# kimkyeonghun/MSA

Hardware: AMD Instinct MI355X
Metric: train-step samples/sec (higher is better)
Workload: dtype bf16

## Files before the change

### include/mmbert_hip.h

```cpp
#ifndef MMBERT_HIP_H
#define MMBERT_HIP_H
#include <stddef.h>
#include <stdint.h>

#ifdef __cplusplus
extern "C" {
#endif

typedef struct ihipStream_t* mmbert_stream_t;

#define MMBERT_EPI_BIAS 1
#define MMBERT_EPI_GELU 2
#define MMBERT_EPI_RESID 4
#define MMBERT_EPI_GELU_BWD 8
#define MMBERT_EPI_OUT_F32 16

int mmbert_gemm_nt(mmbert_stream_t stream, const void* A, int lda, const void* B, int ldb, void* C, int ldc,
                   int M, int N, int K, int epi, const float* bias, const void* R, int ldr, void* aux, int ldaux,
                   const void* U, int ldu, float alpha, const float* alpha_dev,
                   uint32_t drop_stream, uint32_t drop_thr16, float drop_scale, int* tile_queue);

int mmbert_gemm_nt_splitk(mmbert_stream_t stream, const void* A, int lda, const void* B, int ldb, void* C, int ldc,
                          int M, int N, int K, void* workspace, const void* R, int ldr);
size_t mmbert_gemm_nt_splitk_workspace(int M, int N, int K);

void mmbert_gemm_nt_force(int mode);
int mmbert_gemm_nt_describe(int M, int N, int K, int epi, int with_queue, int* out);
void mmbert_gemm_tn_force_splits(int splits);
void mmbert_gemm_tn_force_one_launch(int on);

size_t mmbert_gemm_tn_workspace(int M, int N, int K, int* splits_out);
int mmbert_gemm_tn(mmbert_stream_t stream, const void* A, int lda, const void* B, int ldb, float* W, int ldw,
                   int M, int N, int K, int accumulate, float alpha, const float* alpha_dev, void* slab, float* bias_out);
size_t mmbert_gemm_tn_grouped_workspace(int nprob, const int* N, const int* K, int M, int* splits_out);
int mmbert_gemm_tn_grouped(mmbert_stream_t stream, int nprob, const void* const* A, const int* lda, const void* const* B, const int* ldb,
                           float* const* W, float* const* bias, const int* N, const int* K, int M,
                           int accumulate, float alpha, const float* alpha_dev, void* slab);
int mmbert_gemm_tn_grouped_rows(mmbert_stream_t stream, int nprob, const void* const* A, const int* lda, const void* const* B, const int* ldb,
                                float* const* W, float* const* bias, const int* N, const int* K, const int* M,
                                int accumulate, const int* accumulate_each, float alpha, const float* alpha_dev, void* slab);

int mmbert_colsum(mmbert_stream_t stream, const void* X, int ldx, int M, int N, float* out, float alpha, const float* alpha_dev);

uint32_t mmbert_rng_stream(uint64_t seed, uint32_t site);
uint32_t mmbert_dropout_thr16(float p);
int mmbert_dropout_mask(mmbert_stream_t stream, uint8_t* out, size_t n, uint32_t rng_stream, uint32_t thr16);

int mmbert_mlm_mask(mmbert_stream_t stream, int64_t* ids, int64_t* labels, size_t n, uint32_t rng_stream, uint32_t select_thr16,
                    uint32_t replace_thr16, int64_t special0, int64_t special1, int64_t special2, int64_t mask_id);

int mmbert_ln_fwd(mmbert_stream_t stream, const void* x, int ldx, const int* in_rows, void* y, int ldy, const int* out_rows,
                  int M, int H, const float* gamma, const float* beta, float eps, float* mean, float* rstd,
                  uint32_t dstream, uint32_t dthr, float dscale, int drop_row0);
int mmbert_ln_bwd(mmbert_stream_t stream, const void* dy, int lddy, const int* dy_rows, const void* x, int ldx, const int* x_rows,
                  const float* mean, const float* rstd, const float* gamma, int M, int H,
                  void* dx, int lddx, const int* dx_rows, void* dx2, int lddx2, float* dgamma, float* dbeta, float* dbias2,
                  uint32_t post_stream, uint32_t post_thr, float post_scale,
                  uint32_t pre_stream, uint32_t pre_thr, float pre_scale,
                  float* partial_ws , const int* drop_rows,
                  int defer_reduce ,
                  int dy_row_limit );
size_t mmbert_ln_bwd_workspace(int M, int H);
int mmbert_ln_bwd_reduce(mmbert_stream_t stream, int items, const float* const* partial_ws, float* const* dgamma, float* const* dbeta,
                         float* const* dbias2, int M, int H);
int mmbert_ln_bwd_reduce_rows(mmbert_stream_t stream, int items, const float* const* partial_ws, float* const* dgamma, float* const* dbeta,
                              float* const* dbias2, const int* M, int H);

int mmbert_embed_gather(mmbert_stream_t stream, const int64_t* ids, const int64_t* tts, const float* word, const float* type,
                        const float* pos, int n, int T, int H, int V, void* out, int ldo);
int mmbert_embed_scatter(mmbert_stream_t stream, const int64_t* ids, const int64_t* tts, const void* d, int ldd, int n, int T, int H, int V,
                         float* gword, float* gtype, float* gpos, float* type_slab);

int mmbert_pair_proj_fwd(mmbert_stream_t stream, const void* feat, int feat_f64, int B, int P, int D, const float* W, const float* bias, int H,
                         void* out, int ldo, int T);
int mmbert_pair_proj_bwd(mmbert_stream_t stream, const void* feat, int feat_f64, int B, int P, int D, const void* J, const void* dJ, int ld, int T,
                         float* dW, float* db, int H, void* workspace );
size_t mmbert_pair_proj_bwd_workspace(int B, int P, int D, int H);

int mmbert_attn_tile_rows(int which);
int mmbert_attn_kv_len(mmbert_stream_t stream, const float* key_bias, const int* bias_start, const int* seq_len, int nseq, int* kv_len);
int mmbert_attn_fwd(mmbert_stream_t stream, const void* qkv, void* ctx, float* lse, const float* key_bias, const int* bias_start, int H, int heads,
                    const int* seq_start, const int* seq_len, const unsigned* elem_base, const int* tile_seq, const int* tile_r0, int ntiles,
                    uint32_t dstream, uint32_t dthr, float dscale, const int* kv_len, const int* tile_qshift, const int* tile_qend);
int mmbert_attn_fwd_first(mmbert_stream_t stream, const void* qkv, void* ctx, const float* key_bias, const int* bias_start, int H, int heads,
                          const int* seq_start, const int* seq_len, const int* q_row, int nseq, const int* kv_len);
int mmbert_attn_probs_first(mmbert_stream_t stream, const void* qkv, float* probs, int ld, const float* key_bias, const int* bias_start, int H, int heads,
                            const int* seq_start, const int* seq_len, const int* q_row, int nseq, const int* kv_len );
int mmbert_attn_bwd(mmbert_stream_t stream, const void* qkv, const void* ctx, const void* dctx, void* dqkv, const float* lse, float* delta,
                    const float* key_bias, const int* bias_start, int H, int heads, const int* seq_start, const int* seq_len, const unsigned* elem_base,
                    const int* qtile_seq, const int* qtile_r0, int nqtiles,
                    const int* tile_seq, const int* tile_r0, int ntiles,
                    uint32_t dstream, uint32_t dthr, float dscale, const int* kv_len,
                    const int* qtile_qshift, const int* qtile_qend, int split,
                    const int* q_limit);
int mmbert_attn_q_limit(mmbert_stream_t stream, const int* rows, int n, const int* seq_start, int nseq, int* q_limit);
int mmbert_attn_dropout_mask(mmbert_stream_t stream, uint8_t* out, int S, unsigned elem_base, int head, uint32_t rng_stream, uint32_t thr16);

int mmbert_ce_fwd(mmbert_stream_t stream, const void* logits, int ldv, int V, const int64_t* labels, int M,
                  const int* seg_bounds, int nseg, float* inv_count, float* loss_sum, float* row_lse,
                  int logits_f32 ,
                  float* row_loss );
int mmbert_ce_bwd(mmbert_stream_t stream, const void* logits, int ldv, int V, const int64_t* labels, int M,
                  const int* seg_bounds, int nseg, const float* inv_count, const float* gscale, const float* row_lse, void* dlogits, int ldd,
                  const int* rows , int nrows,
                  int logits_f32 );
int mmbert_vocab_topk(mmbert_stream_t stream, const void* logits, int ldv, int V, int M, int logits_f32, int k,
                      const int64_t* labels ,
                      int32_t* top_ids , float* top_logprob , float* row_lse ,
                      float* label_logprob , int32_t* label_rank );
int mmbert_split_rows(mmbert_stream_t stream, const int64_t* row_seq, const int64_t* row_pos, const int* start_a, const int* start_b,
                      const int* valid, int mode, int M, int rows_a, int64_t* perm, int64_t* inv, const int* rank,
                      int* perm32 , int* inv32);

int mmbert_split_layout(mmbert_stream_t stream, const int* seq_len, const int* valid, int nseq, int tile_rows, int xs, int nf_max, int nq_max,
                        int* out);

int mmbert_prologue(mmbert_stream_t stream, int nseg, const void* const* seg_ptr, const long long* seg_stride_b, const long long* seg_stride_p,
                    const int* seg_dtype, const int* seg_pass, const int* seg_offset, const int* seg_len,
                    int npass, const int* pass_len, int B, const int64_t* labels, int vocab,
                    float* key_bias, int* kv_len, int* valid, int* seq_cnt, int* idx, int* words, int* rank, float* key_bias_perm);

int mmbert_rows_to_block(mmbert_stream_t stream, const int64_t* ids, const void* rows, int rows_bf16, int ldr, int n, int H,
                         const int64_t* uni, int U, int V, float* block);

int mmbert_pack_i64(mmbert_stream_t stream, int nseg, const int64_t* const* src, const long long* dst_offset, const long long* count,
                    const long long* fill, int64_t* out);

int mmbert_active_rows(mmbert_stream_t stream, const int64_t* labels, int M, int V, int* idx, int* count);

int mmbert_heads_gate_fwd(mmbert_stream_t stream, const float* P, const float* Apre, const float* const* vw3, const float* const* vb3, int B, int H, float* g, float* C);
int mmbert_heads_loss_fwd(mmbert_stream_t stream, const float* P, const float* XP, const float* rel, const int64_t* ap, const float* lo, const float* sent,
                          int B, int H, float beta, int tanh_lo, float* out5, float* dXP, float* dPc, float* drel, float* dlo, float* nce_part,
                          const float* mlm, int nmlm, float alpha, float* loss_out , float* aux_out );
int mmbert_heads_scale(mmbert_stream_t stream, float* x, size_t n, const float* s);
int mmbert_heads_seed(mmbert_stream_t stream, const float* src, size_t n, const float* s, float* dst, float* zero, size_t nzero, float* dmlm, int nmlm, float coef);
int mmbert_heads_gate_bwd(mmbert_stream_t stream, const float* dC, const float* P, const float* Apre, const float* g, const float* const* vw3, const float* dPc,
                          int B, int H, float* dP, float* dApre, float* E, float* dg);
int mmbert_heads_tanh(mmbert_stream_t stream, float* x, size_t n);
int mmbert_heads_tanh_bwd(mmbert_stream_t stream, const float* dP, const float* P, float* dpre, size_t n);
int mmbert_heads_colsum(mmbert_stream_t stream, int nseg, const float* const* src, float* const* dst, const int* rows, const int* cols, const int* ld);

typedef struct {
    int B, H, tanh_lo, nmlm;
    float alpha, beta;
    const float* first; const void* y; const int64_t* first_rows; int ldy, ncls;
    const int64_t* ap; const int64_t* ap2; const float* sent; const float* mlm;
    const float *Wp, *bp, *Wal, *bal, *Wsr, *bsr, *Wat, *bat, *vw[3], *vb[3], *Wc1, *bc1, *Wc2, *bc2, *Wq[3], *bq[3];
    float *loss, *aux, *out5, *logits, *t_rel, *rel;
    float* ws;
    const float* dloss; float* dfirst; float* dmlm;
    float *gWp, *gbp, *gWal, *gbal, *gWat, *gbat, *gvw[3], *gvb[3], *gWc1, *gbc1, *gWc2, *gbc2, *gWq[3], *gbq[3];
    unsigned* sync;
    const int64_t* sent_cls; int64_t* pred;
} mmbert_heads_step;
int mmbert_heads_step_struct_size(void);
size_t mmbert_heads_step_workspace(int B, int H);
int mmbert_heads_step_fwd(mmbert_stream_t stream, const mmbert_heads_step* p);
int mmbert_heads_step_bwd(mmbert_stream_t stream, const mmbert_heads_step* p);
int mmbert_heads_step_fwd_levels(mmbert_stream_t stream, const mmbert_heads_step* p, int lo, int hi);
int mmbert_heads_step_bwd_levels(mmbert_stream_t stream, const mmbert_heads_step* p, int lo, int hi);
int mmbert_heads_predict(mmbert_stream_t stream, const mmbert_heads_step* p);
int mmbert_heads_step_outputs(int B, int H, size_t* pooled_offset, size_t* fused_offset);
int mmbert_heads_step_dmlm(mmbert_stream_t stream, const mmbert_heads_step* p);

typedef struct { const float* X; const float* W; int ldx, ldw, inner, row0, rows, w_inner_major; } mmbert_skinny_src;
typedef struct { float* Y; const float* bias; int ldy, M, N, nsrc, act, accumulate; mmbert_skinny_src src[4]; } mmbert_skinny_op;
typedef struct { const float* dY; const float* X; float* dW; float* db; int ldy, ldx, ldw, M, N, K; } mmbert_skinny_wgrad_op;
int mmbert_skinny_mm(mmbert_stream_t stream, int nops, const mmbert_skinny_op* ops);
size_t mmbert_skinny_mm_workspace(int nops, const mmbert_skinny_op* ops);
int mmbert_skinny_mm_ordered(mmbert_stream_t stream, int nops, const mmbert_skinny_op* ops, void* workspace);
int mmbert_skinny_wgrad(mmbert_stream_t stream, int nops, const mmbert_skinny_wgrad_op* ops);

typedef struct { uint32_t stream, thr16; float scale; } mmbert_drop;
typedef struct {
    const float* key_bias; const int* bias_start; const int* seq_start; const int* seq_len; const unsigned* elem_base;
    const int* ftile_seq; const int* ftile_r0; const int* ftile_qshift; const int* ftile_qend;
    const int* qtile_seq; const int* qtile_r0; const int* qtile_qshift; const int* qtile_qend;
    const int* tile_seq; const int* tile_r0;
    const int* kv_len;
    int nftiles, nqtiles, ntiles, split, heads, pad_;
} mmbert_attn_layout;
typedef struct {
    const void* x;
    const void* Wqkv; const void* Wo; const void* W1; const void* W2;
    const float* bqkv; const float* bo; const float* b1; const float* b2; const float* ln1_g; const float* ln1_b; const float* ln2_g; const float* ln2_b;
    void* qkv; void* actx; float* lse; void* z1; void* y1; float* m1; float* r1; void* u ; void* g; void* z2; void* y2; float* m2; float* r2;
    const int* y2_rows;
    int* tile_queue;
    mmbert_drop att, h1, h2;
    int rows, H, I, ldx, ldy2; float ln_eps;
} mmbert_layer_fwd_args;
typedef struct {
    const void* dy; const int* dy_rows;
    const void* z2; const float* m2; const float* r2; const float* ln2_g; float* g_ln2_g; float* g_ln2_b; float* ln2_ws;
    const void* z1; const float* m1; const float* r1; const float* ln1_g; float* g_ln1_g; float* g_ln1_b; float* ln1_ws;
    const void* u; const void* qkv; const void* actx; const float* lse;
    const void* W2T; const void* W1T; const void* WoT; const void* WqkvT;
    void* dz2; void* dz2d ; void* du; void* dy1; void* dz1; void* dz1d ; void* dctx; void* dqkv; float* delta; void* dx;
    int* tile_queue;
    mmbert_drop att, h1, h2;
    int rows, H, I, lddy;
} mmbert_layer_bwd_args;
int mmbert_layer_fwd(mmbert_stream_t stream, const mmbert_attn_layout* layout, const mmbert_layer_fwd_args* a);
int mmbert_layer_bwd(mmbert_stream_t stream, const mmbert_attn_layout* layout, const mmbert_layer_bwd_args* a);
int mmbert_layer_struct_sizes(int* out );

void mmbert_set_deterministic(int on);
int mmbert_get_deterministic(void);
int mmbert_id_runs_sum_rows(mmbert_stream_t stream, const void* src, int src_bf16, int lds, const int64_t* ids, int n,
                            int H, int V, const int64_t* uni, int U, float* dst, int ldd);

int mmbert_adamw(mmbert_stream_t stream, float* p, float* g, float* m, float* v, void* p_bf16, const uint8_t* flags, size_t n,
                 double lr, double beta1, double beta2, double eps, double wd, int step, double gscale, int mode, int zero_grad);

int mmbert_adamw_devscale(mmbert_stream_t stream, float* p, float* g, float* m, float* v, void* p_bf16, const uint8_t* flags, size_t n,
                          double lr, double beta1, double beta2, double eps, double wd, int step, const float* coef, int mode, int zero_grad);

#define MMBERT_ADAMW_MAX_GROUPS 255
#define MMBERT_ADAMW_MAX_SLOTS 64
int mmbert_adamw_grouped(mmbert_stream_t stream, float* p, float* g, float* m, float* v, void* p_bf16, const uint8_t* flags,
                         const uint8_t* group_of_block, size_t n, const double* hyper, int ngroups, int step, double gscale,
                         const float* coef, int mode, int zero_grad);

#define MMBERT_GRAD_NORM_WORKSPACE 8192
int mmbert_grad_norm(mmbert_stream_t stream, const float* g, size_t n, const int64_t* segs, int nseg, double norm_type, double max_norm,
                     double gscale, void* workspace, float* out);
int mmbert_grad_scale(mmbert_stream_t stream, float* g, size_t n, const int64_t* segs, int nseg, const float* coef);

int mmbert_gelu_bwd(mmbert_stream_t stream, const void* dy, const void* u, void* du, size_t n);

int mmbert_cast_f32_bf16(mmbert_stream_t stream, const float* x, void* y, size_t n);
int mmbert_cast_bf16_f32(mmbert_stream_t stream, const void* x, float* y, size_t n);
int mmbert_transpose_cast(mmbert_stream_t stream, const float* src, void* dst, const void* descs, int ndesc, int total_tiles);
int mmbert_compact_rows(mmbert_stream_t stream, const int* rows32, const int64_t* rows64, int n, const int64_t* extra, int nextra, const int64_t* map,
                        int64_t* out64, int* out32);
int mmbert_compact_rows_inv(mmbert_stream_t stream, const int* rows32, const int64_t* rows64, int n, const int64_t* extra, int nextra, const int64_t* map,
                            int64_t* out64, int* out32, int64_t* inv_stamp, unsigned stamp);
int mmbert_scatter_rows_zero(mmbert_stream_t stream, int nseg, const void* const* src, void* const* dst, const long long* src_pitch,
                             const long long* dst_pitch, const int* row_bytes, const int64_t* inv_stamp, unsigned stamp, int nlist, int nrows);
int mmbert_gather_rows(mmbert_stream_t stream, int nseg, const void* const* src, void* const* dst, const long long* src_pitch, const long long* dst_pitch,
                       const int* row_bytes, const int* idx, int nrows);
int mmbert_transpose_bf16(mmbert_stream_t stream, const void* src, void* dst, const void* descs, int ndesc, int total_tiles);

#ifdef __cplusplus
}
#endif
#endif
```

### msa_amd/_lib.py

```python
from __future__ import annotations

import ctypes as C
import os

HERE = os.path.dirname(os.path.abspath(__file__))
LIB_PATH = os.environ.get("MMBERT_LIB_PATH") or os.path.join(HERE, "libmmbert_hip.so")

P, I, F, D, U32, SZ, U64 = C.c_void_p, C.c_int, C.c_float, C.c_double, C.c_uint32, C.c_size_t, C.c_uint64

SIGNATURES = {
    "mmbert_gemm_nt": (I, [P, P, I, P, I, P, I, I, I, I, I, P, P, I, P, I, P, I, F, P, U32, U32, F, P]),
    "mmbert_gemm_nt_force": (None, [I]),
    "mmbert_gemm_nt_describe": (I, [I, I, I, I, I, P]),
    "mmbert_gemm_nt_splitk": (I, [P, P, I, P, I, P, I, I, I, I, P, P, I]),
    "mmbert_gemm_nt_splitk_workspace": (SZ, [I, I, I]),
    "mmbert_gemm_tn_force_splits": (None, [I]),
    "mmbert_gemm_tn_force_one_launch": (None, [I]),
    "mmbert_gemm_tn_workspace": (SZ, [I, I, I, P]),
    "mmbert_gemm_tn": (I, [P, P, I, P, I, P, I, I, I, I, I, F, P, P, P]),
    "mmbert_gemm_tn_grouped_workspace": (SZ, [I, P, P, I, P]),
    "mmbert_gemm_tn_grouped": (I, [P, I, P, P, P, P, P, P, P, P, I, I, F, P, P]),
    "mmbert_gemm_tn_grouped_rows": (I, [P, I, P, P, P, P, P, P, P, P, P, I, P, F, P, P]),
    "mmbert_colsum": (I, [P, P, I, I, I, P, F, P]),
    "mmbert_rng_stream": (U32, [U64, U32]),
    "mmbert_dropout_thr16": (U32, [F]),
    "mmbert_dropout_mask": (I, [P, P, SZ, U32, U32]),
    "mmbert_mlm_mask": (I, [P, P, P, SZ, U32, U32, U32, C.c_int64, C.c_int64, C.c_int64, C.c_int64]),
    "mmbert_ln_fwd": (I, [P, P, I, P, P, I, P, I, I, P, P, F, P, P, U32, U32, F, I]),
    "mmbert_ln_bwd": (I, [P, P, I, P, P, I, P, P, P, P, I, I, P, I, P, P, I, P, P, P, U32, U32, F, U32, U32, F, P, P, I, I]),
    "mmbert_ln_bwd_reduce": (I, [P, I, P, P, P, P, I, I]),
    "mmbert_ln_bwd_reduce_rows": (I, [P, I, P, P, P, P, P, I]),
    "mmbert_ln_bwd_workspace": (SZ, [I, I]),
    "mmbert_embed_gather": (I, [P, P, P, P, P, P, I, I, I, I, P, I]),
    "mmbert_embed_scatter": (I, [P, P, P, P, I, I, I, I, I, P, P, P, P]),
    "mmbert_pair_proj_fwd": (I, [P, P, I, I, I, I, P, P, I, P, I, I]),
    "mmbert_pair_proj_bwd": (I, [P, P, I, I, I, I, P, P, I, I, P, P, I, P]),
    "mmbert_pair_proj_bwd_workspace": (SZ, [I, I, I, I]),
    "mmbert_attn_tile_rows": (I, [I]),
    "mmbert_attn_kv_len": (I, [P, P, P, P, I, P]),
    "mmbert_attn_fwd": (I, [P, P, P, P, P, P, I, I, P, P, P, P, P, I, U32, U32, F, P, P, P]),
    "mmbert_attn_fwd_first": (I, [P, P, P, P, P, I, I, P, P, P, I, P]),
    "mmbert_attn_probs_first": (I, [P, P, P, I, P, P, I, I, P, P, P, I, P]),
    "mmbert_attn_bwd": (I, [P, P, P, P, P, P, P, P, P, I, I, P, P, P, P, P, I, P, P, I, U32, U32, F, P, P, P, I, P]),
    "mmbert_attn_q_limit": (I, [P, P, I, P, I, P]),
    "mmbert_attn_dropout_mask": (I, [P, P, I, C.c_uint, I, U32, U32]),
    "mmbert_ce_fwd": (I, [P, P, I, I, P, I, P, I, P, P, P, I, P]),
    "mmbert_ce_bwd": (I, [P, P, I, I, P, I, P, I, P, P, P, P, I, P, I, I]),
    "mmbert_vocab_topk": (I, [P, P, I, I, I, I, I, P, P, P, P, P, P]),
    "mmbert_active_rows": (I, [P, P, I, I, P, P]),
    "mmbert_prologue": (I, [P, I, P, P, P, P, P, P, P, I, P, I, P, I, P, P, P, P, P, P, P, P]),
    "mmbert_split_rows": (I, [P, P, P, P, P, P, I, I, I, P, P, P, P, P]),
    "mmbert_heads_gate_fwd": (I, [P, P, P, P, P, I, I, P, P]),
    "mmbert_heads_loss_fwd": (I, [P, P, P, P, P, P, P, I, I, F, I, P, P, P, P, P, P, P, I, F, P, P]),
    "mmbert_heads_scale": (I, [P, P, SZ, P]),
    "mmbert_heads_seed": (I, [P, P, SZ, P, P, P, SZ, P, I, F]),
    "mmbert_heads_gate_bwd": (I, [P, P, P, P, P, P, P, I, I, P, P, P, P]),
    "mmbert_heads_tanh": (I, [P, P, SZ]),
    "mmbert_heads_tanh_bwd": (I, [P, P, P, P, SZ]),
    "mmbert_heads_colsum": (I, [P, I, P, P, P, P, P]),
    "mmbert_skinny_mm": (I, [P, I, P]),
    "mmbert_skinny_mm_workspace": (SZ, [I, P]),
    "mmbert_skinny_mm_ordered": (I, [P, I, P, P]),
    "mmbert_heads_step_struct_size": (I, []),
    "mmbert_heads_step_workspace": (SZ, [I, I]),
    "mmbert_heads_step_fwd": (I, [P, P]),
    "mmbert_heads_step_bwd": (I, [P, P]),
    "mmbert_heads_step_fwd_levels": (I, [P, P, I, I]),
    "mmbert_heads_step_bwd_levels": (I, [P, P, I, I]),
    "mmbert_heads_step_dmlm": (I, [P, P]),
    "mmbert_heads_predict": (I, [P, P]),
    "mmbert_heads_step_outputs": (I, [I, I, P, P]),
    "mmbert_layer_fwd": (I, [P, P, P]),
    "mmbert_layer_bwd": (I, [P, P, P]),
    "mmbert_layer_struct_sizes": (I, [P]),
    "mmbert_set_deterministic": (None, [I]),
    "mmbert_get_deterministic": (I, []),
    "mmbert_id_runs_sum_rows": (I, [P, P, I, I, P, I, I, I, P, I, P, I]),
    "mmbert_skinny_wgrad": (I, [P, I, P]),
    "mmbert_adamw": (I, [P, P, P, P, P, P, P, SZ, D, D, D, D, D, I, D, I, I]),
    "mmbert_adamw_devscale": (I, [P, P, P, P, P, P, P, SZ, D, D, D, D, D, I, P, I, I]),
    "mmbert_adamw_grouped": (I, [P, P, P, P, P, P, P, P, SZ, P, I, I, D, P, I, I]),
    "mmbert_grad_norm": (I, [P, P, SZ, P, I, D, D, D, P, P]),
    "mmbert_grad_scale": (I, [P, P, SZ, P, I, P]),
    "mmbert_gelu_bwd": (I, [P, P, P, P, SZ]),
    "mmbert_cast_f32_bf16": (I, [P, P, P, SZ]),
    "mmbert_cast_bf16_f32": (I, [P, P, P, SZ]),
    "mmbert_transpose_cast": (I, [P, P, P, P, I, I]),
    "mmbert_transpose_bf16": (I, [P, P, P, P, I, I]),
    "mmbert_gather_rows": (I, [P, I, P, P, P, P, P, P, I]),
    "mmbert_compact_rows": (I, [P, P, P, I, P, I, P, P, P]),
    "mmbert_compact_rows_inv": (I, [P, P, P, I, P, I, P, P, P, P, C.c_uint]),
    "mmbert_scatter_rows_zero": (I, [P, I, P, P, P, P, P, P, C.c_uint, I, I]),
    "mmbert_pack_i64": (I, [P, I, P, P, P, P, P]),
    "mmbert_rows_to_block": (I, [P, P, P, I, I, I, I, P, I, I, P]),
    "mmbert_split_layout": (I, [P, P, P, I, I, I, I, I, P]),
}

_lib = None


def load() -> C.CDLL:
    global _lib
    if _lib is not None:
        return _lib
    if not os.path.exists(LIB_PATH):
        raise RuntimeError(
            f"{LIB_PATH} not found: the MI355X kernels are not built and there is no CPU fallback. "
            "Run `python -m msa_amd.build` (needs hipcc) first.")
    lib = C.CDLL(LIB_PATH)
    for name, (res, args) in SIGNATURES.items():
        fn = getattr(lib, name)
        fn.restype = res
        fn.argtypes = args
    _lib = lib
    return lib


def check(code: int, what: str) -> None:
    if code != 0:
        raise RuntimeError(f"{what} failed with code {code} "
                           f"({'invalid argument' if code < 0 else 'hipError_t'})")
```

### msa_amd/csrc/gemm.hip

```cpp
#include "common.h"
#include <atomic>
#include <cstdio>
#include <cstdlib>
#include <cstring>
#include <type_traits>

typedef __attribute__((ext_vector_type(4))) unsigned u32x4;
typedef __attribute__((ext_vector_type(2))) unsigned u32x2;

#define EPI_BIAS 1
#define EPI_GELU 2
#define EPI_RESID 4
#define EPI_GELU_BWD 8
#define EPI_OUT_F32 16

struct GemmNT {
    const bf16_t* A; const bf16_t* B; void* C;
    const float* bias; const bf16_t* R; bf16_t* aux; const bf16_t* U; const float* alpha_dev;
    int M, N, K, lda, ldb, ldc, ldr, ldaux, ldu;
    float alpha;
    uint32_t drop_stream, drop_thr16; float drop_scale;
    int kt_per_split; long long split_stride;
    int* tile_counter; int* tile_counter_next;
    int queue_xcd;
    int group_m;
};

__device__ __forceinline__ int xcd_remap(int bid, int nwg) {
    const int q = nwg >> 3, r = nwg & 7, x = bid & 7, j = bid >> 3;
    return (x < r ? x * (q + 1) : r * (q + 1) + (x - r) * q) + j;
}

__device__ __forceinline__ void ntp_tile_mn(int t, int tiles_m, int tiles_n, int gm, int& tm, int& tn) {
    if (gm <= 1) { tm = t / tiles_n; tn = t - tm * tiles_n; return; }
    const int per = gm * tiles_n, g = t / per, r = t - g * per;
    const int gs = min(gm, tiles_m - g * gm);
    tn = r / gs;
    tm = g * gm + (r - tn * gs);
}

template <int EPI>
__device__ __forceinline__ void epi_store(const GemmNT& p, int m, int n, float (&v)[4]) {
    if constexpr (EPI & EPI_BIAS) {
        const float4 b = *(const float4*)(p.bias + n);
        v[0] += b.x; v[1] += b.y; v[2] += b.z; v[3] += b.w;
    }
    if constexpr (EPI & EPI_GELU) {
        if (p.aux) {
            bf16x4 u = {f2bf(v[0]), f2bf(v[1]), f2bf(v[2]), f2bf(v[3])};
            *(bf16x4*)(p.aux + (size_t)m * p.ldaux + n) = u;
        }
#pragma unroll
        for (int r = 0; r < 4; ++r) v[r] = gelu_erf(v[r]);
    }
    if constexpr (EPI & EPI_GELU_BWD) {
        const bf16x4 u = *(const bf16x4*)(p.U + (size_t)m * p.ldu + n);
#pragma unroll
        for (int r = 0; r < 4; ++r) v[r] *= gelu_erf_grad(bf2f(u[r]));
    }
    if constexpr (EPI & EPI_RESID) {
        if (p.drop_thr16) {
            bool k[4];
            mmb_keep4(p.drop_stream, (uint64_t)m * p.N + n, p.drop_thr16, k);
#pragma unroll
            for (int r = 0; r < 4; ++r) v[r] = k[r] ? v[r] * p.drop_scale : 0.f;
        }
        const bf16x4 rr = *(const bf16x4*)(p.R + (size_t)m * p.ldr + n);
#pragma unroll
        for (int r = 0; r < 4; ++r) v[r] += bf2f(rr[r]);
    }
    if constexpr (EPI & EPI_OUT_F32) {
        *(float4*)((float*)p.C + (size_t)m * p.ldc + n) = make_float4(v[0], v[1], v[2], v[3]);
    } else {
        bf16x4 o = {f2bf(v[0]), f2bf(v[1]), f2bf(v[2]), f2bf(v[3])};
        *(bf16x4*)((bf16_t*)p.C + (size_t)m * p.ldc + n) = o;
    }
}

template <int EPI>
__device__ __forceinline__ void epi_store8(const GemmNT& p, int m, int n, float (&v)[8]) {
    if constexpr (EPI & EPI_BIAS) {
        const float4 b0 = *(const float4*)(p.bias + n), b1 = *(const float4*)(p.bias + n + 4);
        v[0] += b0.x; v[1] += b0.y; v[2] += b0.z; v[3] += b0.w; v[4] += b1.x; v[5] += b1.y; v[6] += b1.z; v[7] += b1.w;
    }
    if constexpr (EPI & EPI_GELU) {
        if (p.aux) {
            bf16x8 u;
#pragma unroll
            for (int r = 0; r < 8; ++r) u[r] = f2bf(v[r]);
            *(bf16x8*)(p.aux + (size_t)m * p.ldaux + n) = u;
        }
#pragma unroll
        for (int r = 0; r < 8; ++r) v[r] = gelu_erf(v[r]);
    }
    if constexpr (EPI & EPI_GELU_BWD) {
        const bf16x8 u = *(const bf16x8*)(p.U + (size_t)m * p.ldu + n);
#pragma unroll
        for (int r = 0; r < 8; ++r) v[r] *= gelu_erf_grad(bf2f(u[r]));
    }
    if constexpr (EPI & EPI_RESID) {
        if (p.drop_thr16) {
            bool k0[4], k1[4];
            const uint64_t idx = (uint64_t)m * p.N + n;
            mmb_keep4(p.drop_stream, idx, p.drop_thr16, k0);
            mmb_keep4(p.drop_stream, idx + 4, p.drop_thr16, k1);
#pragma unroll
            for (int r = 0; r < 4; ++r) { v[r] = k0[r] ? v[r] * p.drop_scale : 0.f; v[4 + r] = k1[r] ? v[4 + r] * p.drop_scale : 0.f; }
        }
        const bf16x8 rr = *(const bf16x8*)(p.R + (size_t)m * p.ldr + n);
#pragma unroll
        for (int r = 0; r < 8; ++r) v[r] += bf2f(rr[r]);
    }
    if constexpr (EPI & EPI_OUT_F32) {
        float* c = (float*)p.C + (size_t)m * p.ldc + n;
        *(float4*)c = make_float4(v[0], v[1], v[2], v[3]);
        *(float4*)(c + 4) = make_float4(v[4], v[5], v[6], v[7]);
    } else {
        bf16x8 o;
#pragma unroll
        for (int r = 0; r < 8; ++r) o[r] = f2bf(v[r]);
        *(bf16x8*)((bf16_t*)p.C + (size_t)m * p.ldc + n) = o;
    }
}

template <int EPI>
__global__ __launch_bounds__(256, 2) void gemm_nt_kernel(const GemmNT p) {
    extern __shared__ __attribute__((aligned(16))) char smem[];
    const int tid = threadIdx.x, lane = tid & 63;
    const int wave = __builtin_amdgcn_readfirstlane(tid >> 6);
    const int wm = wave >> 1, wn = wave & 1;
    const int tiles_n = (p.N + 127) >> 7, tiles_m = (p.M + 127) >> 7;
    const int tile = xcd_remap(blockIdx.x, tiles_m * tiles_n);
    const int m0 = (tile / tiles_n) << 7, n0 = (tile % tiles_n) << 7;
    const int kt0 = p.kt_per_split ? (int)blockIdx.z * p.kt_per_split : 0;
    const int kt1 = p.kt_per_split ? min(p.K >> 6, kt0 + p.kt_per_split) : (p.K >> 6);

    const int srow = lane >> 3, schunk = (lane & 7) ^ srow;
    const bf16_t* a_src[4]; const bf16_t* b_src[4];
#pragma unroll
    for (int i = 0; i < 4; ++i) {
        const int r = (wave * 4 + i) * 8 + srow;
        const int ra = min(m0 + r, p.M - 1), rb = min(n0 + r, p.N - 1);
        a_src[i] = p.A + (size_t)ra * p.lda + schunk * 8;
        b_src[i] = p.B + (size_t)rb * p.ldb + schunk * 8;
    }
    auto stage = [&](int buf, int kt) {
        char* base = smem + buf * 32768 + wave * 4096;
#pragma unroll
        for (int i = 0; i < 4; ++i) {
            __builtin_amdgcn_global_load_lds(GPTR(a_src[i] + kt * 64), LPTR(base + i * 1024), 16, 0, 0);
            __builtin_amdgcn_global_load_lds(GPTR(b_src[i] + kt * 64), LPTR(base + 16384 + i * 1024), 16, 0, 0);
        }
    };

    f32x4 acc[4][4];
#pragma unroll
    for (int i = 0; i < 4; ++i)
#pragma unroll
        for (int j = 0; j < 4; ++j) acc[i][j] = (f32x4){0.f, 0.f, 0.f, 0.f};

    const int fr = lane & 15, fq = lane >> 4;
    auto compute = [&](int buf) {
        const char* As = smem + buf * 32768;
        const char* Bs = As + 16384;
#pragma unroll
        for (int kk = 0; kk < 2; ++kk) {
            bf16x8 af[4], bfr[4];
#pragma unroll
            for (int i = 0; i < 4; ++i) {
                const int ra = wm * 64 + i * 16 + fr, rb = wn * 64 + i * 16 + fr;
                af[i] = *(const bf16x8*)(As + ra * 128 + (((kk * 4 + fq) ^ (ra & 7)) << 4));
                bfr[i] = *(const bf16x8*)(Bs + rb * 128 + (((kk * 4 + fq) ^ (rb & 7)) << 4));
            }
#pragma unroll
            for (int i = 0; i < 4; ++i)
#pragma unroll
                for (int j = 0; j < 4; ++j)
                    acc[i][j] = __builtin_amdgcn_mfma_f32_16x16x32_bf16(bfr[j], af[i], acc[i][j], 0, 0, 0);
        }
    };

    stage(0, kt0);
    asm volatile("s_waitcnt vmcnt(0)" ::: "memory");
    __syncthreads();
    int cur = 0;
    for (int kt = kt0; kt < kt1 - 1; ++kt) {
        stage(cur ^ 1, kt + 1);
        compute(cur);
        asm volatile("s_waitcnt vmcnt(0)" ::: "memory");
        __syncthreads();
        cur ^= 1;
    }
    compute(cur);

    const float alpha = p.alpha * (p.alpha_dev ? *p.alpha_dev : 1.0f);
#pragma unroll
    for (int i = 0; i < 4; ++i) {
        const int m = m0 + wm * 64 + i * 16 + fr;
        if (m >= p.M) continue;
#pragma unroll
        for (int j = 0; j < 4; ++j) {
            const int n = n0 + wn * 64 + j * 16 + fq * 4;
            if (n >= p.N) continue;
            float v[4];
#pragma unroll
            for (int r = 0; r < 4; ++r) v[r] = acc[i][j][r] * alpha;
            if constexpr (EPI == EPI_OUT_F32) {
                if (p.kt_per_split) {
                    *(float4*)((float*)p.C + (size_t)blockIdx.z * p.split_stride + (size_t)m * p.ldc + n) = make_float4(v[0], v[1], v[2], v[3]);
                    continue;
                }
            }
            epi_store<EPI>(p, m, n, v);
        }
    }
}

template <int EPI>
static int launch_nt(hipStream_t s, const GemmNT& p) {
    const int tiles = ((p.M + 127) / 128) * ((p.N + 127) / 128);
    static std::atomic<unsigned long long> attr_done{0};
    if (int e = mmb_allow_lds((const void*)gemm_nt_kernel<EPI>, 65536, attr_done)) return e;
    hipLaunchKernelGGL(gemm_nt_kernel<EPI>, dim3(tiles), dim3(256), 65536, s, p);
    MMB_CHECK_LAUNCH();
    return 0;
}

#ifdef MMB_STAMPS
__device__ unsigned long long* g_stamps = nullptr;
#define MMB_STAMP(var) { __builtin_amdgcn_sched_barrier(0); asm volatile("s_memtime %0\n\ts_waitcnt lgkmcnt(0)" : "=s"(var) :: "memory"); __builtin_amdgcn_sched_barrier(0); }
#else
#define MMB_STAMP(var)
#endif

static std::atomic<int> g_nt_force{0};
static int device_cus() { return mmb_device_cus(); }

__host__ __device__ constexpr int mmb_waitcnt(int vm, int lgkm) { return (vm & 15) | ((vm >> 4) << 14) | 0x70 | (lgkm << 8); }

template <int OFF>
__device__ __forceinline__ void lds_read16f(f32x4& dst, uint32_t lds_addr) {
    asm volatile("ds_read_b128 %0, %1 offset:%2" : "=v"(dst) : "v"(lds_addr), "i"(OFF) : "memory");
}


template <int EPI, bool MULTI, int MQ>
__global__ __launch_bounds__(512, 2) void gemm_nt8_kernel(const GemmNT p) {
#if __HIP_DEVICE_COMPILE__
    extern __shared__ __attribute__((aligned(16))) char smem[];
    const int tid = threadIdx.x, lane = tid & 63;
    const int wave = __builtin_amdgcn_readfirstlane(tid >> 6);
    const int wr = wave >> 2, wc = wave & 3;
    constexpr int MQ0 = (MQ == 7) ? 4 : MQ, MQ1 = (MQ == 7) ? 3 : MQ, NB = MQ0 + MQ1;
    constexpr int BMT = 32 * NB;
    const int tiles_n = (p.N + 255) >> 8, tiles_m = (p.M + BMT - 1) / BMT;
    const int ntiles = tiles_m * tiles_n, G = gridDim.x;
    const int nt = p.K >> 6;
    const float alpha_all = __builtin_bit_cast(float, __builtin_amdgcn_readfirstlane(__builtin_bit_cast(int, p.alpha * (p.alpha_dev ? *p.alpha_dev : 1.0f))));

    const auto rsA = __builtin_amdgcn_make_buffer_rsrc((void*)p.A, 0, (int)((uint32_t)p.M * (uint32_t)p.lda * 2u), 0x00020000);
    const auto rsB = __builtin_amdgcn_make_buffer_rsrc((void*)p.B, 0, (int)((uint32_t)p.N * (uint32_t)p.ldb * 2u), 0x00020000);
    struct Src { uint32_t a[2][2], b[2][2]; };
    auto set_src = [&](int v, Src& o) {
        int l = lane;
        asm volatile("" : "+v"(l));
        int tmi, tni;
        ntp_tile_mn(xcd_remap(v, ntiles), tiles_m, tiles_n, p.group_m, tmi, tni);
        const int tm0 = tmi * BMT, tn0 = tni << 8;
        const int pos = l & 7;
#pragma unroll
        for (int i = 0; i < 2; ++i) {
            const int j = wave + 8 * i, r = 8 * j + (l >> 3);
            const uint32_t chunk_a = (uint32_t)(pos ^ ((r >> 1) & 7));
            const uint32_t chunk_b = (uint32_t)(pos ^ (((r >> 1) & 1) | (((r >> 3) & 3) << 1)));
#pragma unroll
            for (int h = 0; h < 2; ++h) {
                const int mqh = h ? MQ1 : MQ0;
                const int ga = tm0 + (r / (16 * mqh)) * (16 * NB) + (h ? 16 * MQ0 : 0) + (r % (16 * mqh));
                const int gb = tn0 + (r >> 5) * 64 + h * 32 + (r & 31);
                o.a[h][i] = ((uint32_t)min(ga, p.M - 1) * (uint32_t)p.lda + chunk_a * 8u) * 2u;
                o.b[h][i] = ((uint32_t)min(gb, p.N - 1) * (uint32_t)p.ldb + chunk_b * 8u) * 2u;
            }
        }
    };
    Src cur;
    set_src(blockIdx.x, cur);
    Src nxt_store;
    Src& nxt = MULTI ? nxt_store : cur;
    if constexpr (MULTI) nxt_store = cur;
    auto stage_c = [&](auto apw_c, int buf, int which, const Src& o, int kt) {
        constexpr int APW = decltype(apw_c)::value;
        const uint32_t kb = (uint32_t)kt * 128u;
        const int h = which >> 1;
        char* base = smem + buf * 65536 + ((which & 1) ? 0 : 32768) + h * 16384 + wave * 1024;
        if (which & 1) {
            __builtin_amdgcn_raw_ptr_buffer_load_lds(rsA, LPTR(base), 16, o.a[h][0], kb, 0, 0);
            const int mqh = h ? MQ1 : MQ0;
            if (mqh == 4 || (mqh == 3 && APW == 2)) __builtin_amdgcn_raw_ptr_buffer_load_lds(rsA, LPTR(base + 8192), 16, o.a[h][1], kb, 0, 0);
        } else {
            __builtin_amdgcn_raw_ptr_buffer_load_lds(rsB, LPTR(base), 16, o.b[h][0], kb, 0, 0);
            __builtin_amdgcn_raw_ptr_buffer_load_lds(rsB, LPTR(base + 8192), 16, o.b[h][1], kb, 0, 0);
        }
    };

    typedef const __attribute__((address_space(3))) char* lds_cptr;
    typedef const __attribute__((address_space(3))) bf16x8* lds_frag;
    const int fr = lane & 15, fq = lane >> 4;
    const int swa = ((fq ^ (fr >> 1)) & 7) << 4;
    const int swb = ((fq ^ (((fr >> 1) & 1) | ((fr >> 2) << 1))) & 7) << 4;
    const lds_cptr a_rd = (lds_cptr)LPTR(smem) + (wr * (16 * MQ0) + fr) * 128;
    const lds_cptr b_rd = (lds_cptr)LPTR(smem) + 32768 + (wc * 32 + 8 * (fr >> 2) + (fr & 3)) * 128;
    lds_cptr a_rd1 = a_rd + 65536, b_rd1 = b_rd + 65536;
    asm volatile("" : "+v"(a_rd1), "+v"(b_rd1));

    bf16x8 af[2][MQ0], b0f[2][2], b1f[2][2];
    f32x4 acc[NB][4];

    auto read_a = [&](int buf, int h) {
        lds_cptr ab = buf ? a_rd1 : a_rd;
        if (MQ0 != MQ1 && h) ab += wr * (16 * (MQ1 - MQ0) * 128);
#pragma unroll
        for (int ks = 0; ks < 2; ++ks)
#pragma unroll
            for (int i = 0; i < MQ0; ++i)
                if (i < (h ? MQ1 : MQ0)) af[ks][i] = *(lds_frag)(ab + h * 16384 + i * 2048 + (swa ^ (ks * 64)));
    };
    auto read_b = [&](int buf, int h, bf16x8 (&bf)[2][2]) {
        const lds_cptr bb = buf ? b_rd1 : b_rd;
#pragma unroll
        for (int ks = 0; ks < 2; ++ks)
#pragma unroll
            for (int j = 0; j < 2; ++j) bf[ks][j] = *(lds_frag)(bb + h * 16384 + j * 512 + (swb ^ (ks * 64)));
    };
    auto mma = [&](int qa, int qb, const bf16x8 (&bf)[2][2], bool first) {
#pragma unroll
        for (int ks = 0; ks < 2; ++ks)
#pragma unroll
            for (int i = 0; i < MQ0; ++i)
#pragma unroll
                for (int j = 0; j < 2; ++j) {
                    if (i >= (qa ? MQ1 : MQ0)) continue;
                    f32x4& c = acc[qa * MQ0 + i][qb * 2 + j];
                    c = __builtin_amdgcn_mfma_f32_16x16x32_bf16(bf[ks][j], af[ks][i], (first && ks == 0) ? (f32x4){0.f, 0.f, 0.f, 0.f} : c, 0, 0, 0);
                }
    };

    auto body = [&](auto apw_c) {
    constexpr int INFL = 4 + (MQ0 == 4 ? 2 : (MQ0 == 2 ? 1 : decltype(apw_c)::value));
    auto stage = [&](int buf, int which, const Src& o, int kt) { stage_c(apw_c, buf, which, o, kt); };
    const int qx = (MULTI && p.queue_xcd) ? (int)(blockIdx.x & 7) : 0, qs = (MULTI && p.queue_xcd) ? 8 : 1;
    auto queue_fetch = [](int* counter) {
        int r;
        asm volatile("s_nop 4\n\tglobal_atomic_add %0, %1, %2, %3 sc0" : "=&v"(r) : "v"(0), "v"(1), "s"(counter) : "memory");
        return r;
    };
    auto vq_write = [&](int value) {
        const uint32_t vq_addr = (uint32_t)(size_t)LPTR(smem) + 131072u;
        asm volatile("ds_write_b32 %0, %1\n\ts_waitcnt lgkmcnt(0)" :: "v"(vq_addr), "v"(value) : "memory");
    };
    int first_fetch = 0;
    if constexpr (MULTI) { if (p.tile_counter && tid == 0) first_fetch = queue_fetch(p.tile_counter + qx); }
    stage(0, 0, cur, 0); stage(0, 1, cur, 0); stage(0, 2, cur, 0); stage(0, 3, cur, 0);
    stage(1, 0, cur, 1); stage(1, 1, cur, 1); stage(1, 2, cur, 1);
    __builtin_amdgcn_s_waitcnt(mmb_waitcnt(INFL, 15));
    if constexpr (MULTI) {
        if (p.tile_counter && tid == 0) {
            asm volatile("" : "+v"(first_fetch) :: "memory");
            vq_write(G + qs * first_fetch + qx);
        }
    }
    __builtin_amdgcn_s_barrier();
    if (wr == 1) __builtin_amdgcn_s_barrier();

#define NT8_PHASE(READS, LGK_BEFORE_BARRIER, STAGE, VMWAIT, QA, QB, BF, FIRST)                                       \
    {                                                                                                               \
        READS;                                                                                                      \
        STAGE;                                                                                                      \
        if (LGK_BEFORE_BARRIER >= 0) __builtin_amdgcn_s_waitcnt(mmb_waitcnt(63, LGK_BEFORE_BARRIER < 0 ? 0 : LGK_BEFORE_BARRIER)); \
        if (VMWAIT >= 0) __builtin_amdgcn_s_waitcnt(mmb_waitcnt(VMWAIT < 0 ? 0 : VMWAIT, 15));                       \
        __builtin_amdgcn_s_barrier();                                                                               \
        __builtin_amdgcn_s_waitcnt(mmb_waitcnt(63, 0));                                                             \
        __builtin_amdgcn_sched_barrier(0);                                                                          \
        __builtin_amdgcn_s_setprio(1);                                                                              \
        mma(QA, QB, BF, FIRST);                                                                                     \
        __builtin_amdgcn_s_setprio(0);                                                                              \
        __builtin_amdgcn_s_barrier();                                                                               \
        __builtin_amdgcn_sched_barrier(0);                                                                          \
    }
#define NT8_KTILE(D, S1, K1, S2, K2, FIRST)                                                                                   \
    NT8_PHASE((read_b(D, 0, b0f), __builtin_amdgcn_sched_barrier(0), read_a(D, 0)), 2 * MQ0, stage(D ^ 1, 3, S1, K1), -1, 0, 0, b0f, FIRST) \
    NT8_PHASE(read_b(D, 1, b1f), -1, stage(D, 0, S2, K2), -1, 0, 1, b1f, FIRST)                                               \
    NT8_PHASE(read_a(D, 1), -1, stage(D, 1, S2, K2), -1, 1, 1, b1f, FIRST)                                                    \
    NT8_PHASE((void)0, -1, stage(D, 2, S2, K2), INFL, 1, 0, b0f, FIRST)

    for (int v = blockIdx.x, vn = ntiles; v < ntiles; v = vn) {
        int tmi, tni;
        ntp_tile_mn(xcd_remap(v, ntiles), tiles_m, tiles_n, p.group_m, tmi, tni);
        const int m0 = tmi * BMT, n0 = tni << 8;
        __builtin_amdgcn_s_waitcnt(mmb_waitcnt(INFL, 15));
        NT8_KTILE(0, cur, 1, cur, 2, true)
        if constexpr (EPI & EPI_BIAS) {
            int l = lane;
            asm volatile("" : "+v"(l));
            auto kpb = __builtin_amdgcn_kernarg_segment_ptr();
            asm volatile("" : "+s"(kpb));
            const __attribute__((address_space(4))) GemmNT& qb = *(const __attribute__((address_space(4))) GemmNT*)kpb;
            const auto rsBias = __builtin_amdgcn_make_buffer_rsrc((void*)qb.bias, 0, qb.N * 4, 0x00020000);
            __builtin_amdgcn_raw_ptr_buffer_load_lds(rsBias, LPTR(smem + 131136 + wave * 256), 4, l * 4, (n0 + wc * 64) * 4, 0, 0);
        }
        int fetched = 0;
        if constexpr (MULTI) {
            if (p.tile_counter) {
                int qv;
                const uint32_t vq_addr = (uint32_t)(size_t)LPTR(smem) + 131072u;
                asm volatile("ds_read_b32 %0, %1\n\ts_waitcnt lgkmcnt(0)" : "=v"(qv) : "v"(vq_addr) : "memory");
                vn = __builtin_amdgcn_readfirstlane(qv);
                if (tid == 0 && vn < ntiles) fetched = queue_fetch(p.tile_counter + qx);
            } else {
                vn = v + G;
            }
            if (vn < ntiles) set_src(vn, nxt_store);
        }
        NT8_KTILE(1, cur, 2, cur, 3, false)
        if constexpr (MULTI) {
            if (p.tile_counter && tid == 0 && vn < ntiles) {
                asm volatile("" : "+v"(fetched) :: "memory");
                vq_write(G + qs * fetched + qx);
            }
        }
        for (int t = 2; t < nt - 2; t += 2) {
            NT8_KTILE(0, cur, t + 1, cur, t + 2, false)
            NT8_KTILE(1, cur, t + 2, cur, t + 3, false)
        }
        NT8_KTILE(0, cur, nt - 1, nxt, 0, false)
        NT8_KTILE(1, nxt, 0, nxt, 1, false)
        if constexpr (MULTI) cur = nxt_store;

        auto kp = __builtin_amdgcn_kernarg_segment_ptr();
        asm volatile("" : "+s"(kp));
        const __attribute__((address_space(4))) GemmNT& q = *(const __attribute__((address_space(4))) GemmNT*)kp;
        int elane = lane;
        asm volatile("" : "+v"(elane));
        const int efr = elane & 15, efq = elane >> 4;
        const float alpha = alpha_all;
        const bool interior = (m0 + BMT <= q.M) && (n0 + 256 <= q.N);
        const int mrow = m0 + wr * (16 * NB) + efr;
        const int ncol = n0 + wc * 64 + efq * 8;
        constexpr int PRE = 3;
        bf16x8 pre[NB][2];
        constexpr uint32_t CSZ = (EPI & EPI_OUT_F32) ? 4u : 2u;
        const uint32_t um = (uint32_t)q.M, um1 = um ? um - 1u : 0u, un = um ? (uint32_t)q.N : 0u;
        const auto rsC = __builtin_amdgcn_make_buffer_rsrc((void*)q.C, 0, (int)((um1 * (uint32_t)q.ldc + un) * CSZ), 0x00020000);
        const uint32_t voffC = ((uint32_t)mrow * (uint32_t)q.ldc + (uint32_t)ncol) * CSZ, rowC = 16u * (uint32_t)q.ldc * CSZ;
        const bf16_t* presrc = (EPI & EPI_RESID) ? q.R : q.U;
        const uint32_t preld = (uint32_t)((EPI & EPI_RESID) ? q.ldr : q.ldu);
        const auto rsP = __builtin_amdgcn_make_buffer_rsrc((void*)presrc, 0, (int)((EPI & (EPI_RESID | EPI_GELU_BWD)) ? (um1 * preld + un) * 2u : 0u), 0x00020000);
        const uint32_t voffP = ((uint32_t)mrow * preld + (uint32_t)ncol) * 2u, rowP = 32u * preld;
        auto load_pre = [&](int i) {
            if constexpr (EPI & (EPI_RESID | EPI_GELU_BWD)) {
                const uint32_t vo = voffP + (uint32_t)i * rowP;
                pre[i][0] = __builtin_bit_cast(bf16x8, __builtin_amdgcn_raw_buffer_load_b128(rsP, vo, 0, 0));
                pre[i][1] = __builtin_bit_cast(bf16x8, __builtin_amdgcn_raw_buffer_load_b128(rsP, vo + 64u, 0, 0));
            }
        };
#pragma unroll
        for (int i = 0; i < PRE; ++i) load_pre(i);
        float bias[16];
        if constexpr (EPI & EPI_BIAS) {
            const uint32_t baddr = (uint32_t)(size_t)LPTR(smem) + 131136u + wave * 256u + efq * 32u;
            f32x4 b4[4];
            lds_read16f<0>(b4[0], baddr); lds_read16f<16>(b4[1], baddr); lds_read16f<128>(b4[2], baddr); lds_read16f<144>(b4[3], baddr);
            asm volatile("s_waitcnt lgkmcnt(0)" : "+v"(b4[0]), "+v"(b4[1]), "+v"(b4[2]), "+v"(b4[3]) :: "memory");
#pragma unroll
            for (int c = 0; c < 4; ++c)
#pragma unroll
                for (int r = 0; r < 4; ++r) bias[4 * c + r] = b4[c][r];
        }
        const uint32_t dthr = (EPI & EPI_RESID) ? q.drop_thr16 : 0u;
        const uint32_t dthr_s = dthr - 32768u;
        const float dscale = (EPI & EPI_RESID) ? q.drop_scale : 1.0f;
        const uint32_t halfN = (uint32_t)q.N >> 1;
        const uint32_t seed0 = (EPI & EPI_RESID) ? ((uint32_t)mrow * halfN + ((uint32_t)ncol >> 1)) * MMB_WEYL + q.drop_stream : 0u;
        const uint32_t seed_row = 16u * halfN * MMB_WEYL;
#pragma unroll
        for (int i = 0; i < NB; ++i) {
#pragma unroll
            for (int h = 0; h < 2; ++h) {
#pragma unroll
                for (int r = 0; r < 8; ++r) {
                    float v_ = acc[i][2 * h + (r >> 2)][r & 3] * alpha;
                    if constexpr (EPI & EPI_BIAS) v_ += bias[8 * h + r];
                    acc[i][2 * h + (r >> 2)][r & 3] = v_;
                }
                if constexpr (EPI & EPI_RESID) {
                    if (dthr) {
#pragma unroll
                        for (int k = 0; k < 4; ++k) {
                            uint32_t hb = mmb_pair_mix(seed0 + (uint32_t)i * seed_row + (uint32_t)(16 * h + k) * MMB_WEYL);
                            asm("" : "+v"(hb));
                            f32x4& a4 = acc[i][2 * h + (k >> 1)];
                            const bool keep0 = (int16_t)(uint16_t)(hb & 0xFFFFu) >= (int16_t)(uint16_t)dthr_s;
                            const bool keep1 = (int16_t)(uint16_t)(hb >> 16) >= (int16_t)(uint16_t)dthr_s;
                            a4[(2 * k) & 3] = keep0 ? a4[(2 * k) & 3] * dscale : 0.f;
                            a4[(2 * k + 1) & 3] = keep1 ? a4[(2 * k + 1) & 3] * dscale : 0.f;
                        }
                    }
                }
            }
        }
#pragma unroll
        for (int i = 0; i < NB; ++i) {
            if (i + PRE < NB) load_pre(i + PRE);
            const int m = mrow + 16 * i;
#pragma unroll
            for (int h = 0; h < 2; ++h) {
                const int n = ncol + 32 * h;
                float vv[8];
#pragma unroll
                for (int r = 0; r < 8; ++r) vv[r] = acc[i][2 * h + (r >> 2)][r & 3];
                const bool ok = interior || (m < q.M && n + 8 <= q.N);
                if constexpr (EPI & EPI_GELU) {
                    if (q.aux) {
                        bf16x8 u;
#pragma unroll
                        for (int r = 0; r < 8; ++r) u[r] = f2bf(vv[r]);
                        const auto rsX = __builtin_amdgcn_make_buffer_rsrc((void*)q.aux, 0, (int)((um1 * (uint32_t)q.ldaux + un) * 2u), 0x00020000);
                        const uint32_t vo = ((uint32_t)mrow * (uint32_t)q.ldaux + (uint32_t)ncol) * 2u + (uint32_t)i * (32u * (uint32_t)q.ldaux) + (uint32_t)h * 64u;
                        if (ok) __builtin_amdgcn_raw_buffer_store_b128(__builtin_bit_cast(u32x4, u), rsX, vo, 0, 0);
                    }
#pragma unroll
                    for (int r = 0; r < 8; r += 4) {
                        mmb_f2 g0 = {vv[r], vv[r + 1]}, g1 = {vv[r + 2], vv[r + 3]};
                        gelu_erf4(g0, g1);
                        vv[r] = g0.x; vv[r + 1] = g0.y; vv[r + 2] = g1.x; vv[r + 3] = g1.y;
                    }
                }
                if constexpr (EPI & EPI_GELU_BWD) {
#pragma unroll
                    for (int r = 0; r < 8; r += 4) {
                        mmb_f2 d0, d1;
                        gelu_erf_grad4((mmb_f2){bf2f(pre[i][h][r]), bf2f(pre[i][h][r + 1])}, (mmb_f2){bf2f(pre[i][h][r + 2]), bf2f(pre[i][h][r + 3])}, d0, d1);
                        vv[r] *= d0.x; vv[r + 1] *= d0.y; vv[r + 2] *= d1.x; vv[r + 3] *= d1.y;
                    }
                }
                if constexpr (EPI & EPI_RESID) {
#pragma unroll
                    for (int r = 0; r < 8; ++r) vv[r] += bf2f(pre[i][h][r]);
                }
                const uint32_t voC = voffC + (uint32_t)i * rowC + (uint32_t)h * (32u * CSZ);
                if constexpr (EPI & EPI_OUT_F32) {
                    f32x4 lo = {vv[0], vv[1], vv[2], vv[3]}, hi = {vv[4], vv[5], vv[6], vv[7]};
                    asm volatile("" : "+v"(lo), "+v"(hi));
                    if (ok) {
                        __builtin_amdgcn_raw_buffer_store_b128(__builtin_bit_cast(u32x4, lo), rsC, voC, 0, 0);
                        __builtin_amdgcn_raw_buffer_store_b128(__builtin_bit_cast(u32x4, hi), rsC, voC + 16u, 0, 0);
                    }
                } else {
                    bf16x8 o;
#pragma unroll
                    for (int r = 0; r < 8; ++r) o[r] = f2bf(vv[r]);
                    u32x4 ow = __builtin_bit_cast(u32x4, o);
                    asm volatile("" : "+v"(ow));
                    if (ok) __builtin_amdgcn_raw_buffer_store_b128(ow, rsC, voC, 0, 0);
                }
            }
        }
    }
#undef NT8_KTILE
#undef NT8_PHASE
    };
    if constexpr (MQ0 == 3 || MQ1 == 3) {
        if (wave < 4) body(std::integral_constant<int, 2>{}); else body(std::integral_constant<int, 1>{});
    } else {
        body(std::integral_constant<int, MQ0 / 2>{});
    }
    if (wr == 0) __builtin_amdgcn_s_barrier();
    asm volatile("s_waitcnt vmcnt(0)" ::: "memory");
    if constexpr (MULTI) {
        auto kpe = __builtin_amdgcn_kernarg_segment_ptr();
        asm volatile("" : "+s"(kpe));
        const __attribute__((address_space(4))) GemmNT& qe = *(const __attribute__((address_space(4))) GemmNT*)kpe;
        if (qe.tile_counter && tid == 0) {
            if (atomicAdd(qe.tile_counter_next, 1) == (int)gridDim.x - 1) {
                for (int x = 0; x < 8; ++x) atomicExch(qe.tile_counter + x, 0);
                atomicExch(qe.tile_counter_next, 0);
            }
        }
    }
#endif
}

template <int EPI, bool MULTI, int MQ>
static int launch_nt8_form(hipStream_t s, const GemmNT& q, int workgroups) {
    static std::atomic<unsigned long long> attr_done{0};
    constexpr int LDS = 131072 + 64 + 8 * 256;
    if (int e = mmb_allow_lds((const void*)gemm_nt8_kernel<EPI, MULTI, MQ>, LDS, attr_done)) return e;
    hipLaunchKernelGGL((gemm_nt8_kernel<EPI, MULTI, MQ>), dim3(workgroups), dim3(512), LDS, s, q);
    MMB_CHECK_LAUNCH();
    return 0;
}
template <int EPI>
static int launch_nt8(hipStream_t s, const GemmNT& p, int bm, int tiles, int workgroups, int group_m) {
    GemmNT q = p;
    q.group_m = group_m;
    const bool use_queue = p.tile_counter && tiles > workgroups && !(workgroups & 7);
    if (!use_queue) q.tile_counter = q.tile_counter_next = nullptr;
    q.queue_xcd = 1;
    const bool multi = tiles > workgroups;
    if (bm == 128) return launch_nt8_form<EPI, false, 2>(s, q, workgroups);
    if (bm == 192) return multi ? launch_nt8_form<EPI, true, 3>(s, q, workgroups) : launch_nt8_form<EPI, false, 3>(s, q, workgroups);
    if (bm == 224) return multi ? launch_nt8_form<EPI, true, 7>(s, q, workgroups) : launch_nt8_form<EPI, false, 7>(s, q, workgroups);
    return multi ? launch_nt8_form<EPI, true, 4>(s, q, workgroups) : launch_nt8_form<EPI, false, 4>(s, q, workgroups);
}

enum { NTK_128 = 0, NTK_8PHASE = 3 };
struct NTChoice { int kernel, bm, tiles, workgroups, group_m, use_queue; };

static bool nt8_eligible(const GemmNT& p, int epi) {
    const long long m = p.M, esz = (epi & EPI_OUT_F32) ? 4 : 2;
    return !(p.K & 127) && p.K >= 256 && m * p.lda < (1ll << 31) && (long long)p.N * p.ldb < (1ll << 31) && m * p.ldc * esz < (1ll << 32) &&
           m * p.ldr * 2 < (1ll << 32) && m * p.ldaux * 2 < (1ll << 32) && m * p.ldu * 2 < (1ll << 32);
}

static int nt_group_m(int M, int N, int K, int bm, int tiles, int cus) {
    if (tiles <= cus) return 1;
    if ((long long)N * K * 2 > (8ll << 20)) return tiles > 4 * cus ? 4 : 1;
    return ((M + bm - 1) / bm + 7) / 8;
}

static NTChoice nt_choose(const GemmNT& p, int epi) {
    NTChoice c = {NTK_128, 128, ((p.M + 127) / 128) * ((p.N + 127) / 128), 0, 1, 0};
    c.workgroups = c.tiles;
    const int force = g_nt_force.load();
    const bool big = (p.M >= 512) && (p.N >= 256) && !(p.N & 7) && !(p.ldc & 7) && !(p.ldr & 7) && !(p.ldaux & 7) && !(p.ldu & 7);
    if (force == 1 || !nt8_eligible(p, epi) || (p.N & 7) || (force == 0 && !big)) return c;
    const int cus = device_cus(), tn = (p.N + 255) / 256;
    auto tiles_of = [&](int h) { return ((p.M + h - 1) / h) * tn; };
    const int t128 = tiles_of(128), t192 = tiles_of(192), t224 = tiles_of(224), t256 = tiles_of(256);
    auto take = [&](int h) {
        const int t = tiles_of(h);
        c.kernel = NTK_8PHASE; c.bm = h; c.tiles = t;
        c.workgroups = (h == 128 || t <= cus) ? t : cus;
        c.group_m = nt_group_m(p.M, p.N, p.K, h, t, cus);
        c.use_queue = p.tile_counter != nullptr && t > c.workgroups && !(cus & 7);
        return c;
    };
    if (force == 128 || force == 192 || force == 224 || force == 256) return take(force);
    if (t256 <= cus) {
        if (2 * t256 <= cus) {
            if (t128 <= cus && 2 * t128 >= cus) return take(128);
            if (force == 0 && c.tiles <= 2 * cus) return c;
            return take(256);
        }
        if (t192 <= cus) return take(192);
        if (t224 <= cus && t224 > t256) return take(224);
        return take(256);
    }
    auto rounds = [&](int t) { return (long long)((t + cus - 1) / cus); };
    const long long c192 = rounds(t192) * 1680, c224 = rounds(t224) * 1800, c256 = rounds(t256) * 2048;
    int h = 224;
    if (100 * c256 < 97 * c224 && c256 <= c192) h = 256;
    else if (100 * c192 < 97 * c224 && c192 < c256) h = 192;
    return take(h);
}

template <int EPI>
static int dispatch_nt(hipStream_t s, const GemmNT& p) {
    const NTChoice c = nt_choose(p, EPI);
    if (c.kernel == NTK_128) return launch_nt<EPI>(s, p);
    return launch_nt8<EPI>(s, p, c.bm, c.tiles, c.workgroups, c.group_m);
}

struct TNProb { const bf16_t* A; const bf16_t* B; float* W; float* bias; int N, K, lda, ldb, tiles_k, tile0, M, slab_off, bias_off, acc; };
#define TN_MAXP 52
struct GemmTNG {
    TNProb pr[TN_MAXP];
    float* slab; const float* alpha_dev;
    float* bias_slab; long long bias_stride;
    long long slab_stride;
    int nprob, total_tiles, M, splits, rows_per_split, accumulate;
    float alpha;
    int tile_base;
    int remap_n;
};

__device__ __forceinline__ int tn_swz(int row) { return ((row & 3) | ((row >> 1) & 4)) << 1; }

template <int OFF>
__device__ __forceinline__ void tr_read(u32x2& dst, unsigned lds_addr) {
    asm volatile("ds_read_b64_tr_b16 %0, %1 offset:%2" : "=v"(dst) : "v"(lds_addr), "i"(OFF) : "memory");
}

__global__ __launch_bounds__(512, 2) void gemm_tn8_kernel(const GemmTNG g) {
#if __HIP_DEVICE_COMPILE__
    extern __shared__ __attribute__((aligned(16))) char smem[];
    const int tid = threadIdx.x, lane = tid & 63;
    const int wave = __builtin_amdgcn_readfirstlane(tid >> 6);
    const int wr = wave >> 2, wc = wave & 3;
    int t_lin = g.tile_base + ((int)blockIdx.x < g.remap_n ? xcd_remap(blockIdx.x, g.remap_n) : (int)blockIdx.x);
    const __attribute__((address_space(4))) GemmTNG& gq = *(const __attribute__((address_space(4))) GemmTNG*)__builtin_amdgcn_kernarg_segment_ptr();
    int pi = 0;
    {
        int lo = 0, hi = g.nprob - 1;
        while (lo < hi) { const int mid = (lo + hi + 1) >> 1; if (gq.pr[mid].tile0 <= t_lin) lo = mid; else hi = mid - 1; }
        pi = lo;
    }
    const __attribute__((address_space(4))) TNProb& pr = gq.pr[pi];
    const bf16_t* Ap = pr.A; const bf16_t* Bp = pr.B; float* Wp = pr.W; float* biasp = pr.bias;
    const int N = pr.N, K = pr.K, lda = pr.lda, ldb = pr.ldb, tiles_k = pr.tiles_k;
    const int slab_off = pr.slab_off, bias_off = pr.bias_off;
    t_lin -= pr.tile0;
    const int n0 = (t_lin / tiles_k) << 8, k0 = (t_lin % tiles_k) << 8;
    const int split = blockIdx.y;
    const int mbeg = split * g.rows_per_split;
    const int mend = min(pr.M, mbeg + g.rows_per_split);
    const int nt = (mend - mbeg + 63) >> 6;
    const bool do_bias = (biasp != nullptr) && (k0 == 0);

    const auto rsY = __builtin_amdgcn_make_buffer_rsrc((void*)Ap, 0, (int)((uint32_t)max(mend, 0) * (uint32_t)lda * 2u), 0x00020000);
    const auto rsX = __builtin_amdgcn_make_buffer_rsrc((void*)Bp, 0, (int)((uint32_t)max(mend, 0) * (uint32_t)ldb * 2u), 0x00020000);
    uint32_t y_off[2], x_off[2];
    {
        const int row4 = lane >> 4, pos = lane & 15;
        const int key = (row4 | (((wave >> 1) & 1) << 2)) << 1;
#pragma unroll
        for (int h = 0; h < 2; ++h) {
            const int cy = min(n0 + h * 128 + ((pos ^ key) << 3), N - 8);
            const int cx = min(k0 + h * 128 + ((pos ^ key) << 3), K - 8);
            y_off[h] = ((uint32_t)row4 * (uint32_t)lda + (uint32_t)cy) * 2u;
            x_off[h] = ((uint32_t)row4 * (uint32_t)ldb + (uint32_t)cx) * 2u;
        }
    }
    auto stage = [&](int buf, int which, int kt) {
        const int h = which >> 1;
        const uint32_t row = (uint32_t)(mbeg + kt * 64 + 4 * wave);
        char* base = smem + buf * 65536 + ((which & 1) ? 0 : 32768) + h * 16384 + wave * 1024;
        if (which & 1) {
            __builtin_amdgcn_raw_ptr_buffer_load_lds(rsX, LPTR(base), 16, x_off[h], row * (uint32_t)ldb * 2u, 0, 0);
            __builtin_amdgcn_raw_ptr_buffer_load_lds(rsX, LPTR(base + 8192), 16, x_off[h], (row + 32u) * (uint32_t)ldb * 2u, 0, 0);
        } else {
            __builtin_amdgcn_raw_ptr_buffer_load_lds(rsY, LPTR(base), 16, y_off[h], row * (uint32_t)lda * 2u, 0, 0);
            __builtin_amdgcn_raw_ptr_buffer_load_lds(rsY, LPTR(base + 8192), 16, y_off[h], (row + 32u) * (uint32_t)lda * 2u, 0, 0);
        }
    };

    const int g4 = lane >> 4, r0 = 8 * g4 + ((lane >> 2) & 3), pp = lane & 3;
    const int keyr = tn_swz(r0);
    const unsigned lds0 = (unsigned)(uintptr_t)LPTR(smem);
    unsigned adX[2][4], adY[2][2];
#pragma unroll
    for (int i = 0; i < 4; ++i) {
        const int chunk = wr * 8 + 2 * i + (pp >> 1);
        adX[0][i] = lds0 + r0 * 256 + ((chunk ^ keyr) << 4) + ((pp & 1) << 3);
        adX[1][i] = adX[0][i] + 65536;
    }
#pragma unroll
    for (int j = 0; j < 2; ++j) {
        const int chunk = wc * 4 + 2 * j + (pp >> 1);
        adY[0][j] = lds0 + 32768 + r0 * 256 + ((chunk ^ keyr) << 4) + ((pp & 1) << 3);
        adY[1][j] = adY[0][j] + 65536;
    }

    u32x2 xlo[2][4], xhi[2][4], y0lo[2][2], y0hi[2][2], y1lo[2][2], y1hi[2][2];
    f32x4 acc[8][4];
#pragma unroll
    for (int i = 0; i < 8; ++i)
#pragma unroll
        for (int j = 0; j < 4; ++j) acc[i][j] = (f32x4){0.f, 0.f, 0.f, 0.f};
    float bsum[2][2] = {{0.f, 0.f}, {0.f, 0.f}};

    auto read_x_ks = [&](auto buf_c, auto h_c, auto ks_c) {
        constexpr int D = decltype(buf_c)::value, OFF = decltype(h_c)::value * 16384 + decltype(ks_c)::value * 8192, KS = decltype(ks_c)::value;
#pragma unroll
        for (int i = 0; i < 4; ++i) { tr_read<OFF>(xlo[KS][i], adX[D][i]); tr_read<OFF + 1024>(xhi[KS][i], adX[D][i]); }
    };
    auto read_y = [&](auto buf_c, auto h_c, u32x2 (&lo)[2][2], u32x2 (&hi)[2][2]) {
        constexpr int D = decltype(buf_c)::value, OFF = decltype(h_c)::value * 16384;
#pragma unroll
        for (int ks = 0; ks < 2; ++ks)
#pragma unroll
            for (int j = 0; j < 2; ++j) {
                if (ks == 0) { tr_read<OFF>(lo[0][j], adY[D][j]); tr_read<OFF + 1024>(hi[0][j], adY[D][j]); }
                else         { tr_read<OFF + 8192>(lo[1][j], adY[D][j]); tr_read<OFF + 8192 + 1024>(hi[1][j], adY[D][j]); }
            }
    };
    auto mma = [&](int qa, int qb, const u32x2 (&ylo)[2][2], const u32x2 (&yhi)[2][2]) {
#pragma unroll
        for (int ks = 0; ks < 2; ++ks) {
            bf16x8 yf[2];
#pragma unroll
            for (int j = 0; j < 2; ++j) { const u32x4 v = {ylo[ks][j][0], ylo[ks][j][1], yhi[ks][j][0], yhi[ks][j][1]}; yf[j] = __builtin_bit_cast(bf16x8, v); }
#pragma unroll
            for (int i = 0; i < 4; ++i) {
                const u32x4 v = {xlo[ks][i][0], xlo[ks][i][1], xhi[ks][i][0], xhi[ks][i][1]};
                const bf16x8 xf = __builtin_bit_cast(bf16x8, v);
#pragma unroll
                for (int j = 0; j < 2; ++j)
                    acc[qa * 4 + i][qb * 2 + j] = __builtin_amdgcn_mfma_f32_16x16x32_bf16(xf, yf[j], acc[qa * 4 + i][qb * 2 + j], 0, 0, 0);
            }
        }
    };
    auto bias_add = [&](int hb, const u32x2 (&ylo)[2][2], const u32x2 (&yhi)[2][2]) {
#pragma unroll
        for (int j = 0; j < 2; ++j) {
            const uint32_t w0 = wr ? ylo[1][j][0] : ylo[0][j][0], w1 = wr ? ylo[1][j][1] : ylo[0][j][1];
            const uint32_t w2 = wr ? yhi[1][j][0] : yhi[0][j][0], w3 = wr ? yhi[1][j][1] : yhi[0][j][1];
            float s = bsum[hb][j];
            s += __builtin_bit_cast(float, w0 << 16); s += __builtin_bit_cast(float, w0 & 0xFFFF0000u);
            s += __builtin_bit_cast(float, w1 << 16); s += __builtin_bit_cast(float, w1 & 0xFFFF0000u);
            s += __builtin_bit_cast(float, w2 << 16); s += __builtin_bit_cast(float, w2 & 0xFFFF0000u);
            s += __builtin_bit_cast(float, w3 << 16); s += __builtin_bit_cast(float, w3 & 0xFFFF0000u);
            bsum[hb][j] = s;
        }
    };

#ifdef MMB_STAMPS
    unsigned long long ts0 = 0, ts1 = 0, tr0 = 0, tr1 = 0;
    asm volatile("s_memrealtime %0\n\ts_waitcnt lgkmcnt(0)" : "=s"(tr0) :: "memory");
    MMB_STAMP(ts0)
#endif
    typedef std::integral_constant<int, 0> I0; typedef std::integral_constant<int, 1> I1;
#define TN8_PHASE(READS, STAGE, VMWAIT, QA, QB, YLO, YHI, BIAS_HB)                                                    \
    {                                                                                                                \
        READS;                                                                                                       \
        STAGE;                                                                                                       \
        if (VMWAIT >= 0) __builtin_amdgcn_s_waitcnt(mmb_waitcnt(VMWAIT < 0 ? 0 : VMWAIT, 15));                        \
        __builtin_amdgcn_s_barrier();                                                                                \
        asm volatile("s_waitcnt lgkmcnt(0)" ::: "memory");                                                           \
        __builtin_amdgcn_sched_barrier(0);                                                                           \
        __builtin_amdgcn_s_setprio(1);                                                                               \
        mma(QA, QB, YLO, YHI);                                                                                       \
        if (BIAS_HB >= 0) { if (do_bias) bias_add(BIAS_HB < 0 ? 0 : BIAS_HB, YLO, YHI); }                             \
        __builtin_amdgcn_s_setprio(0);                                                                               \
        __builtin_amdgcn_s_barrier();                                                                                \
        __builtin_amdgcn_sched_barrier(0);                                                                           \
    }
#define TN8_KTILE(DC, D, T)                                                                                                          \
    TN8_PHASE((read_y(DC{}, I0{}, y0lo, y0hi), read_x_ks(DC{}, I0{}, I0{}), ({ asm volatile("s_waitcnt lgkmcnt(8)" ::: "memory"); }), \
               read_x_ks(DC{}, I0{}, I1{})), stage(D ^ 1, 3, (T) + 1), -1, 0, 0, y0lo, y0hi, 0)                                       \
    TN8_PHASE(read_y(DC{}, I1{}, y1lo, y1hi), stage(D, 0, (T) + 2), -1, 0, 1, y1lo, y1hi, 1)                                          \
    TN8_PHASE((read_x_ks(DC{}, I1{}, I0{}), read_x_ks(DC{}, I1{}, I1{})), stage(D, 1, (T) + 2), -1, 1, 1, y1lo, y1hi, -1)             \
    TN8_PHASE((void)0, stage(D, 2, (T) + 2), 6, 1, 0, y0lo, y0hi, -1)

    if (nt > 0) {
        stage(0, 0, 0); stage(0, 1, 0); stage(0, 2, 0); stage(0, 3, 0);
        stage(1, 0, 1); stage(1, 1, 1); stage(1, 2, 1);
        __builtin_amdgcn_s_waitcnt(mmb_waitcnt(6, 15));
        __builtin_amdgcn_s_barrier();
        if (wr == 1) __builtin_amdgcn_s_barrier();
        int t = 0;
        while (true) {
            TN8_KTILE(I0, 0, t) if (++t >= nt) break;
            TN8_KTILE(I1, 1, t) if (++t >= nt) break;
        }
        if (wr == 0) __builtin_amdgcn_s_barrier();
        asm volatile("s_waitcnt vmcnt(0)" ::: "memory");
    }
#undef TN8_KTILE
#undef TN8_PHASE
#ifdef MMB_STAMPS
    MMB_STAMP(ts1)
#endif

    const float alpha = g.alpha * (g.alpha_dev ? *g.alpha_dev : 1.0f);
    const int fr = lane & 15, fq = lane >> 4;
    float* out = split > 0 ? g.slab + (size_t)(split - 1) * g.slab_stride + slab_off : Wp;
    const bool accum = (split == 0) && pr.acc;
#pragma unroll
    for (int ib = 0; ib < 8; ib += 2) {
        float4 old[2][4];
        if (accum) {
#pragma unroll
            for (int u = 0; u < 2; ++u) {
                const int kc = min(k0 + ((ib + u) >> 2) * 128 + wr * 64 + ((ib + u) & 3) * 16 + fq * 4, K - 4);
#pragma unroll
                for (int jb = 0; jb < 4; ++jb) {
                    const int nc = min(n0 + (jb >> 1) * 128 + wc * 32 + (jb & 1) * 16 + fr, N - 1);
                    old[u][jb] = *(const float4*)(out + (size_t)nc * K + kc);
                }
            }
        }
#pragma unroll
        for (int u = 0; u < 2; ++u) {
            const int k = k0 + ((ib + u) >> 2) * 128 + wr * 64 + ((ib + u) & 3) * 16 + fq * 4;
            if (k >= K) continue;
#pragma unroll
            for (int jb = 0; jb < 4; ++jb) {
                const int n = n0 + (jb >> 1) * 128 + wc * 32 + (jb & 1) * 16 + fr;
                if (n >= N) continue;
                const f32x4 a = acc[ib + u][jb];
                float4 v = make_float4(a[0] * alpha, a[1] * alpha, a[2] * alpha, a[3] * alpha);
                if (accum) { v.x += old[u][jb].x; v.y += old[u][jb].y; v.z += old[u][jb].z; v.w += old[u][jb].w; }
                *(float4*)(out + (size_t)n * K + k) = v;
            }
        }
    }
    if (do_bias) {
        float* red = (float*)smem;
        float v[2][2];
#pragma unroll
        for (int hb = 0; hb < 2; ++hb)
#pragma unroll
            for (int j = 0; j < 2; ++j) {
                float s = bsum[hb][j];
                s += __shfl_xor(s, 16, 64);
                s += __shfl_xor(s, 32, 64);
                v[hb][j] = s;
            }
        __syncthreads();
        if (wr == 1 && fq == 0) {
#pragma unroll
            for (int hb = 0; hb < 2; ++hb)
#pragma unroll
                for (int j = 0; j < 2; ++j) red[((wc * 2 + hb) * 2 + j) * 16 + fr] = v[hb][j];
        }
        __syncthreads();
        if (wr == 0 && fq == 0) {
#pragma unroll
            for (int hb = 0; hb < 2; ++hb)
#pragma unroll
                for (int j = 0; j < 2; ++j) {
                    const int n = n0 + hb * 128 + wc * 32 + j * 16 + fr;
                    if (n >= N) continue;
                    const float bv = (v[hb][j] + red[((wc * 2 + hb) * 2 + j) * 16 + fr]) * alpha;
                    if (split > 0 && gq.bias_slab) gq.bias_slab[(size_t)(split - 1) * gq.bias_stride + bias_off + n] = bv;
                    else atomicAdd(biasp + n, bv);
                }
        }
    }
#ifdef MMB_STAMPS
    if (g_stamps && tid == 0) {
        asm volatile("s_waitcnt vmcnt(0)" ::: "memory");
        asm volatile("s_memrealtime %0\n\ts_waitcnt lgkmcnt(0)" : "=s"(tr1) :: "memory");
        unsigned long long te;
        MMB_STAMP(te)
        unsigned long long* o = g_stamps + ((size_t)(blockIdx.y * gridDim.x + blockIdx.x)) * 6;
        o[0] = ts1 - ts0; o[1] = (unsigned long long)(nt > 0 ? 2 * nt : 0); o[2] = te - ts1; o[3] = 1; o[4] = tr0; o[5] = tr1;
    }
#endif
#endif
}

struct TNReduce { float* W[TN_MAXP]; long long off[TN_MAXP + 1]; int nprob, splits, accumulate; long long slab_stride;
                  float* bias[TN_MAXP]; long long boff[TN_MAXP + 1]; const float* bias_slab; long long bias_stride; };
__global__ void tn_reduce_kernel(const TNReduce r, const float* __restrict__ slab) {
    if (r.bias_slab) {
        const long long nb = r.boff[r.nprob];
        for (long long e = blockIdx.x * (long long)blockDim.x + threadIdx.x; e < nb; e += (long long)gridDim.x * blockDim.x) {
            int lo = 0, hi = r.nprob - 1;
            while (lo < hi) { const int mid = (lo + hi + 1) >> 1; if (r.boff[mid] <= e) lo = mid; else hi = mid - 1; }
            if (!r.bias[lo]) continue;
            float v = r.bias[lo][e - r.boff[lo]];
            for (int s = 0; s + 1 < r.splits; ++s) v += r.bias_slab[(size_t)s * r.bias_stride + e];
            r.bias[lo][e - r.boff[lo]] = v;
        }
    }
    const long long total4 = r.off[r.nprob] >> 2;
    for (long long i = blockIdx.x * (long long)blockDim.x + threadIdx.x; i < total4; i += (long long)gridDim.x * blockDim.x) {
        const long long e = i << 2;
        int lo = 0, hi = r.nprob - 1;
        while (lo < hi) { const int mid = (lo + hi + 1) >> 1; if (r.off[mid] <= e) lo = mid; else hi = mid - 1; }
        float* W = r.W[lo];
        const long long o = r.off[lo];
        float4* dst = (float4*)(W + (e - o));
        float4 v = *dst;
        for (int s = 0; s + 1 < r.splits; ++s) {
            const float4 t = *(const float4*)(slab + (size_t)s * r.slab_stride + e);
            v.x += t.x; v.y += t.y; v.z += t.z; v.w += t.w;
        }
        *dst = v;
    }
}

__global__ __launch_bounds__(256) void colsum_kernel(const bf16_t* __restrict__ X, int M, int N, int ldx, float* __restrict__ out, float alpha, const float* alpha_dev, int rows_per_block) {
    const int lane = threadIdx.x & 63, sub = threadIdx.x >> 6;
    const int n = (blockIdx.x * 64 + lane) * 8;
    const int mbeg = blockIdx.y * rows_per_block, mend = min(M, mbeg + rows_per_block);
    float s[8];
#pragma unroll
    for (int r = 0; r < 8; ++r) s[r] = 0.f;
    if (n < N) {
        int m = mbeg + sub;
        for (; m + 12 < mend; m += 16) {
            bf16x8 v[4];
#pragma unroll
            for (int u = 0; u < 4; ++u) v[u] = *(const bf16x8*)(X + (size_t)(m + 4 * u) * ldx + n);
#pragma unroll
            for (int u = 0; u < 4; ++u)
#pragma unroll
                for (int r = 0; r < 8; ++r) s[r] += bf2f(v[u][r]);
        }
        for (; m < mend; m += 4) {
            const bf16x8 v = *(const bf16x8*)(X + (size_t)m * ldx + n);
#pragma unroll
            for (int r = 0; r < 8; ++r) s[r] += bf2f(v[r]);
        }
    }
    __shared__ float red[4][64][9];
#pragma unroll
    for (int r = 0; r < 8; ++r) red[sub][lane][r] = s[r];
    __syncthreads();
    if (sub == 0 && n < N) {
        const float a = alpha * (alpha_dev ? *alpha_dev : 1.0f);
#pragma unroll
        for (int r = 0; r < 8; ++r)
            atomicAdd(out + n + r, (red[0][lane][r] + red[1][lane][r] + red[2][lane][r] + red[3][lane][r]) * a);
    }
}

extern "C" {

__global__ void nt_splitk_reduce_kernel(const float* __restrict__ slabs, int splits, long long stride, int M, int N, bf16_t* __restrict__ C, int ldc,
                                        const bf16_t* __restrict__ R, int ldr) {
    const long long i = ((long long)blockIdx.x * blockDim.x + threadIdx.x) * 4;
    if (i >= (long long)M * N) return;
    float4 a = *(const float4*)(slabs + i);
    for (int z = 1; z < splits; ++z) { const float4 b = *(const float4*)(slabs + z * stride + i); a.x += b.x; a.y += b.y; a.z += b.z; a.w += b.w; }
    const int m = (int)(i / N), n = (int)(i - (long long)m * N);
    if (R) { const bf16x4 r = *(const bf16x4*)(R + (size_t)m * ldr + n); a.x += bf2f(r[0]); a.y += bf2f(r[1]); a.z += bf2f(r[2]); a.w += bf2f(r[3]); }
    bf16x4 o = {f2bf(a.x), f2bf(a.y), f2bf(a.z), f2bf(a.w)};
    *(bf16x4*)(C + (size_t)m * ldc + n) = o;
}

static int nt_splitk_plan(int M, int N, int K) {
    const int tiles = ((M + 127) / 128) * ((N + 127) / 128), kt = K >> 6;
    int splits = (2 * device_cus() + tiles - 1) / tiles;
    if (splits > kt / 4) splits = kt / 4;
    if (splits < 1) splits = 1;
    return splits;
}
size_t mmbert_gemm_nt_splitk_workspace(int M, int N, int K) { return (size_t)nt_splitk_plan(M, N, K) * M * N * sizeof(float); }

int mmbert_gemm_nt_splitk(hipStream_t stream, const void* A, int lda, const void* B, int ldb, void* C, int ldc,
                          int M, int N, int K, void* workspace, const void* R, int ldr) {
    if (M <= 0 || N <= 0) return 0;
    if (K <= 0 || (K & 63) || (N & 3) || (lda & 7) || (ldb & 7) || (ldc & 3) || !workspace || (R && (ldr & 3))) return -1;
    GemmNT p = {};
    p.A = (const bf16_t*)A; p.B = (const bf16_t*)B; p.C = workspace; p.M = M; p.N = N; p.K = K; p.lda = lda; p.ldb = ldb; p.ldc = N;
    p.alpha = 1.0f;
    const int splits = nt_splitk_plan(M, N, K), kt = K >> 6;
    p.kt_per_split = (kt + splits - 1) / splits;
    p.split_stride = (long long)M * N;
    const int zs = (kt + p.kt_per_split - 1) / p.kt_per_split;
    static std::atomic<unsigned long long> attr_done{0};
    if (int e = mmb_allow_lds((const void*)gemm_nt_kernel<EPI_OUT_F32>, 65536, attr_done)) return e;
    hipLaunchKernelGGL(gemm_nt_kernel<EPI_OUT_F32>, dim3(((M + 127) / 128) * ((N + 127) / 128), 1, zs), dim3(256), 65536, stream, p);
    MMB_CHECK_LAUNCH();
    const long long n4 = ((long long)M * N + 3) / 4;
    hipLaunchKernelGGL(nt_splitk_reduce_kernel, dim3((unsigned)((n4 + 255) / 256)), dim3(256), 0, stream, (const float*)workspace, zs, p.split_stride, M, N, (bf16_t*)C, ldc,
                       (const bf16_t*)R, ldr);
    MMB_CHECK_LAUNCH();
    return 0;
}

int mmbert_gemm_nt(hipStream_t stream, const void* A, int lda, const void* B, int ldb, void* C, int ldc,
                   int M, int N, int K, int epi, const float* bias, const void* R, int ldr, void* aux, int ldaux,
                   const void* U, int ldu, float alpha, const float* alpha_dev,
                   uint32_t drop_stream, uint32_t drop_thr16, float drop_scale, int* tile_queue) {
    if (M <= 0 || N <= 0) return 0;
    if (K <= 0 || (K & 63) || (N & 3) || (lda & 7) || (ldb & 7) || (ldc & 3)) return -1;
    GemmNT p;
    p.A = (const bf16_t*)A; p.B = (const bf16_t*)B; p.C = C; p.bias = bias; p.R = (const bf16_t*)R;
    p.aux = (bf16_t*)aux; p.U = (const bf16_t*)U; p.alpha_dev = alpha_dev;
    p.M = M; p.N = N; p.K = K; p.lda = lda; p.ldb = ldb; p.ldc = ldc; p.ldr = ldr; p.ldaux = ldaux; p.ldu = ldu;
    p.alpha = alpha; p.drop_stream = drop_stream; p.drop_thr16 = drop_thr16; p.drop_scale = drop_scale;
    p.kt_per_split = 0; p.split_stride = 0; p.group_m = 1;
    p.tile_counter = tile_queue; p.tile_counter_next = tile_queue ? tile_queue + 8 : nullptr;
    switch (epi) {
        case 0: return dispatch_nt<0>(stream, p);
        case EPI_BIAS: return dispatch_nt<EPI_BIAS>(stream, p);
        case EPI_BIAS | EPI_GELU: return dispatch_nt<EPI_BIAS | EPI_GELU>(stream, p);
        case EPI_BIAS | EPI_RESID: return dispatch_nt<EPI_BIAS | EPI_RESID>(stream, p);
        case EPI_RESID: return dispatch_nt<EPI_RESID>(stream, p);
        case EPI_GELU_BWD: return dispatch_nt<EPI_GELU_BWD>(stream, p);
        case EPI_OUT_F32: return dispatch_nt<EPI_OUT_F32>(stream, p);
        case EPI_BIAS | EPI_OUT_F32: return dispatch_nt<EPI_BIAS | EPI_OUT_F32>(stream, p);
        default: return -2;
    }
}

int mmbert_gemm_nt_describe(int M, int N, int K, int epi, int with_queue, int* out) {
    if (!out || M <= 0 || N <= 0 || K <= 0) return -1;
    GemmNT p = {};
    p.M = M; p.N = N; p.K = K; p.lda = K; p.ldb = K; p.ldc = N; p.ldr = (epi & (EPI_RESID)) ? N : 0; p.ldaux = (epi & EPI_GELU) ? N : 0;
    p.ldu = (epi & EPI_GELU_BWD) ? N : 0;
    static int dummy_queue[16];
    p.tile_counter = with_queue ? dummy_queue : nullptr;
    const NTChoice c = nt_choose(p, epi);
    const int cus = device_cus();
    out[0] = c.kernel; out[1] = c.bm; out[2] = c.kernel == NTK_128 ? 128 : 256; out[3] = c.tiles; out[4] = c.workgroups;
    out[5] = (int)(100.0 * c.tiles / cus + 0.5); out[6] = c.group_m; out[7] = cus;
    return 0;
}

#ifdef MMB_STAMPS
int mmbert_debug_set_stamps(void* buf) {
    return (int)hipMemcpyToSymbol(HIP_SYMBOL(g_stamps), &buf, sizeof(buf));
}
#endif
void mmbert_gemm_nt_force(int mode) {
    g_nt_force.store((mode == 1 || mode == 8 || mode == 128 || mode == 192 || mode == 224 || mode == 256) ? mode : 0);
}

static std::atomic<int> g_tn_splits{0};
void mmbert_gemm_tn_force_splits(int splits) { g_tn_splits.store(splits); }
static std::atomic<int> g_tn_one_launch{0};
void mmbert_gemm_tn_force_one_launch(int on) { g_tn_one_launch.store(on ? 1 : 0); }
static int tn_plan(int nprob, const int* N, const int* K, int M, int* splits_out, int* tiles_out) {
    int tiles = 0;
    double elems = 0;
    for (int i = 0; i < nprob; ++i) { tiles += ((N[i] + 255) / 256) * ((K[i] + 255) / 256); elems += (double)N[i] * K[i]; }
    constexpr double T_ROW = 21e-9, T_FIX = 8e-6;
    const int slots = device_cus();
    const int max_splits = (M + 511) / 512;
    double cost[9];
    double best_cost = 1e300;
    int top = 1;
    for (int sp = 1; sp <= 8 && sp <= (max_splits < 1 ? 1 : max_splits); ++sp) {
        const long long wgs = (long long)tiles * sp;
        const long long rounds = (wgs + slots - 1) / slots;
        const double rows = (double)((M + sp - 1) / sp);
        cost[sp] = (rows * T_ROW + T_FIX) * (double)rounds + (sp - 1) * elems * 8.0 / 9.4e12;
        if (cost[sp] < best_cost) best_cost = cost[sp];
        top = sp;
    }
    int best = 1;
    for (int sp = 1; sp <= top; ++sp)
        if (cost[sp] <= 1.03 * best_cost) { best = sp; break; }
    int splits = best;
    if (tiles >= slots && nprob > 8) splits = 1;
    if (g_tn_splits.load() > 0) splits = g_tn_splits.load();
    if (splits > max_splits) splits = max_splits;
    if (splits < 1) splits = 1;
    *splits_out = splits; *tiles_out = tiles;
    return 0;
}

size_t mmbert_gemm_tn_grouped_workspace(int nprob, const int* N, const int* K, int M, int* splits_out) {
    int splits, tiles;
    tn_plan(nprob, N, K, M, &splits, &tiles);
    if (splits_out) *splits_out = splits;
    if (splits == 1) return 0;
    size_t elems = 0, cols = 0;
    for (int i = 0; i < nprob; ++i) { elems += (size_t)N[i] * K[i]; cols += (size_t)N[i]; }
    return (size_t)(splits - 1) * (elems + cols) * sizeof(float);
}

size_t mmbert_gemm_tn_workspace(int M, int N, int K, int* splits_out) {
    return mmbert_gemm_tn_grouped_workspace(1, &N, &K, M, splits_out);
}

int mmbert_gemm_tn_grouped_rows(hipStream_t stream, int nprob, const void* const* A, const int* lda, const void* const* B, const int* ldb,
                                float* const* W, float* const* bias, const int* N, const int* K, const int* Mrows,
                                int accumulate, const int* accumulate_each, float alpha, const float* alpha_dev, void* slab) {
    if (nprob <= 0) return 0;
    if (nprob > TN_MAXP) return -1;
    const int M = Mrows[0];
    if (M <= 0) return 0;
    int nlong = 0;
    while (nlong < nprob && Mrows[nlong] == M) ++nlong;
    for (int i = nlong; i < nprob; ++i)
        if (Mrows[i] >= M || Mrows[i] <= 0) return -1;
    GemmTNG g;
    int splits, tiles_long, tiles_all;
    tn_plan(nlong, N, K, M, &splits, &tiles_long);
    if (nlong < nprob) splits = 1;
    long long off = 0, boff = 0;
    int tile0 = 0;
    TNReduce r;
    for (int i = 0; i < nprob; ++i) {
        if ((N[i] & 7) || (K[i] & 7) || (lda[i] & 7) || (ldb[i] & 7) || N[i] < 8 || K[i] < 8) return -1;
        TNProb& q = g.pr[i];
        q.A = (const bf16_t*)A[i]; q.B = (const bf16_t*)B[i]; q.W = W[i]; q.bias = bias ? bias[i] : nullptr;
        q.N = N[i]; q.K = K[i]; q.lda = lda[i]; q.ldb = ldb[i]; q.M = Mrows[i]; q.acc = accumulate_each ? accumulate_each[i] : accumulate;
        q.tiles_k = (K[i] + 255) / 256; q.tile0 = tile0; q.slab_off = (int)off; q.bias_off = (int)boff;
        r.W[i] = W[i]; r.off[i] = off; r.bias[i] = q.bias; r.boff[i] = boff;
        boff += N[i];
        tile0 += ((N[i] + 255) / 256) * q.tiles_k;
        off += (long long)N[i] * K[i];
    }
    tiles_all = tile0;
    if (splits > 1 && off > 0x7fffffffLL) return -1;
    for (int i = nprob; i < TN_MAXP; ++i) { g.pr[i] = g.pr[0]; g.pr[i].tile0 = 0x7fffffff; r.W[i] = nullptr; r.bias[i] = nullptr; }
    for (int i = nprob; i <= TN_MAXP; ++i) { r.off[i] = off; r.boff[i] = boff; }
    if (splits > 1 && !slab) return -3;
    g.slab = (float*)slab; g.alpha_dev = alpha_dev; g.slab_stride = off;
    const bool det_bias = splits > 1 && mmb_deterministic();
    g.bias_slab = det_bias ? (float*)slab + (size_t)(splits - 1) * off : nullptr;
    g.bias_stride = boff;
    r.bias_slab = g.bias_slab; r.bias_stride = boff; g.nprob = nprob; g.total_tiles = tiles_all; g.M = M;
    g.splits = splits; g.rows_per_split = (((M + splits - 1) / splits) + 31) / 32 * 32; g.accumulate = accumulate; g.alpha = alpha;
    static std::atomic<unsigned long long> attr_done8{0};
    if (int e = mmb_allow_lds((const void*)gemm_tn8_kernel, 131072, attr_done8)) return e;
    auto kern = gemm_tn8_kernel;
    const int cus_ = device_cus();
    const int tiles_short = tiles_all - tiles_long;
    if (splits == 1 && (tiles_long > cus_ || tiles_short > 0)) {
        const int step_ = g_tn_one_launch.load() ? (tiles_long > 0 ? tiles_long : 1) : cus_;
        for (int base = 0; base < tiles_long; base += step_) {
            const int n = tiles_long - base < step_ ? tiles_long - base : step_;
            const bool last = base + step_ >= tiles_long;
            g.tile_base = base; g.remap_n = n;
            hipLaunchKernelGGL(kern, dim3(n + (last ? tiles_short : 0), 1), dim3(512), 131072, stream, g);
            MMB_CHECK_LAUNCH();
        }
    } else {
        g.tile_base = 0; g.remap_n = tiles_long;
        hipLaunchKernelGGL(kern, dim3(tiles_long, splits), dim3(512), 131072, stream, g);
    }
    MMB_CHECK_LAUNCH();
    if (splits > 1) {
        r.nprob = nprob; r.splits = splits; r.accumulate = accumulate; r.slab_stride = off;
        const long long total4 = off / 4;
        const int blocks = (int)((total4 + 255) / 256 < 4096 ? (total4 + 255) / 256 : 4096);
        hipLaunchKernelGGL(tn_reduce_kernel, dim3(blocks), dim3(256), 0, stream, r, (const float*)slab);
        MMB_CHECK_LAUNCH();
    }
    return 0;
}

int mmbert_gemm_tn_grouped(hipStream_t stream, int nprob, const void* const* A, const int* lda, const void* const* B, const int* ldb,
                           float* const* W, float* const* bias, const int* N, const int* K, int M,
                           int accumulate, float alpha, const float* alpha_dev, void* slab) {
    if (nprob <= 0 || M <= 0) return 0;
    if (nprob > TN_MAXP) return -1;
    int Ms[TN_MAXP];
    for (int i = 0; i < nprob; ++i) Ms[i] = M;
    return mmbert_gemm_tn_grouped_rows(stream, nprob, A, lda, B, ldb, W, bias, N, K, Ms, accumulate, nullptr, alpha, alpha_dev, slab);
}

int mmbert_gemm_tn(hipStream_t stream, const void* A, int lda, const void* B, int ldb, float* W, int ldw,
                   int M, int N, int K, int accumulate, float alpha, const float* alpha_dev, void* slab, float* bias_out) {
    if (ldw != K) return -1;
    return mmbert_gemm_tn_grouped(stream, 1, &A, &lda, &B, &ldb, &W, &bias_out, &N, &K, M, accumulate, alpha, alpha_dev, slab);
}

int mmbert_colsum(hipStream_t stream, const void* X, int ldx, int M, int N, float* out, float alpha, const float* alpha_dev) {
    if (M <= 0 || N <= 0) return 0;
    if ((N & 7) || (ldx & 7)) return -1;
    const int gx = (N / 8 + 63) / 64;
    int gy = (2048 + gx - 1) / gx;
    int rows = (M + gy - 1) / gy; if (rows < 32) rows = 32;
    if (mmb_deterministic()) rows = M;
    gy = (M + rows - 1) / rows;
    hipLaunchKernelGGL(colsum_kernel, dim3(gx, gy), dim3(256), 0, stream, (const bf16_t*)X, M, N, ldx, out, alpha, alpha_dev, rows);
    MMB_CHECK_LAUNCH();
    return 0;
}

}
```

### msa_amd/csrc/layer.hip

```cpp
#include <hip/hip_runtime.h>
#include "../../include/mmbert_hip.h"

extern "C" {

int mmbert_layer_struct_sizes(int* out) {
    if (!out) return -1;
    out[0] = (int)sizeof(mmbert_attn_layout); out[1] = (int)sizeof(mmbert_layer_fwd_args); out[2] = (int)sizeof(mmbert_layer_bwd_args);
    return 0;
}

#define MMB_TRY(call) do { const int e_ = (call); if (e_) return e_; } while (0)

int mmbert_layer_fwd(mmbert_stream_t s, const mmbert_attn_layout* L, const mmbert_layer_fwd_args* a) {
    if (!L || !a || a->rows <= 0) return a && a->rows == 0 ? 0 : -1;
    const int M = a->rows, H = a->H, I = a->I;
    MMB_TRY(mmbert_gemm_nt(s, a->x, a->ldx, a->Wqkv, H, a->qkv, 3 * H, M, 3 * H, H, MMBERT_EPI_BIAS, a->bqkv, nullptr, 0, nullptr, 0, nullptr, 0,
                           1.0f, nullptr, 0, 0, 1.0f, a->tile_queue));
    MMB_TRY(mmbert_attn_fwd(s, a->qkv, a->actx, a->lse, L->key_bias, L->bias_start, H, L->heads, L->seq_start, L->seq_len, L->elem_base,
                            L->ftile_seq, L->ftile_r0, L->nftiles, a->att.stream, a->att.thr16, a->att.scale, L->kv_len, L->ftile_qshift, L->ftile_qend));
    MMB_TRY(mmbert_gemm_nt(s, a->actx, H, a->Wo, H, a->z1, H, M, H, H, MMBERT_EPI_BIAS | MMBERT_EPI_RESID, a->bo, a->x, a->ldx, nullptr, 0, nullptr, 0,
                           1.0f, nullptr, a->h1.stream, a->h1.thr16, a->h1.scale, a->tile_queue));
    MMB_TRY(mmbert_ln_fwd(s, a->z1, H, nullptr, a->y1, H, nullptr, M, H, a->ln1_g, a->ln1_b, a->ln_eps, a->m1, a->r1, 0, 0, 1.0f, 0));
    MMB_TRY(mmbert_gemm_nt(s, a->y1, H, a->W1, H, a->g, I, M, I, H, MMBERT_EPI_BIAS | MMBERT_EPI_GELU, a->b1, nullptr, 0, a->u, a->u ? I : 0, nullptr, 0,
                           1.0f, nullptr, 0, 0, 1.0f, a->tile_queue));
    MMB_TRY(mmbert_gemm_nt(s, a->g, I, a->W2, I, a->z2, H, M, H, I, MMBERT_EPI_BIAS | MMBERT_EPI_RESID, a->b2, a->y1, H, nullptr, 0, nullptr, 0,
                           1.0f, nullptr, a->h2.stream, a->h2.thr16, a->h2.scale, a->tile_queue));
    MMB_TRY(mmbert_ln_fwd(s, a->z2, H, nullptr, a->y2, a->ldy2, a->y2_rows, M, H, a->ln2_g, a->ln2_b, a->ln_eps, a->m2, a->r2, 0, 0, 1.0f, 0));
    return 0;
}

int mmbert_layer_bwd(mmbert_stream_t s, const mmbert_attn_layout* L, const mmbert_layer_bwd_args* a) {
    if (!L || !a || a->rows <= 0) return a && a->rows == 0 ? 0 : -1;
    const int M = a->rows, H = a->H, I = a->I;
    MMB_TRY(mmbert_ln_bwd(s, a->dy, a->lddy, a->dy_rows, a->z2, H, nullptr, a->m2, a->r2, a->ln2_g, M, H, a->dz2, H, nullptr, a->dz2d, a->dz2d ? H : 0,
                          a->g_ln2_g, a->g_ln2_b, nullptr, 0, 0, 1.0f, a->h2.stream, a->dz2d ? a->h2.thr16 : 0, a->h2.scale, a->ln2_ws, nullptr, 1, 0));
    const void* dz2d = a->dz2d ? a->dz2d : a->dz2;
    MMB_TRY(mmbert_gemm_nt(s, dz2d, H, a->W2T, H, a->du, I, M, I, H, MMBERT_EPI_GELU_BWD, nullptr, nullptr, 0, nullptr, 0, a->u, I,
                           1.0f, nullptr, 0, 0, 1.0f, a->tile_queue));
    MMB_TRY(mmbert_gemm_nt(s, a->du, I, a->W1T, I, a->dy1, H, M, H, I, MMBERT_EPI_RESID, nullptr, a->dz2, H, nullptr, 0, nullptr, 0,
                           1.0f, nullptr, 0, 0, 1.0f, a->tile_queue));
    MMB_TRY(mmbert_ln_bwd(s, a->dy1, H, nullptr, a->z1, H, nullptr, a->m1, a->r1, a->ln1_g, M, H, a->dz1, H, nullptr, a->dz1d, a->dz1d ? H : 0,
                          a->g_ln1_g, a->g_ln1_b, nullptr, 0, 0, 1.0f, a->h1.stream, a->dz1d ? a->h1.thr16 : 0, a->h1.scale, a->ln1_ws, nullptr, 1, 0));
    const void* dz1d = a->dz1d ? a->dz1d : a->dz1;
    MMB_TRY(mmbert_gemm_nt(s, dz1d, H, a->WoT, H, a->dctx, H, M, H, H, 0, nullptr, nullptr, 0, nullptr, 0, nullptr, 0,
                           1.0f, nullptr, 0, 0, 1.0f, a->tile_queue));
    MMB_TRY(mmbert_attn_bwd(s, a->qkv, a->actx, a->dctx, a->dqkv, a->lse, a->delta, L->key_bias, L->bias_start, H, L->heads, L->seq_start, L->seq_len,
                            L->elem_base, L->qtile_seq, L->qtile_r0, L->nqtiles, L->tile_seq, L->tile_r0, L->ntiles,
                            a->att.stream, a->att.thr16, a->att.scale, L->kv_len, L->qtile_qshift, L->qtile_qend, L->split, nullptr));
    MMB_TRY(mmbert_gemm_nt(s, a->dqkv, 3 * H, a->WqkvT, 3 * H, a->dx, H, M, H, 3 * H, MMBERT_EPI_RESID, nullptr, a->dz1, H, nullptr, 0, nullptr, 0,
                           1.0f, nullptr, 0, 0, 1.0f, a->tile_queue));
    return 0;
}

}
```

### msa_amd/model.py

```python
from __future__ import annotations

import json
import os
from typing import Optional

import contextlib

import torch
import torch.nn as nn
import torch.nn.functional as F

from . import ops
from .flat import FlatParams

MODALITY_DIMS = {"mosi": (47, 74), "mosei": (35, 74), "ur_funny": (371, 81)}
LN_EPS_JOINT = 1e-5
MASK_NEG = -10000.0


class MMBertConfig:

    def __init__(self, vocab_size=30522, hidden_size=768, num_hidden_layers=12, num_attention_heads=12,
                 intermediate_size=3072, max_position_embeddings=512, type_vocab_size=2,
                 hidden_dropout_prob=0.1, attention_probs_dropout_prob=0.1, layer_norm_eps=1e-12,
                 initializer_range=0.02, pad_token_id=0, hidden_act="gelu", is_decoder=False, **unused):
        self.vocab_size, self.hidden_size = vocab_size, hidden_size
        self.num_hidden_layers, self.num_attention_heads = num_hidden_layers, num_attention_heads
        self.intermediate_size, self.max_position_embeddings = intermediate_size, max_position_embeddings
        self.type_vocab_size = type_vocab_size
        self.hidden_dropout_prob, self.attention_probs_dropout_prob = hidden_dropout_prob, attention_probs_dropout_prob
        self.layer_norm_eps, self.initializer_range = layer_norm_eps, initializer_range
        self.pad_token_id, self.hidden_act, self.is_decoder = pad_token_id, hidden_act, is_decoder
        self.output_attentions = False
        self.output_hidden_states = False


class _Box(nn.Module):
    pass


def _make_bert_holder(cfg) -> nn.Module:
    H, I = cfg.hidden_size, cfg.intermediate_size
    bert = _Box()
    emb = _Box()
    emb.word_embeddings = nn.Embedding(cfg.vocab_size, H, padding_idx=cfg.pad_token_id)
    emb.position_embeddings = nn.Embedding(cfg.max_position_embeddings, H)
    emb.token_type_embeddings = nn.Embedding(cfg.type_vocab_size, H)
    emb.LayerNorm = nn.LayerNorm(H, eps=cfg.layer_norm_eps)
    bert.embeddings = emb
    enc = _Box()
    layers = []
    for _ in range(cfg.num_hidden_layers):
        lay = _Box()
        att = _Box()
        att.self = _Box()
        att.self.query, att.self.key, att.self.value = nn.Linear(H, H), nn.Linear(H, H), nn.Linear(H, H)
        att.output = _Box()
        att.output.dense = nn.Linear(H, H)
        att.output.LayerNorm = nn.LayerNorm(H, eps=cfg.layer_norm_eps)
        lay.attention = att
        lay.intermediate = _Box()
        lay.intermediate.dense = nn.Linear(H, I)
        lay.output = _Box()
        lay.output.dense = nn.Linear(I, H)
        lay.output.LayerNorm = nn.LayerNorm(H, eps=cfg.layer_norm_eps)
        layers.append(lay)
    enc.layer = nn.ModuleList(layers)
    bert.encoder = enc
    bert.pooler = _Box()
    bert.pooler.dense = nn.Linear(H, H)
    return bert


def _hf_init(module: nn.Module, std: float, skip: Optional[nn.Module] = None):
    skipped = set(id(x) for x in skip.modules()) if skip is not None else ()
    for m in module.modules():
        if id(m) in skipped:
            continue
        if isinstance(m, nn.Linear):
            nn.init.normal_(m.weight, mean=0.0, std=std)
            if m.bias is not None:
                nn.init.zeros_(m.bias)
        elif isinstance(m, nn.Embedding):
            nn.init.normal_(m.weight, mean=0.0, std=std)
            if m.padding_idx is not None:
                with torch.no_grad():
                    m.weight[m.padding_idx].zero_()
        elif isinstance(m, nn.LayerNorm):
            nn.init.ones_(m.weight)
            nn.init.zeros_(m.bias)


class CPC(nn.Module):

    def __init__(self, x_size, y_size, n_layers=1, activation="Tanh"):
        super().__init__()
        if n_layers != 1:
            raise NotImplementedError("the reference builds a projection for n_layers == 1 only (REF:MMBertEmbedding.py:15-19)")
        self.x_size, self.y_size, self.layers = x_size, y_size, n_layers
        self.activation = getattr(nn, activation)
        self.net = nn.Linear(y_size, x_size)

    def forward(self, x, y):
        unit = lambda t: t / torch.linalg.vector_norm(t, dim=1, keepdim=True)
        sim = unit(x) @ unit(self.net(y)).t()
        return (torch.logsumexp(sim, dim=1) - torch.diagonal(sim)).mean()


class JointEmbeddings(nn.Module):

    def __init__(self, hidden_size, dropout_prob, dataset):
        super().__init__()
        if dataset not in MODALITY_DIMS:
            raise KeyError(dataset)
        self.VISUALDIM, self.SPEECHDIM = MODALITY_DIMS[dataset]
        H = hidden_size
        self.W_cv = nn.Linear(self.VISUALDIM + H, H)
        self.W_cs = nn.Linear(self.SPEECHDIM + H, H)
        self.Wv = nn.Linear(self.VISUALDIM, H)
        self.Ws = nn.Linear(self.SPEECHDIM, H)
        self.LayerNorm = nn.LayerNorm(H)
        self.dropout_prob = dropout_prob
        self.dropout = nn.Dropout(dropout_prob)
        self._owner = None

    def which(self, pair_ids) -> str:
        d = pair_ids.size()[-1]
        if d == self.VISUALDIM:
            return "Wv"
        if d == self.SPEECHDIM:
            return "Ws"
        raise Exception("Wrong Dimension")

    def forward(self, input_embs, pair_ids):
        assert input_embs is not None, "You miss input_embs"
        assert pair_ids is not None, "You miss pair_ids"
        if self._owner is None:
            raise RuntimeError("JointEmbeddings must be attached with MMBertModel.set_joint_embeddings()")
        top = self._owner()
        top._ensure_ready(input_embs.device)
        B, T, H = input_embs.shape
        e1 = input_embs.reshape(B * T, H).to(torch.bfloat16)
        drop = ops.make_drop(self.dropout_prob if self.training else 0.0, top._next_seed(), 1001)
        out = _JointFn.apply(e1, self.LayerNorm.weight, top, (_pair_features(pair_ids, e1.device),), (self.which(pair_ids),), B, T, drop)
        return out.view(B, -1, H).float()


class _JointFn(torch.autograd.Function):

    @staticmethod
    def forward(ctx, e1, anchor, top, feats, whichs, B, T, drop):
        w = top._w
        H = e1.shape[1]
        S = T + sum(f.shape[1] for f in feats)
        j0 = torch.empty((B * S, H), device=e1.device, dtype=torch.bfloat16)
        j0.view(B, S, H)[:, :T].copy_(e1.view(B, T, H))
        off = T
        for feat, which in zip(feats, whichs):
            ops.pair_proj_fwd(feat, w[which + "_w"], w[which + "_b"], j0, T, seq_len=S, offset=off)
            off += feat.shape[1]
        x, mean, rstd = ops.ln_fwd(j0, w["joint_ln_g"], w["joint_ln_b"], LN_EPS_JOINT, drop=drop)
        ctx.top, ctx.whichs, ctx.B, ctx.T, ctx.drop, ctx.nf = top, whichs, B, T, drop, len(feats)
        ctx.save_for_backward(j0, mean, rstd, *feats)
        return x

    @staticmethod
    def backward(ctx, dx):
        j0, mean, rstd, *feats = ctx.saved_tensors
        w, B, T = ctx.top._w, ctx.B, ctx.T
        H = j0.shape[1]
        S = j0.shape[0] // B
        dj0 = ops.ln_bwd(dx.contiguous(), j0, mean, rstd, w["joint_ln_g"], w["g_joint_ln_g"], w["g_joint_ln_b"], post_drop=ctx.drop)
        off = T
        for feat, which in zip(feats, ctx.whichs):
            ops.pair_proj_bwd(feat, j0, dj0, T, w["g_" + which + "_w"], w["g_" + which + "_b"], seq_len=S, offset=off)
            off += feat.shape[1]
        de1 = dj0.view(B, -1, H)[:, :T].reshape(B * T, H)
        return de1, None, None, None, None, None, None, None


def _pair_features(f, dev):
    f = f.to(dev)
    if f.dtype not in (torch.float32, torch.float64):
        f = f.float()
    return f.contiguous()


def _check_unchanged(feats, versions):
    for f, v in zip(feats, versions):
        if f._version != v:
            raise RuntimeError("a pair-feature tensor needed for gradient computation has been modified by an inplace operation "
                               "between forward and backward (the projection's weight gradient reads the caller's tensor)")


_cu_count = {}
_defer_fits = {}
_DEFER_ENV = os.environ.get("MMBERT_DEFER_WGRADS")


def _auto_defer_wgrads(H, I, L, x_dev, rows=None) -> bool:
    key = str(x_dev)
    cus = _cu_count.get(key)
    if cus is None:
        cus = _cu_count[key] = int(torch.cuda.get_device_properties(x_dev).multi_processor_count)
    c = lambda n: (n + 255) // 256
    t = 2 * c(I) * c(H) + c(3 * H) * c(H) + c(H) * c(H)
    if not (L > 2 and (L - 1) * t >= cus):
        return False
    if rows is None or ops.deterministic():
        return True
    fk = (key, H, I, L, -(-int(rows) // 2048))
    ent = _defer_fits.get(fk)
    if ent is None or ent[1] <= 0:
        need = L * (fk[4] * 2048) * (2 * I + 8 * H) * 2
        free, _total = torch.cuda.mem_get_info(x_dev)
        cached = torch.cuda.memory_reserved(x_dev) - torch.cuda.memory_allocated(x_dev)
        ent = _defer_fits[fk] = [need <= 0.5 * (free + cached), 256]
    ent[1] -= 1
    return ent[0]


def _wgrad(top, probs):
    f = top._flat
    if not f.stale:
        ops.gemm_tn_grouped(probs, accumulate=True)
    else:
        ops.gemm_tn_grouped(probs, accumulate=[f.take_accumulate([q[2]]) for q in probs])


def _late_wgrad(top, prob, defer: bool):
    if defer:
        pend = _late_pending(top)
        if any(q[2] is prob[2] for q in pend):
            _flush_late_wgrads(top)
            pend = []
        if not pend:
            top.__dict__["_late_wgrads"] = (torch._C._current_graph_task_id(), pend)
        pend.append(prob)
    else:
        _wgrad(top, [prob])


def _late_pending(top):
    pend = top.__dict__.get("_late_wgrads")
    return pend[1] if pend is not None and pend[0] == torch._C._current_graph_task_id() else []


def _take_late_wgrads(top):
    late = _late_pending(top)
    top.__dict__.pop("_late_wgrads", None)
    return late


def _flush_late_wgrads(top, long_probs=(), deferred=False):
    late = _take_late_wgrads(top)
    long_probs = list(long_probs)
    if not deferred or not long_probs:
        for c in range(0, len(long_probs), 48):
            _wgrad(top, long_probs[c:c + 48])
        for q in late:
            _wgrad(top, [q])
        return
    chunks = [long_probs[c:c + 48] for c in range(0, len(long_probs), 48)]
    if late and len(chunks[-1]) + len(late) <= ops.TN_MAX_PROBLEMS:
        chunks[-1] = chunks[-1] + late
        late = []
    side = getattr(top, "wgrad_side_stream", True) and long_probs[0][0].is_cuda
    if side:
        _join_wgrads(top)
        s = ops.side_stream("wgrads", long_probs[0][0].device)
        s.wait_stream(torch.cuda.current_stream())
        with torch.cuda.stream(s):
            for c in chunks:
                _wgrad(top, c)
            for q in late:
                _wgrad(top, [q])
            top.__dict__["_wgrad_join"] = (s.record_event(), chunks, late)
        return
    for c in chunks:
        _wgrad(top, c)
    for q in late:
        _wgrad(top, [q])


def _join_heads(top):
    j = top.__dict__.pop("_heads_join", None)
    if j:
        torch.cuda.current_stream().wait_event(j[-1][0])


def _join_wgrads(top):
    j = top.__dict__.pop("_wgrad_join", None)
    if j is not None:
        torch.cuda.current_stream().wait_event(j[0])


class _EncoderFn:

    @staticmethod
    def run_forward(top, x, layout, key_bias, seed, kv_len, keep, y_out=None, y_rows=None, stop=None, train=None, probe=None):
        cfg = top.config
        H, L = cfg.hidden_size, cfg.num_hidden_layers
        nl = L if stop is None else stop
        train = top.training if train is None else train
        ph = cfg.hidden_dropout_prob if train else 0.0
        pa = cfg.attention_probs_dropout_prob if train else 0.0
        saved = []
        composite = getattr(top, "composite_layers", True) and ops.launches_unwrapped() and top.debug_hidden is None
        if composite:
            AL = ops.attn_layout_struct(key_bias, layout, backward=False)
            if kv_len is not None and not getattr(layout, "split", False):
                AL.kv_len = kv_len.data_ptr()
            I_, M_, dev = cfg.intermediate_size, x.shape[0], x.device
            heads = layout.heads
            bf, f32 = torch.bfloat16, torch.float32
            tq = ops._tile_queue(dev)
            for i in range(nl):
                lw = top._lw[i]
                d_att, d_h1, d_h2 = (ops.make_drop(pa, seed, 8 * i), ops.make_drop(ph, seed, 8 * i + 1), ops.make_drop(ph, seed, 8 * i + 2))
                last = i == L - 1 and y_out is not None
                qkv, actx, z1, y1 = (torch.empty((M_, 3 * H), device=dev, dtype=bf), torch.empty((M_, H), device=dev, dtype=bf),
                                     torch.empty((M_, H), device=dev, dtype=bf), torch.empty((M_, H), device=dev, dtype=bf))
                g, z2 = torch.empty((M_, I_), device=dev, dtype=bf), torch.empty((M_, H), device=dev, dtype=bf)
                lse = torch.empty((M_, heads), device=dev, dtype=f32)
                u = torch.empty((M_, I_), device=dev, dtype=bf) if keep else None
                if keep:
                    m1, r1, m2, r2 = (torch.empty(M_, device=dev, dtype=f32) for _ in range(4))
                else:
                    m1 = r1 = m2 = r2 = None
                y2 = y_out if last else torch.empty((M_, H), device=dev, dtype=bf)
                a = lw.get("_fwd_args")
                if a is None:
                    a = lw["_fwd_args"] = ops._LayerFwd()
                    for n in ("Wqkv", "Wo", "W1", "W2", "bqkv", "bo", "b1", "b2", "ln1_g", "ln1_b", "ln2_g", "ln2_b"):
                        assert lw[n].is_contiguous()
                        setattr(a, n, lw[n].data_ptr())
                    a.H, a.I, a.ln_eps = H, I_, cfg.layer_norm_eps
                a.x, a.ldx, a.rows = x.data_ptr(), x.stride(0), M_
                a.qkv, a.actx, a.lse, a.z1, a.y1, a.g, a.z2 = qkv.data_ptr(), actx.data_ptr(), lse.data_ptr(), z1.data_ptr(), y1.data_ptr(), g.data_ptr(), z2.data_ptr()
                a.u, a.m1, a.r1, a.m2, a.r2 = ops._ptr(u), ops._ptr(m1), ops._ptr(r1), ops._ptr(m2), ops._ptr(r2)
                a.y2, a.ldy2, a.y2_rows = y2.data_ptr(), y2.stride(0), ops._ptr(y_rows) if last else None
                a.tile_queue = tq
                ops._set_drop(a.att, d_att); ops._set_drop(a.h1, d_h1); ops._set_drop(a.h2, d_h2)
                ops.layer_fwd(AL, a)
                if probe is not None:
                    probe(i, qkv)
                if keep:
                    saved.append((x, qkv, actx, lse, z1, m1, r1, y1, u, g, z2, m2, r2, d_att, d_h1, d_h2))
                x = y2
            return x, saved
        for i in range(nl):
            lw = top._lw[i]
            d_att, d_h1, d_h2 = (ops.make_drop(pa, seed, 8 * i), ops.make_drop(ph, seed, 8 * i + 1), ops.make_drop(ph, seed, 8 * i + 2))
            qkv = ops.gemm_nt(x, lw["Wqkv"], bias=lw["bqkv"])
            actx, lse = ops.attn_fwd(qkv, key_bias, layout, H, drop=d_att, kv_len=kv_len)
            if probe is not None:
                probe(i, qkv)
            z1 = ops.gemm_nt(actx, lw["Wo"], bias=lw["bo"], resid=x, drop=d_h1)
            y1, m1, r1 = ops.ln_fwd(z1, lw["ln1_g"], lw["ln1_b"], cfg.layer_norm_eps, stats=keep)
            u = torch.empty((x.shape[0], cfg.intermediate_size), device=x.device, dtype=torch.bfloat16) if keep else None
            g = ops.gemm_nt(y1, lw["W1"], bias=lw["b1"], gelu=True, aux=u)
            z2 = ops.gemm_nt(g, lw["W2"], bias=lw["b2"], resid=y1, drop=d_h2)
            last = i == L - 1 and y_out is not None
            y2, m2, r2 = ops.ln_fwd(z2, lw["ln2_g"], lw["ln2_b"], cfg.layer_norm_eps, stats=keep,
                                    out=y_out if last else None, out_rows=y_rows if last else None)
            if keep:
                saved.append((x, qkv, actx, lse, z1, m1, r1, y1, u, g, z2, m2, r2, d_att, d_h1, d_h2))
            x = y2
            if top.debug_hidden is not None:
                top.debug_hidden.setdefault("_layers_packed", []).append(None if last else y2.detach())
        return x, saved

    @staticmethod
    def run_top_first(top, x, layout, key_bias, kv_len, q_rows, probe=None):
        cfg = top.config
        H = cfg.hidden_size
        lw = top._lw[cfg.num_hidden_layers - 1]
        qkv = ops.gemm_nt(x, lw["Wqkv"], bias=lw["bqkv"])
        actx = ops.attn_fwd_first(qkv, key_bias, layout, H, q_rows, kv_len=kv_len)
        if probe is not None:
            probe(cfg.num_hidden_layers - 1, qkv)
        del qkv
        xr = ops.gather_rows([x], q_rows)[0]
        z1 = ops.gemm_nt(actx, lw["Wo"], bias=lw["bo"], resid=xr)
        y1, _, _ = ops.ln_fwd(z1, lw["ln1_g"], lw["ln1_b"], cfg.layer_norm_eps, stats=False)
        g = ops.gemm_nt(y1, lw["W1"], bias=lw["b1"], gelu=True)
        z2 = ops.gemm_nt(g, lw["W2"], bias=lw["b2"], resid=y1)
        y2, _, _ = ops.ln_fwd(z2, lw["ln2_g"], lw["ln2_b"], cfg.layer_norm_eps, stats=False)
        return y2

    @staticmethod
    def run_backward(top, layout, key_bias, kv_len, saved, dy, dy_rows, top_rows, compact=None, lnd=None):
        H = top.config.hidden_size
        L = top.config.num_hidden_layers
        top._flat.grads_dirty = True
        top._flat.attach_lazy()
        top._flat.wait_transposes()
        _join_wgrads(top)
        _join_heads(top)
        M_all = saved[0][0].shape[0]
        ra = layout.rows_a if getattr(layout, "split", False) else M_all
        if dy is not None and dy_rows is None and ra < dy.shape[0]:
            dy = dy[:ra]
        own_lnd = lnd is None
        if own_lnd:
            lnd = ops.LnDeferred(2 * L)
        pair_wgrads, held = getattr(top, "pair_wgrads", True), None
        dw = getattr(top, "defer_wgrads", None)
        if dw is None and _DEFER_ENV:
            dw = _DEFER_ENV != "0"
        if dw is None:
            dw = _auto_defer_wgrads(H, top.config.intermediate_size, L, x_dev=saved[0][0].device, rows=ra)
        defer_wgrads, deferred = (top.grad_hook is None and bool(dw)), []
        composite_bwd = getattr(top, "composite_layers", True) and ops.launches_unwrapped()
        AL = tq = None
        for i in reversed(range(L)):
            lw = top._lw[i]
            saved_i = saved[i]
            saved[i] = None
            if ra < M_all:
                saved_i = tuple(t[:ra] if torch.is_tensor(t) else t for t in saved_i)
            x, qkv, actx, lse, z1, m1, r1, y1, u, g, z2, m2, r2, d_att, d_h1, d_h2 = saved_i
            if i == L - 1 and (top_rows is not None or compact is not None):
                R = None
                R32 = None
                if compact is not None:
                    rows_l, rows_f, dy_c = compact
                    rinv = top.__dict__.get("_row_inverse")
                    if rinv is None or rinv.table.numel() < M_all or rinv.table.device != rows_f.device:
                        rinv = top.__dict__["_row_inverse"] = ops.RowInverse(M_all, rows_f.device)
                    R, R32 = ops.compact_rows(rows_l, rows_f, layout.inv if getattr(layout, "split", False) else None, inverse=rinv)
                elif top_rows is not None:
                    Ro = _EncoderFn._sparse_rows(top_rows, None, ra)
                    if Ro is not None:
                        R = layout.inv.index_select(0, Ro) if getattr(layout, "split", False) else Ro
                        src_rows = Ro if dy_rows is not None else R
                        (dy_c,) = ops.gather_rows([dy], src_rows.int())
                if R is not None:
                    dy = _EncoderFn._last_layer_sparse(top, lw, layout, key_bias, kv_len, saved_i, dy_c, R, H, ra, R32, lnd,
                                                       rinv if compact is not None else None, deferred if defer_wgrads else None)
                    if top.grad_hook is not None:
                        lnd.flush()
                    dy_rows = None
                    top._layer_grads_done(i)
                    continue
                if compact is not None:
                    raise RuntimeError("compact output gradient without the sparse top-layer path")
            if composite_bwd:
                dev, bf = z2.device, torch.bfloat16
                I_ = top.config.intermediate_size
                if AL is None:
                    AL = ops.attn_layout_struct(key_bias, layout, backward=True)
                    if kv_len is not None and not getattr(layout, "split", False):
                        AL.kv_len = kv_len.data_ptr()
                    tq = ops._tile_queue(dev)
                dz2, dz1, dy1, dctx, dx_ = (torch.empty((ra, H), device=dev, dtype=bf) for _ in range(5))
                dz2d = torch.empty((ra, H), device=dev, dtype=bf) if d_h2[1] else None
                dz1d = torch.empty((ra, H), device=dev, dtype=bf) if d_h1[1] else None
                du, dqkv = torch.empty((ra, I_), device=dev, dtype=bf), torch.empty((ra, 3 * H), device=dev, dtype=bf)
                delta = torch.empty((ra, layout.heads), device=dev, dtype=torch.float32)
                lnd.reserve(2, ra, H, dev)
                ws2 = lnd.slot(ra, H, dev, lw["g_ln2_g"], lw["g_ln2_b"], None)
                ws1 = lnd.slot(ra, H, dev, lw["g_ln1_g"], lw["g_ln1_b"], None)
                b = lw.get("_bwd_args")
                if b is None:
                    b = lw["_bwd_args"] = ops._LayerBwd()
                    for n in ("W2T", "W1T", "WoT", "WqkvT", "ln2_g", "ln1_g", "g_ln2_g", "g_ln2_b", "g_ln1_g", "g_ln1_b"):
                        assert lw[n].is_contiguous()
                        setattr(b, n, lw[n].data_ptr())
                    b.H, b.I = H, I_
                b.dy, b.lddy, b.dy_rows, b.rows = dy.data_ptr(), dy.stride(0), ops._ptr(dy_rows), ra
                b.z2, b.m2, b.r2, b.ln2_ws, b.z1, b.m1, b.r1, b.ln1_ws = z2.data_ptr(), m2.data_ptr(), r2.data_ptr(), ws2, z1.data_ptr(), m1.data_ptr(), r1.data_ptr(), ws1
                b.u, b.qkv, b.actx, b.lse = u.data_ptr(), qkv.data_ptr(), actx.data_ptr(), lse.data_ptr()
                b.dz2, b.dz2d, b.du, b.dy1, b.dz1, b.dz1d = dz2.data_ptr(), ops._ptr(dz2d), du.data_ptr(), dy1.data_ptr(), dz1.data_ptr(), ops._ptr(dz1d)
                b.dctx, b.dqkv, b.delta, b.dx, b.tile_queue = dctx.data_ptr(), dqkv.data_ptr(), delta.data_ptr(), dx_.data_ptr(), tq
                ops._set_drop(b.att, d_att); ops._set_drop(b.h1, d_h1); ops._set_drop(b.h2, d_h2)
                ops.layer_bwd(AL, b)
                dy_rows = None
                dy = dx_
                if dz2d is None:
                    dz2d = dz2
                if dz1d is None:
                    dz1d = dz1
            else:
              dz2d = torch.empty((ra, H), device=z2.device, dtype=torch.bfloat16) if d_h2[1] else None
              dz2 = ops.ln_bwd(dy, z2, m2, r2, lw["ln2_g"], lw["g_ln2_g"], lw["g_ln2_b"], dx2=dz2d, pre_drop=d_h2, deferred=lnd, dy_rows=dy_rows)
              dy_rows = None
              if dz2d is None:
                  dz2d = dz2
              du = ops.gemm_nt(dz2d, lw["W2T"], gelu_bwd_u=u)
              dy1 = ops.gemm_nt(du, lw["W1T"], resid=dz2)
              dz1d = torch.empty((ra, H), device=z2.device, dtype=torch.bfloat16) if d_h1[1] else None
              dz1 = ops.ln_bwd(dy1, z1, m1, r1, lw["ln1_g"], lw["g_ln1_g"], lw["g_ln1_b"], dx2=dz1d, pre_drop=d_h1, deferred=lnd)
              if dz1d is None:
                  dz1d = dz1
              dctx = ops.gemm_nt(dz1d, lw["WoT"])
              dqkv = ops.attn_bwd(qkv, actx, dctx, lse, key_bias, layout, H, drop=d_att, kv_len=kv_len)
              dy = ops.gemm_nt(dqkv, lw["WqkvT"], resid=dz1)
            probs = [(du, y1, lw["g_W1"], lw["g_b1"]), (dz2d, g, lw["g_W2"], lw["g_b2"]),
                     (dqkv, x, lw["g_Wqkv"], lw["g_bqkv"]), (dz1d, actx, lw["g_Wo"], lw["g_bo"])]
            if defer_wgrads:
                deferred.extend(probs)
                top._layer_grads_done(i)
                continue
            if pair_wgrads:
                if held is None and i > 0:
                    held = (i, probs)
                    continue
                if held is not None:
                    _wgrad(top, held[1] + probs)
                    if top.grad_hook is not None:
                        lnd.flush()
                    top._layer_grads_done(held[0])
                    held = None
                else:
                    _wgrad(top, probs)
            else:
                _wgrad(top, probs)
            if top.grad_hook is not None:
                lnd.flush()
            top._layer_grads_done(i)
        if own_lnd:
            lnd.flush()
        _flush_late_wgrads(top, deferred, deferred=defer_wgrads)
        return dy

    @staticmethod
    def _sparse_rows(top_rows, layout, ra):
        (idx, host, ev), first = top_rows
        n = _active_row_count(top_rows[0])
        r = n + first.numel()
        if 4 * r > ra or int(host[1]) != 0:
            return None
        R = torch.cat((idx[:n].long(), first))
        if layout is not None and getattr(layout, "split", False):
            R = layout.inv.index_select(0, R)
        return R

    @staticmethod
    def _last_layer_sparse(top, lw, layout, key_bias, kv_len, saved_i, dy_c, R, H, ra, R32=None, lnd=None, rinv=None, deferred=None):
        cfg = top.config
        x, qkv, actx, lse, z1, m1, r1, y1, u, g, z2, m2, r2, d_att, d_h1, d_h2 = saved_i
        if R32 is None:
            R32 = R.int()
        m2_c, r2_c, u_c, m1_c, r1_c, y1_c, g_c, actx_c = ops.gather_rows([m2, r2, u, m1, r1, y1, g, actx], R32)
        dy = dy_c
        dz2d_c = torch.empty_like(dy_c) if d_h2[1] else None
        dz2_c = ops.ln_bwd(dy_c, z2, m2_c, r2_c, lw["ln2_g"], lw["g_ln2_g"], lw["g_ln2_b"], x_rows=R32, dx2=dz2d_c, pre_drop=d_h2,
                           drop_rows=R32, deferred=lnd)
        if dz2d_c is None:
            dz2d_c = dz2_c
        du_c = ops.gemm_nt(dz2d_c, lw["W2T"], gelu_bwd_u=u_c)
        dy1_c = ops.gemm_nt_splitk(du_c, lw["W1T"], resid=dz2_c) if du_c.shape[0] <= 1024 else ops.gemm_nt(du_c, lw["W1T"], resid=dz2_c)
        dz1d_c = torch.empty_like(dy_c) if d_h1[1] else None
        dz1_c = ops.ln_bwd(dy1_c, z1, m1_c, r1_c, lw["ln1_g"], lw["g_ln1_g"], lw["g_ln1_b"], x_rows=R32, dx2=dz1d_c, pre_drop=d_h1,
                           drop_rows=R32, deferred=lnd)
        if dz1d_c is None:
            dz1d_c = dz1_c
        dctx_c = ops.gemm_nt(dz1d_c, lw["WoT"])
        if rinv is not None:
            dctx, dz1 = ops.scatter_rows_zero([dctx_c, dz1_c], rinv, ra)
        else:
            dctx = torch.zeros((ra, H), device=dy.device, dtype=torch.bfloat16)
            dctx.index_copy_(0, R, dctx_c)
        qlim = ops.attn_q_limit(R32, layout) if getattr(top, "top_layer_query_limit", True) else None
        dqkv = ops.attn_bwd(qkv, actx, dctx, lse, key_bias, layout, H, drop=d_att, kv_len=kv_len, q_limit=qlim)
        if rinv is None:
            dz1 = torch.zeros((ra, H), device=dy.device, dtype=torch.bfloat16)
            dz1.index_copy_(0, R, dz1_c)
        out = ops.gemm_nt(dqkv, lw["WqkvT"], resid=dz1)
        few = [(du_c, y1_c, lw["g_W1"], lw["g_b1"]), (dz2d_c, g_c, lw["g_W2"], lw["g_b2"]), (dz1d_c, actx_c, lw["g_Wo"], lw["g_bo"])]
        if deferred is not None and getattr(top, "late_wgrads", True):
            deferred.append((dqkv, x, lw["g_Wqkv"], lw["g_bqkv"]))
            for q in few:
                _late_wgrad(top, q, True)
        else:
            _wgrad(top, few)
            _wgrad(top, [(dqkv, x, lw["g_Wqkv"], lw["g_bqkv"])])
        return out


def _trunk_static(plan, B, T, lens, joff, dev):
    key = ("trunk_static", T, tuple(sorted(joff.items())))
    st = plan.get(key)
    if st is None:
        jrows = {}
        for k, lo in joff.items():
            b = torch.arange(B, dtype=torch.int32)[:, None] * lens[k] + torch.arange(T, dtype=torch.int32)[None, :] + lo
            jrows[k] = b.reshape(-1).to(dev)
        groups, k = [], 0
        while k < len(lens):
            k1 = k
            while k1 + 1 < len(lens) and ((k1 + 1) in joff) == (k in joff):
                k1 += 1
            groups.append((k in joff, k, k1 + 1, torch.cat([jrows[q] for q in range(k, k1 + 1)]) if k in joff else None))
            k = k1 + 1
        st = plan[key] = dict(jrows=jrows, groups=groups, arange=torch.arange(len(lens) * B * T, dtype=torch.int32, device=dev))
    return st


class _Trunk:
    __slots__ = ("ids", "tts", "B", "T", "lens", "pair_info", "feats", "feat_versions", "plan", "layout", "split", "key_bias", "kv_len", "seed", "top_rows",
                 "d_emb", "d_joint", "infer", "late_split", "compact", "J_pre", "predict", "attention", "dense")


class _TrunkFn(torch.autograd.Function):

    @staticmethod
    def forward(ctx, anchor, top, t):
        cfg, w = top.config, top._w
        H = cfg.hidden_size
        B, T, lens, plan, split = t.B, t.T, t.lens, t.plan, t.split
        bounds, tokens = plan["bounds"], plan["layout"].tokens
        dev = t.ids.device
        keep = ctx.needs_input_grad[0] and not t.predict
        late = t.layout
        npass = len(lens)
        joint = [k for k in range(npass) if t.pair_info[k] is not None]
        joff, jtot = {}, 0
        for k in joint:
            joff[k] = jtot
            jtot += B * lens[k]
        early = split is not None and not t.late_split and not t.infer
        dropped = split is not None and getattr(split, "dropped", False)
        Mx = split.rows_packed if early else tokens
        pad = 1 if (early and dropped) else 0
        pre = t.J_pre
        t.J_pre = None
        if pre is not None and pre[0].shape[0] == jtot:
            buf = torch.empty((Mx + pad, H), device=dev, dtype=torch.bfloat16)
            X, J = buf[:Mx], pre[0]
        else:
            pre = None
            buf = torch.empty((Mx + pad + jtot, H), device=dev, dtype=torch.bfloat16)
            X, J = buf[:Mx], buf[Mx + pad:]
        st = _trunk_static(plan, B, T, lens, joff, dev)
        e0 = ops.embed_gather(t.ids, t.tts, w["word"], w["type"], w["pos"], T)
        mean0 = torch.empty(npass * B * T, device=dev, dtype=torch.float32)
        rstd0 = torch.empty_like(mean0)
        for is_joint, k0, k1, jr in st["groups"]:
            rows = slice(k0 * B * T, k1 * B * T)
            if is_joint:
                out, orows = J, jr
            elif early:
                out, orows = X, split.inv32[bounds[k0]:bounds[k1]]
            else:
                out, orows = X[bounds[k0]:bounds[k1]], None
            ops.ln_fwd(e0[rows], w["emb_ln_g"], w["emb_ln_b"], cfg.layer_norm_eps, out=out, out_rows=orows, drop=t.d_emb, drop_row0=k0 * B * T,
                       stats=(mean0[rows], rstd0[rows]))
        jstats = {}
        for n, k in enumerate(joint):
            S = lens[k]
            Jk = J[joff[k]:joff[k] + B * S]
            off = T
            if pre is not None:
                torch.cuda.current_stream().wait_event(pre[1][n])
            else:
# ... 1457 lines not shown
```

### msa_amd/ops.py

```python
from __future__ import annotations

import ctypes
import os
from typing import Optional, Tuple

import numpy as np
import torch

from . import _lib

EPI_BIAS, EPI_GELU, EPI_RESID, EPI_GELU_BWD, EPI_OUT_F32 = 1, 2, 4, 8, 16

SIDE_TRANSPOSES = True
SIDE_STREAM_PRIORITY = "low"
_side_streams = {}


def side_stream(tag: str, device) -> "torch.cuda.Stream":
    key = (tag, str(device), SIDE_STREAM_PRIORITY)
    s = _side_streams.get(key)
    if s is None:
        prio = 0
        if SIDE_STREAM_PRIORITY == "low":
            try:
                prio = max(torch.cuda.Stream.priority_range())
            except Exception:
                prio = 0
        s = _side_streams[key] = torch.cuda.Stream(device=device, priority=prio)
    return s

Drop = Optional[Tuple[int, int, float]]
NO_DROP = (0, 0, 1.0)


_raw_stream = getattr(torch._C, "_cuda_getCurrentRawStream", None)
_raw_device = getattr(torch._C, "_cuda_getDevice", None)


def _stream() -> int:
    if _raw_stream is not None and _raw_device is not None:
        return _raw_stream(_raw_device())
    return torch.cuda.current_stream().cuda_stream


def _ptr(t: Optional[torch.Tensor]) -> Optional[int]:
    return None if t is None else t.data_ptr()


_rng_fn = None


def rng_stream(seed: int, site: int) -> int:
    global _rng_fn
    if _rng_fn is None:
        _rng_fn = _lib.load().mmbert_rng_stream
    return _rng_fn(seed & 0xFFFFFFFFFFFFFFFF, site & 0xFFFFFFFF)


_thr_cache = {}


def make_drop(p: float, seed: int, site: int) -> Tuple[int, int, float]:
    if p <= 0.0:
        return NO_DROP
    t = _thr_cache.get(p)
    if t is None:
        thr = _lib.load().mmbert_dropout_thr16(p)
        t = _thr_cache[p] = (thr, 1.0 / (1.0 - thr / 65536.0))
    return (rng_stream(seed, site), t[0], t[1])


_tile_queues = {}
dynamic_tile_queue = bool(int(__import__("os").environ.get("MMBERT_NT_DYNAMIC", "0")))


def _tile_queue(device) -> Optional[int]:
    if not dynamic_tile_queue:
        return None
    key = (device, _stream())
    q = _tile_queues.get(key)
    if q is None:
        q = _tile_queues[key] = torch.zeros(16, device=device, dtype=torch.int32)
    return q.data_ptr()


def gemm_nt(A, B, *, out=None, bias=None, gelu=False, aux=None, resid=None, gelu_bwd_u=None, alpha=1.0,
            alpha_dev=None, drop: Drop = None, out_f32=False):
    lib = _lib.load()
    M, K = A.shape
    N = B.shape[0]
    assert B.shape[1] == K and A.stride(1) == 1 and B.stride(1) == 1
    if out is None:
        out = torch.empty((M, N), device=A.device, dtype=torch.float32 if out_f32 else torch.bfloat16)
    epi = 0
    if bias is not None:
        epi |= EPI_BIAS
    if gelu:
        epi |= EPI_GELU
    if resid is not None:
        epi |= EPI_RESID
    if gelu_bwd_u is not None:
        epi |= EPI_GELU_BWD
    if out_f32:
        epi |= EPI_OUT_F32
    d = drop or NO_DROP
    _lib.check(lib.mmbert_gemm_nt(_stream(), A.data_ptr(), A.stride(0), B.data_ptr(), B.stride(0), out.data_ptr(), out.stride(0),
                                  M, N, K, epi, _ptr(bias), _ptr(resid), resid.stride(0) if resid is not None else 0,
                                  _ptr(aux), aux.stride(0) if aux is not None else 0,
                                  _ptr(gelu_bwd_u), gelu_bwd_u.stride(0) if gelu_bwd_u is not None else 0,
                                  float(alpha), _ptr(alpha_dev), d[0], d[1], d[2], _tile_queue(A.device)), "mmbert_gemm_nt")
    return out


def gemm_nt_describe(M: int, N: int, K: int, epi: int = 0, with_queue: bool = False) -> dict:
    import ctypes
    out = (ctypes.c_int * 8)()
    _lib.check(_lib.load().mmbert_gemm_nt_describe(int(M), int(N), int(K), int(epi), int(bool(with_queue)), out), "mmbert_gemm_nt_describe")
    kern = {0: "128x128", 1: "ring", 2: "persistent", 3: "8phase"}[out[0]]
    return dict(kernel=kern, tile=f"{out[1]}x{out[2]}", tiles=out[3], workgroups=out[4], rounds=out[5] / 100.0, group_m=out[6], cus=out[7])


_slab_cache = {}


def _slab(nbytes: int, device) -> Optional[torch.Tensor]:
    if nbytes == 0:
        return None
    key = (device, _stream())
    t = _slab_cache.get(key)
    if t is None or t.numel() < nbytes:
        t = torch.empty(nbytes, device=device, dtype=torch.uint8)
        _slab_cache[key] = t
    return t


_ws_cache = {}


def _ws_f32(nfloats: int, device) -> torch.Tensor:
    key = (device, _stream())
    t = _ws_cache.get(key)
    if t is None or t.numel() < nfloats:
        t = torch.empty(max(nfloats, 1), device=device, dtype=torch.float32)
        _ws_cache[key] = t
    return t


def gemm_nt_splitk(A, B, out=None, resid=None):
    lib = _lib.load()
    M, K = A.shape
    N = B.shape[0]
    if out is None:
        out = torch.empty((M, N), device=A.device, dtype=torch.bfloat16)
    if resid is not None:
        assert resid.shape == (M, N) and resid.dtype == torch.bfloat16 and resid.stride(1) == 1
    ws = _ws_f32((lib.mmbert_gemm_nt_splitk_workspace(M, N, K) + 3) // 4, A.device)
    _lib.check(lib.mmbert_gemm_nt_splitk(_stream(), A.data_ptr(), A.stride(0), B.data_ptr(), B.stride(0), out.data_ptr(), out.stride(0),
                                         M, N, K, ws.data_ptr(), _ptr(resid), 0 if resid is None else resid.stride(0)), "mmbert_gemm_nt_splitk")
    return out


def gemm_tn(A, B, W, *, accumulate=True, alpha=1.0, alpha_dev=None, bias_out=None):
    lib = _lib.load()
    M, N = A.shape
    K = B.shape[1]
    assert B.shape[0] == M and W.shape == (N, K) and W.dtype == torch.float32 and W.is_contiguous()
    need = lib.mmbert_gemm_tn_workspace(M, N, K, None)
    slab = _slab(need, A.device)
    _lib.check(lib.mmbert_gemm_tn(_stream(), A.data_ptr(), A.stride(0), B.data_ptr(), B.stride(0), W.data_ptr(), W.stride(0),
                                  M, N, K, 1 if accumulate else 0, float(alpha), _ptr(alpha_dev), _ptr(slab), _ptr(bias_out)), "mmbert_gemm_tn")
    return W


TN_MAX_PROBLEMS = 52
_PtrArr = {n: (ctypes.c_void_p * n) for n in range(1, TN_MAX_PROBLEMS + 1)}
_IntArr = {n: (ctypes.c_int * n) for n in range(1, TN_MAX_PROBLEMS + 1)}


def gemm_tn_grouped(problems, *, accumulate=True, alpha=1.0):
    lib = _lib.load()
    n = len(problems)
    each = None
    if isinstance(accumulate, (list, tuple)):
        each = [1 if a else 0 for a in accumulate]
        accumulate = all(each)
        if accumulate or not any(each):
            each = None
    rows = [p[0].shape[0] for p in problems]
    if any(rows[i] < rows[i + 1] for i in range(n - 1)):
        order = sorted(range(n), key=lambda i: -rows[i])
        problems = [problems[i] for i in order]
        rows = [rows[i] for i in order]
        if each is not None:
            each = [each[i] for i in order]
    M = rows[0]
    PA, IA = _PtrArr[n], _IntArr[n]
    Ns = IA(*[p[0].shape[1] for p in problems])
    Ks = IA(*[p[1].shape[1] for p in problems])
    mixed = rows[-1] != M
    slab = None
    if not mixed:
        need = lib.mmbert_gemm_tn_grouped_workspace(n, Ns, Ks, M, None)
        slab = _slab(need, problems[0][0].device)
    _lib.check(lib.mmbert_gemm_tn_grouped_rows(
        _stream(), n, PA(*[p[0].data_ptr() for p in problems]), IA(*[p[0].stride(0) for p in problems]),
        PA(*[p[1].data_ptr() for p in problems]), IA(*[p[1].stride(0) for p in problems]),
        PA(*[p[2].data_ptr() for p in problems]), PA(*[(p[3].data_ptr() if p[3] is not None else None) for p in problems]),
        Ns, Ks, IA(*rows), 1 if accumulate else 0, IA(*each) if each is not None else None, float(alpha), None, _ptr(slab)), "mmbert_gemm_tn_grouped_rows")


def colsum(X, out, *, alpha=1.0, alpha_dev=None):
    lib = _lib.load()
    M, N = X.shape
    _lib.check(lib.mmbert_colsum(_stream(), X.data_ptr(), X.stride(0), M, N, out.data_ptr(), float(alpha), _ptr(alpha_dev)), "mmbert_colsum")
    return out


def dropout_mask(n: int, drop: Tuple[int, int, float], device) -> torch.Tensor:
    lib = _lib.load()
    out = torch.empty(n, device=device, dtype=torch.uint8)
    _lib.check(lib.mmbert_dropout_mask(_stream(), out.data_ptr(), n, drop[0], drop[1]), "mmbert_dropout_mask")
    return out


def mlm_mask(ids, p_select: float, seed: int, *, special_ids=(101, 102), mask_id=103, p_replace=0.8, site=4242):
    assert ids.dtype == torch.int64 and ids.is_contiguous() and len(special_ids) <= 3
    sp = list(special_ids) + [special_ids[0] if special_ids else -1] * (3 - len(special_ids))
    labels = torch.empty_like(ids)
    _lib.check(_lib.load().mmbert_mlm_mask(_stream(), ids.data_ptr(), labels.data_ptr(), ids.numel(), rng_stream(seed, site),
                                           int(round(p_select * 65536)), int(round(p_replace * 65536)), sp[0], sp[1], sp[2], mask_id), "mmbert_mlm_mask")
    return labels


def ln_fwd(x, gamma, beta, eps, *, M=None, out=None, in_rows=None, out_rows=None, drop: Drop = None, stats=True, drop_row0=0):
    lib = _lib.load()
    H = x.shape[1]
    if M is None:
        M = in_rows.numel() if in_rows is not None else x.shape[0]
    if out is None:
        out = torch.empty((M, H), device=x.device, dtype=torch.bfloat16)
    if isinstance(stats, tuple):
        mean, rstd = stats
        assert mean.numel() == M and rstd.numel() == M and mean.dtype == torch.float32 and mean.is_contiguous() and rstd.is_contiguous()
    else:
        mean = torch.empty(M, device=x.device, dtype=torch.float32) if stats else None
        rstd = torch.empty(M, device=x.device, dtype=torch.float32) if stats else None
    d = drop or NO_DROP
    _lib.check(lib.mmbert_ln_fwd(_stream(), x.data_ptr(), x.stride(0), _ptr(in_rows), out.data_ptr(), out.stride(0), _ptr(out_rows),
                                 M, H, gamma.data_ptr(), beta.data_ptr(), float(eps), _ptr(mean), _ptr(rstd), d[0], d[1], d[2], int(drop_row0)), "mmbert_ln_fwd")
    return out, mean, rstd


def ln_bwd(dy, x, mean, rstd, gamma, dgamma, dbeta, *, M=None, dx=None, dx2=None, dy_rows=None, x_rows=None, dx_rows=None,
           post_drop: Drop = None, pre_drop: Drop = None, dbias2=None, drop_rows=None, deferred: "LnDeferred" = None, dy_row_limit=0):
    lib = _lib.load()
    H = x.shape[1]
    if M is None:
        M = mean.numel()
    if dx is None:
        dx = torch.empty((M, H), device=x.device, dtype=torch.bfloat16)
    po, pr = post_drop or NO_DROP, pre_drop or NO_DROP
    if deferred is not None:
        ws_ptr = deferred.slot(M, H, x.device, dgamma, dbeta, dbias2)
    else:
        ws_ptr = _ws_f32(lib.mmbert_ln_bwd_workspace(M, H), x.device).data_ptr()
    _lib.check(lib.mmbert_ln_bwd(_stream(), dy.data_ptr(), dy.stride(0), _ptr(dy_rows), x.data_ptr(), x.stride(0), _ptr(x_rows),
                                 mean.data_ptr(), rstd.data_ptr(), gamma.data_ptr(), M, H,
                                 dx.data_ptr(), dx.stride(0), _ptr(dx_rows), _ptr(dx2), dx2.stride(0) if dx2 is not None else 0,
                                 _ptr(dgamma), _ptr(dbeta), _ptr(dbias2), po[0], po[1], po[2], pr[0], pr[1], pr[2], ws_ptr, _ptr(drop_rows),
                                 1 if deferred is not None else 0, int(dy_row_limit)), "mmbert_ln_bwd")
    return dx


_lnd_cache = {}


class LnDeferred:

    def __init__(self, slots: int = 32):
        self.items, self.H, self.ws, self.used = [], None, None, 0
        self.slots = max(1, min(32, int(slots)))

    def slot(self, M, H, device, dgamma, dbeta, dbias2) -> int:
        if self.H is not None and (H != self.H or len(self.items) == self.slots):
            self.flush()
        self.H = H
        per = _lib.load().mmbert_ln_bwd_workspace(M, H)
        ck = (device, _stream())
        if not self.items:
            self.ws, self.used = _lnd_cache.get(ck), 0
        if self.ws is None or self.ws.numel() < self.used + per:
            self.flush()
            self.H = H
            want = max(self.slots * per, 2 * (self.ws.numel() if self.ws is not None else 0))
            self.ws, self.used = torch.empty(want, device=device, dtype=torch.float32), 0
            _lnd_cache[ck] = self.ws
        ptr = self.ws.data_ptr() + 4 * self.used
        self.used += per
        self.items.append((ptr, dgamma.data_ptr(), dbeta.data_ptr(), dbias2.data_ptr() if dbias2 is not None else None, int(M)))
        return ptr

    def reserve(self, n, M, H, device):
        per = _lib.load().mmbert_ln_bwd_workspace(M, H)
        self.slots = min(32, max(self.slots, int(n)))
        assert n <= self.slots, "LnDeferred.reserve: at most 32 slots per reduce launch"
        if self.H is not None and (H != self.H or len(self.items) + n > self.slots):
            self.flush()
        ck = (device, _stream())
        if not self.items:
            self.ws, self.used = _lnd_cache.get(ck), 0
        if self.ws is None or self.ws.numel() < self.used + n * per:
            self.flush()
            want = max(max(self.slots, n) * per, 2 * (self.ws.numel() if self.ws is not None else 0))
            self.ws, self.used = torch.empty(want, device=device, dtype=torch.float32), 0
            _lnd_cache[ck] = self.ws

    def drop(self):
        self.items, self.H, self.used = [], None, 0

    def flush(self):
        n = len(self.items)
        if n:
            PA = ctypes.c_void_p * n
            cols = list(zip(*self.items))
            Ms = (ctypes.c_int * n)(*cols[4])
            _lib.check(_lib.load().mmbert_ln_bwd_reduce_rows(_stream(), n, PA(*cols[0]), PA(*cols[1]), PA(*cols[2]), PA(*cols[3]), Ms, self.H),
                       "mmbert_ln_bwd_reduce_rows")
        self.items, self.H, self.used = [], None, 0


def embed_gather(ids, tts, word, type_, pos, T, out=None):
    lib = _lib.load()
    n = ids.numel()
    V, H = word.shape
    if out is None:
        out = torch.empty((n, H), device=word.device, dtype=torch.bfloat16)
    _lib.check(lib.mmbert_embed_gather(_stream(), ids.data_ptr(), _ptr(tts), word.data_ptr(), type_.data_ptr(), pos.data_ptr(),
                                       n, T, H, V, out.data_ptr(), out.stride(0)), "mmbert_embed_gather")
    return out


def set_deterministic(on: bool) -> None:
    _lib.load().mmbert_set_deterministic(1 if on else 0)


def deterministic() -> bool:
    return bool(_lib.load().mmbert_get_deterministic())


if os.environ.get("MMBERT_DETERMINISTIC", "0") not in ("", "0"):
    set_deterministic(True)


def scatter_add_rows_ordered(keys, src, dst, vocab, union=None):
    keys = keys.reshape(-1).long().contiguous()
    fn, bf = _lib.load().mmbert_id_runs_sum_rows, 1 if src.dtype == torch.bfloat16 else 0
    for off in range(0, keys.numel(), 8192):
        n = min(8192, keys.numel() - off)
        _lib.check(fn(_stream(), src[off:off + n].data_ptr(), bf, src.stride(0), keys[off:off + n].data_ptr(), n, src.shape[1], int(vocab),
                      _ptr(union), 0 if union is None else union.numel(), dst.data_ptr(), dst.stride(0)), "mmbert_id_runs_sum_rows")
    return dst


def rows_to_block(ids, rows, union, vocab, block):
    ids = ids.reshape(-1).long().contiguous()
    union = union.long().contiguous()
    if deterministic():
        if union.numel():
            scatter_add_rows_ordered(ids, rows, block, vocab, union=union)
        return block
    _lib.check(_lib.load().mmbert_rows_to_block(_stream(), ids.data_ptr(), rows.data_ptr(), 1 if rows.dtype == torch.bfloat16 else 0, rows.stride(0),
                                                ids.numel(), rows.shape[1], union.data_ptr(), union.numel(), int(vocab), block.data_ptr()),
               "mmbert_rows_to_block")
    return block


def embed_scatter(ids, tts, d, T, gword, gtype, gpos, vocab=None):
    lib = _lib.load()
    n = ids.numel()
    V, H = gword.shape if gword is not None else (int(vocab), d.shape[1])
    slab = None
    if deterministic():
        slab = _ws_f32(2 * T * H, d.device)
        if gword is not None:
            scatter_add_rows_ordered(ids, d, gword, V)
            gword = None
    _lib.check(lib.mmbert_embed_scatter(_stream(), ids.data_ptr(), _ptr(tts), d.data_ptr(), d.stride(0), n, T, H, V,
                                        _ptr(gword), gtype.data_ptr(), gpos.data_ptr(), _ptr(slab)), "mmbert_embed_scatter")


def _pair_rows(T, Pn, ld, seq_len, offset):
    if seq_len is None:
        return T, 0
    Tp = seq_len - Pn
    return Tp, (offset - Tp) * ld * 2


def pair_proj_fwd(feat, W, bias, out, T, *, seq_len=None, offset=None):
    lib = _lib.load()
    B, Pn, D = feat.shape
    assert feat.dtype in (torch.float32, torch.float64) and feat.is_contiguous()
    H = W.shape[0]
    Tp, shift = _pair_rows(T, Pn, out.stride(0), seq_len, offset)
    _lib.check(lib.mmbert_pair_proj_fwd(_stream(), feat.data_ptr(), 1 if feat.dtype == torch.float64 else 0, B, Pn, D, W.data_ptr(), bias.data_ptr(), H,
                                        out.data_ptr() + shift, out.stride(0), Tp), "mmbert_pair_proj_fwd")


def pair_proj_bwd(feat, J, dJ, T, dW, db, *, seq_len=None, offset=None):
    lib = _lib.load()
    B, Pn, D = feat.shape
    H = dW.shape[0]
    assert J.stride(0) == dJ.stride(0) and feat.dtype in (torch.float32, torch.float64) and feat.is_contiguous()
    Tp, shift = _pair_rows(T, Pn, J.stride(0), seq_len, offset)
    ws = _ws_f32((lib.mmbert_pair_proj_bwd_workspace(B, Pn, D, H) + 3) // 4, feat.device)
    _lib.check(lib.mmbert_pair_proj_bwd(_stream(), feat.data_ptr(), 1 if feat.dtype == torch.float64 else 0, B, Pn, D, J.data_ptr() + shift, dJ.data_ptr() + shift, J.stride(0), Tp,
                                        dW.data_ptr(), db.data_ptr(), H, ws.data_ptr()), "mmbert_pair_proj_bwd")


NO_KEY = -1.0e30


class SeqLayout:
# ... 479 lines not shown

def cast_f32_bf16(x, y):
    _lib.check(_lib.load().mmbert_cast_f32_bf16(_stream(), x.data_ptr(), y.data_ptr(), x.numel()), "mmbert_cast_f32_bf16")
    return y


def cast_bf16_f32(x, y):
    _lib.check(_lib.load().mmbert_cast_bf16_f32(_stream(), x.data_ptr(), y.data_ptr(), x.numel()), "mmbert_cast_bf16_f32")
    return y


def transpose_cast(src_flat, dst_flat, descs_dev, ndesc, total_tiles):
    fn = "mmbert_transpose_cast" if src_flat.dtype == torch.float32 else "mmbert_transpose_bf16"
    assert src_flat.dtype in (torch.float32, torch.bfloat16)
    _lib.check(getattr(_lib.load(), fn)(_stream(), src_flat.data_ptr(), dst_flat.data_ptr(), descs_dev.data_ptr(), ndesc, total_tiles), fn)


def _ptr3(ts):
    return _PtrArr[3](*[t.data_ptr() for t in ts])


def heads_gate_fwd(P, Apre, vws, vbs, B):
    H = P.shape[1]
    g = torch.empty(3 * B, device=P.device, dtype=torch.float32)
    Cc = torch.empty((B, 3 * H), device=P.device, dtype=torch.float32)
    _lib.check(_lib.load().mmbert_heads_gate_fwd(_stream(), P.data_ptr(), Apre.data_ptr(), _ptr3(vws), _ptr3(vbs), B, H, g.data_ptr(), Cc.data_ptr()),
               "mmbert_heads_gate_fwd")
    return g, Cc


def heads_loss_fwd(P, XP, rel, ap, lo, sent, B, beta, tanh_lo, mlm=None, alpha=1.0):
    H = P.shape[1]
    n = 3 * B * H
    seeds = torch.empty(2 * n + 5 * B, device=P.device, dtype=torch.float32)
    out4 = torch.empty(5, device=P.device, dtype=torch.float32)
    if mlm is not None:
        assert mlm.dtype == torch.float32 and mlm.is_contiguous()
    part = torch.empty(3, device=P.device, dtype=torch.float32)
    loss = torch.empty((), device=P.device, dtype=torch.float32)
    aux = torch.empty(3, device=P.device, dtype=torch.float32)
    base = seeds.data_ptr()
    _lib.check(_lib.load().mmbert_heads_loss_fwd(_stream(), P.data_ptr(), XP.data_ptr(), rel.data_ptr(), ap.data_ptr(), lo.data_ptr(), sent.data_ptr(),
                                                 B, H, float(beta), int(tanh_lo), out4.data_ptr(), base, base + 4 * n, base + 4 * (2 * n + B), base + 4 * 2 * n,
                                                 part.data_ptr(), _ptr(mlm), 0 if mlm is None else mlm.numel(), float(alpha),
                                                 loss.data_ptr(), aux.data_ptr()), "mmbert_heads_loss_fwd")
    return out4, seeds, loss, aux


def heads_scale(x, s):
    _lib.check(_lib.load().mmbert_heads_scale(_stream(), x.data_ptr(), x.numel(), s.data_ptr()), "mmbert_heads_scale")


def heads_seed(seeds, d, nzero, nmlm, coef):
    buf = torch.empty(seeds.numel() + nzero + nmlm, device=seeds.device, dtype=torch.float32)
    n = seeds.numel()
    base = buf.data_ptr()
    _lib.check(_lib.load().mmbert_heads_seed(_stream(), seeds.data_ptr(), n, d.data_ptr(), base, base + 4 * n, nzero, base + 4 * (n + nzero), nmlm, float(coef)),
               "mmbert_heads_seed")
    return buf[:n], buf[n:n + nzero], (buf[n + nzero:] if nmlm else None)


def heads_gate_bwd(dC, P, Apre, g, vws, dPc, B):
    H = P.shape[1]
    dP, dA, E = torch.empty_like(P), torch.empty_like(P), torch.empty_like(P)
    dg = torch.empty(3 * B, device=P.device, dtype=torch.float32)
    _lib.check(_lib.load().mmbert_heads_gate_bwd(_stream(), dC.data_ptr(), P.data_ptr(), Apre.data_ptr(), g.data_ptr(), _ptr3(vws), dPc.data_ptr(), B, H,
                                                 dP.data_ptr(), dA.data_ptr(), E.data_ptr(), dg.data_ptr()), "mmbert_heads_gate_bwd")
    return dP, dA, E, dg


def heads_tanh_(x):
    _lib.check(_lib.load().mmbert_heads_tanh(_stream(), x.data_ptr(), x.numel()), "mmbert_heads_tanh")
    return x


def heads_tanh_bwd(dP, P):
    dpre = torch.empty_like(P)
    _lib.check(_lib.load().mmbert_heads_tanh_bwd(_stream(), dP.data_ptr(), P.data_ptr(), dpre.data_ptr(), P.numel()), "mmbert_heads_tanh_bwd")
    return dpre


class RowInverse:

    def __init__(self, nrows, device):
        self.table = torch.zeros(nrows, device=device, dtype=torch.int64)
        self.stamp, self.nlist = 0, 0

    def next(self, nlist):
        self.stamp = self.stamp % 0xFFFFFFF0 + 1
        self.nlist = nlist
        return self.stamp


def compact_rows(rows, extra, row_map=None, inverse: "RowInverse" = None):
    n, ne = rows.numel(), extra.numel()
    out64 = torch.empty(n + ne, device=extra.device, dtype=torch.int64)
    out32 = torch.empty(n + ne, device=extra.device, dtype=torch.int32)
    assert rows.dtype in (torch.int32, torch.int64) and extra.dtype == torch.int64 and rows.is_contiguous() and extra.is_contiguous()
    assert row_map is None or (row_map.dtype == torch.int64 and row_map.is_contiguous())
    r32, r64 = (rows.data_ptr(), None) if rows.dtype == torch.int32 else (None, rows.data_ptr())
    if inverse is None:
        _lib.check(_lib.load().mmbert_compact_rows(_stream(), r32, r64, n, extra.data_ptr(), ne, _ptr(row_map), out64.data_ptr(), out32.data_ptr()), "mmbert_compact_rows")
    else:
        _lib.check(_lib.load().mmbert_compact_rows_inv(_stream(), r32, r64, n, extra.data_ptr(), ne, _ptr(row_map), out64.data_ptr(), out32.data_ptr(),
                                                       inverse.table.data_ptr(), inverse.next(n + ne)), "mmbert_compact_rows_inv")
    return out64, out32


def scatter_rows_zero(srcs, inverse: "RowInverse", nrows):
    n = len(srcs)
    assert 0 < n <= 4 and nrows <= inverse.table.numel() and inverse.stamp != 0
    outs = [torch.empty((nrows, t.shape[1]), device=t.device, dtype=t.dtype) for t in srcs]
    if nrows == 0:
        return outs
    for t in srcs:
        assert t.dim() == 2 and t.stride(1) == 1 and t.shape[0] == inverse.nlist
    LA = ctypes.c_longlong * n
    rb = [t.shape[1] * t.element_size() for t in srcs]
    _lib.check(_lib.load().mmbert_scatter_rows_zero(_stream(), n, _PtrArr[n](*[t.data_ptr() for t in srcs]), _PtrArr[n](*[o.data_ptr() for o in outs]),
                                                    LA(*[t.stride(0) * t.element_size() for t in srcs]), LA(*rb), _IntArr[n](*rb),
                                                    inverse.table.data_ptr(), inverse.stamp, inverse.nlist, nrows), "mmbert_scatter_rows_zero")
    return outs


def gather_rows(srcs, idx32):
    n = len(srcs)
    assert 0 < n <= 12 and idx32.dtype == torch.int32 and idx32.is_contiguous()
    rows = idx32.numel()
    outs = [torch.empty((rows,) + tuple(t.shape[1:]), device=t.device, dtype=t.dtype) for t in srcs]
    if rows == 0:
        return outs
    for t in srcs:
        assert t.dim() in (1, 2) and (t.dim() == 1 or t.stride(1) == 1)
    LA = ctypes.c_longlong * n
    rb = [(t.shape[1] if t.dim() == 2 else 1) * t.element_size() for t in srcs]
    _lib.check(_lib.load().mmbert_gather_rows(_stream(), n, _PtrArr[n](*[t.data_ptr() for t in srcs]), _PtrArr[n](*[o.data_ptr() for o in outs]),
                                              LA(*[t.stride(0) * t.element_size() for t in srcs]), LA(*[b for b in rb]),
                                              _IntArr[n](*rb), idx32.data_ptr(), rows), "mmbert_gather_rows")
    return outs


def pack_i64(segments, total=None):
    LA = ctypes.c_longlong * len(segments)
    srcs, offs, cnts, fills, keep = [], [], [], [], []
    off = 0
    dev = None
    for sg in segments:
        if torch.is_tensor(sg):
            assert sg.dtype == torch.int64 and sg.is_cuda
            t = sg.reshape(-1)
            if not t.is_contiguous():
                t = t.contiguous()
            keep.append(t)
            srcs.append(t.data_ptr()); cnts.append(t.numel()); fills.append(0)
            dev = t.device
        else:
            srcs.append(None); cnts.append(int(sg[0])); fills.append(int(sg[1]))
        offs.append(off)
        off += cnts[-1]
    out = torch.empty(off if total is None else total, device=dev, dtype=torch.int64)
    n = len(segments)
    _lib.check(_lib.load().mmbert_pack_i64(_stream(), n, _PtrArr[n](*srcs), LA(*offs), LA(*cnts), LA(*fills), out.data_ptr()), "mmbert_pack_i64")
    return out, offs


def heads_colsum(pairs):
    n = len(pairs)
    PA, IA = _PtrArr[n], _IntArr[n]
    _lib.check(_lib.load().mmbert_heads_colsum(_stream(), n, PA(*[s.data_ptr() for s, _ in pairs]), PA(*[d.data_ptr() for _, d in pairs]),
                                               IA(*[s.shape[0] for s, _ in pairs]), IA(*[s.shape[1] for s, _ in pairs]),
                                               IA(*[s.stride(0) for s, _ in pairs])), "mmbert_heads_colsum")


_VP, _VP3 = ctypes.c_void_p, ctypes.c_void_p * 3


class _HeadsStep(ctypes.Structure):
    _fields_ = ([("B", ctypes.c_int), ("H", ctypes.c_int), ("tanh_lo", ctypes.c_int), ("nmlm", ctypes.c_int), ("alpha", ctypes.c_float), ("beta", ctypes.c_float),
                 ("first", _VP), ("y", _VP), ("first_rows", _VP), ("ldy", ctypes.c_int), ("ncls", ctypes.c_int), ("ap", _VP), ("ap2", _VP), ("sent", _VP), ("mlm", _VP)]
                + [(n, _VP) for n in ("Wp", "bp", "Wal", "bal", "Wsr", "bsr", "Wat", "bat")] + [("vw", _VP3), ("vb", _VP3)]
                + [(n, _VP) for n in ("Wc1", "bc1", "Wc2", "bc2")] + [("Wq", _VP3), ("bq", _VP3)]
                + [(n, _VP) for n in ("loss", "aux", "out5", "logits", "t_rel", "rel", "ws", "dloss", "dfirst", "dmlm")]
                + [(n, _VP) for n in ("gWp", "gbp", "gWal", "gbal", "gWat", "gbat")] + [("gvw", _VP3), ("gvb", _VP3)]
                + [(n, _VP) for n in ("gWc1", "gbc1", "gWc2", "gbc2")] + [("gWq", _VP3), ("gbq", _VP3)] + [("sync", _VP), ("sent_cls", _VP), ("pred", _VP)])


_heads_sync = {}
_heads_struct_checked = False


def heads_step_struct() -> "_HeadsStep":
    global _heads_struct_checked
    if not _heads_struct_checked:
        n = _lib.load().mmbert_heads_step_struct_size()
        if n != ctypes.sizeof(_HeadsStep):
            raise RuntimeError(f"mmbert_heads_step: the library's struct has {n} bytes, the binding's {ctypes.sizeof(_HeadsStep)}")
        _heads_struct_checked = True
    return _HeadsStep()


def heads_step_sync(device) -> torch.Tensor:
    key = (device, _stream())
    t = _heads_sync.get(key)
    if t is None:
        t = _heads_sync[key] = torch.zeros(4, device=device, dtype=torch.int32)
    return t


def heads_step_workspace(B: int, H: int, device) -> torch.Tensor:
    return torch.empty(_lib.load().mmbert_heads_step_workspace(int(B), int(H)) // 4, device=device, dtype=torch.float32)


def heads_step_fwd(a: "_HeadsStep", lo: int = 1, hi: int = 7):
    _lib.check(_lib.load().mmbert_heads_step_fwd_levels(_stream(), ctypes.addressof(a), lo, hi), "mmbert_heads_step_fwd_levels")


def heads_predict(a: "_HeadsStep"):
    _lib.check(_lib.load().mmbert_heads_predict(_stream(), ctypes.addressof(a)), "mmbert_heads_predict")


def heads_step_outputs(ws: torch.Tensor, B: int, H: int):
    po, fo = ctypes.c_size_t(0), ctypes.c_size_t(0)
    _lib.check(_lib.load().mmbert_heads_step_outputs(int(B), int(H), ctypes.byref(po), ctypes.byref(fo)), "mmbert_heads_step_outputs")
    return ws[po.value:po.value + 3 * B * H].view(3, B, H), ws[fo.value:fo.value + B * H].view(B, H)


def heads_step_dmlm(a: "_HeadsStep"):
    _lib.check(_lib.load().mmbert_heads_step_dmlm(_stream(), ctypes.addressof(a)), "mmbert_heads_step_dmlm")


def heads_step_bwd(a: "_HeadsStep", lo: int = 1, hi: int = 6):
    _lib.check(_lib.load().mmbert_heads_step_bwd_levels(_stream(), ctypes.addressof(a), lo, hi), "mmbert_heads_step_bwd_levels")


class _SkSrc(ctypes.Structure):
    _fields_ = [("X", ctypes.c_void_p), ("W", ctypes.c_void_p), ("ldx", ctypes.c_int), ("ldw", ctypes.c_int), ("inner", ctypes.c_int),
                ("row0", ctypes.c_int), ("rows", ctypes.c_int), ("w_inner_major", ctypes.c_int)]


class _SkOp(ctypes.Structure):
    _fields_ = [("Y", ctypes.c_void_p), ("bias", ctypes.c_void_p), ("ldy", ctypes.c_int), ("M", ctypes.c_int), ("N", ctypes.c_int),
                ("nsrc", ctypes.c_int), ("act", ctypes.c_int), ("accumulate", ctypes.c_int), ("src", _SkSrc * 4)]


class _SkWOp(ctypes.Structure):
    _fields_ = [("dY", ctypes.c_void_p), ("X", ctypes.c_void_p), ("dW", ctypes.c_void_p), ("db", ctypes.c_void_p), ("ldy", ctypes.c_int),
                ("ldx", ctypes.c_int), ("ldw", ctypes.c_int), ("M", ctypes.c_int), ("N", ctypes.c_int), ("K", ctypes.c_int)]


def _f32_2d(t):
    assert t.dtype == torch.float32 and t.dim() == 2 and (t.shape[1] == 1 or t.stride(1) == 1) and t.is_cuda, (t.dtype, t.shape, t.stride())
    return t


def skinny_mm(oplist):
    n = len(oplist)
    arr = (_SkOp * n)()
    keep = []
    for o, (Y, bias, act, accumulate, sources) in zip(arr, oplist):
        _f32_2d(Y)
        o.Y, o.bias, o.ldy, o.M, o.N = Y.data_ptr(), _ptr(bias), Y.stride(0), Y.shape[0], Y.shape[1]
        o.nsrc, o.act, o.accumulate = len(sources), int(act), 1 if accumulate else 0
        for sc, (X, W, wim, row0) in zip(o.src, sources):
            _f32_2d(X); _f32_2d(W)
            inner = X.shape[1]
            assert (W.shape == (inner, Y.shape[1])) if wim else (W.shape == (Y.shape[1], inner)), (W.shape, inner, Y.shape, wim)
            sc.X, sc.W, sc.ldx, sc.ldw, sc.inner, sc.row0, sc.rows, sc.w_inner_major = X.data_ptr(), W.data_ptr(), X.stride(0), W.stride(0), inner, row0, X.shape[0], 1 if wim else 0
            keep.append((X, W))
    lib = _lib.load()
    if deterministic():
        ws = _ws_f32((lib.mmbert_skinny_mm_workspace(n, ctypes.cast(arr, ctypes.c_void_p)) + 3) // 4, oplist[0][0].device)
        _lib.check(lib.mmbert_skinny_mm_ordered(_stream(), n, ctypes.cast(arr, ctypes.c_void_p), ws.data_ptr()), "mmbert_skinny_mm_ordered")
        return
    _lib.check(lib.mmbert_skinny_mm(_stream(), n, ctypes.cast(arr, ctypes.c_void_p)), "mmbert_skinny_mm")


def skinny_wgrad(oplist):
    n = len(oplist)
    arr = (_SkWOp * n)()
    for o, (dY, X, dW, db) in zip(arr, oplist):
        _f32_2d(dY); _f32_2d(X); _f32_2d(dW)
        assert dY.shape[0] == X.shape[0] and dW.shape == (dY.shape[1], X.shape[1]), (dY.shape, X.shape, dW.shape)
        o.dY, o.X, o.dW, o.db = dY.data_ptr(), X.data_ptr(), dW.data_ptr(), _ptr(db)
        o.ldy, o.ldx, o.ldw, o.M, o.N, o.K = dY.stride(0), X.stride(0), dW.stride(0), dY.shape[0], dY.shape[1], X.shape[1]
    _lib.check(_lib.load().mmbert_skinny_wgrad(_stream(), n, ctypes.cast(arr, ctypes.c_void_p)), "mmbert_skinny_wgrad")


class _Drop(ctypes.Structure):
    _fields_ = [("stream", ctypes.c_uint32), ("thr16", ctypes.c_uint32), ("scale", ctypes.c_float)]


_VP, _CI = ctypes.c_void_p, ctypes.c_int


class _AttnLayout(ctypes.Structure):
    _fields_ = [(n, _VP) for n in ("key_bias", "bias_start", "seq_start", "seq_len", "elem_base", "ftile_seq", "ftile_r0", "ftile_qshift", "ftile_qend",
                                    "qtile_seq", "qtile_r0", "qtile_qshift", "qtile_qend", "tile_seq", "tile_r0", "kv_len")] + \
               [(n, _CI) for n in ("nftiles", "nqtiles", "ntiles", "split", "heads", "pad_")]


class _LayerFwd(ctypes.Structure):
    _fields_ = [(n, _VP) for n in ("x", "Wqkv", "Wo", "W1", "W2", "bqkv", "bo", "b1", "b2", "ln1_g", "ln1_b", "ln2_g", "ln2_b",
                                    "qkv", "actx", "lse", "z1", "y1", "m1", "r1", "u", "g", "z2", "y2", "m2", "r2", "y2_rows", "tile_queue")] + \
               [("att", _Drop), ("h1", _Drop), ("h2", _Drop)] + [(n, _CI) for n in ("rows", "H", "I", "ldx", "ldy2")] + [("ln_eps", ctypes.c_float)]


class _LayerBwd(ctypes.Structure):
    _fields_ = [(n, _VP) for n in ("dy", "dy_rows", "z2", "m2", "r2", "ln2_g", "g_ln2_g", "g_ln2_b", "ln2_ws", "z1", "m1", "r1", "ln1_g", "g_ln1_g", "g_ln1_b", "ln1_ws",
                                    "u", "qkv", "actx", "lse", "W2T", "W1T", "WoT", "WqkvT",
                                    "dz2", "dz2d", "du", "dy1", "dz1", "dz1d", "dctx", "dqkv", "delta", "dx", "tile_queue")] + \
               [("att", _Drop), ("h1", _Drop), ("h2", _Drop)] + [(n, _CI) for n in ("rows", "H", "I", "lddy")]


_layer_structs_checked = False


def _check_layer_structs():
    global _layer_structs_checked
    if not _layer_structs_checked:
        sz = (ctypes.c_int * 3)()
        _lib.check(_lib.load().mmbert_layer_struct_sizes(sz), "mmbert_layer_struct_sizes")
        got = (ctypes.sizeof(_AttnLayout), ctypes.sizeof(_LayerFwd), ctypes.sizeof(_LayerBwd))
        if tuple(sz) != got:
            raise RuntimeError(f"msa_amd.ops: structure layout differs from include/mmbert_hip.h: C {tuple(sz)} != ctypes {got}")
        _layer_structs_checked = True


def attn_layout_struct(key_bias, layout, backward: bool):
    _check_layer_structs()
    if key_bias.numel() != layout.bias_len or layout.bias_len == layout.tokens:
        key_bias = pad_key_bias(key_bias, layout) if key_bias.numel() == layout.tokens else key_bias
    split = bool(getattr(layout, "split", False))
    L = _AttnLayout()
    L.key_bias, L.bias_start, L.seq_start, L.seq_len, L.elem_base = (key_bias.data_ptr(), layout.bias_start.data_ptr(), layout.seq_start.data_ptr(),
                                                                     layout.seq_len.data_ptr(), layout.elem_base.data_ptr())
    L.ftile_seq, L.ftile_r0, L.nftiles = layout.ftile_seq.data_ptr(), layout.ftile_r0.data_ptr(), layout.nftiles
    L.ftile_qshift, L.ftile_qend = _ptr(getattr(layout, "ftile_qshift", None)), _ptr(getattr(layout, "ftile_qend", None))
    L.kv_len = _ptr(layout.kv_len) if split else None
    L.split, L.heads = 1 if split else 0, layout.heads
    if backward:
        if split:
            L.qtile_seq, L.qtile_r0, L.nqtiles = layout.tile_seq.data_ptr(), layout.tile_r0.data_ptr(), layout.ntiles
        else:
            L.qtile_seq, L.qtile_r0, L.nqtiles = layout.ftile_seq.data_ptr(), layout.ftile_r0.data_ptr(), layout.nftiles
        L.tile_seq, L.tile_r0, L.ntiles = layout.tile_seq.data_ptr(), layout.tile_r0.data_ptr(), layout.ntiles
        L.qtile_qshift, L.qtile_qend = _ptr(getattr(layout, "qtile_qshift", None)), _ptr(getattr(layout, "qtile_qend", None))
    L._keep = (key_bias, layout)
    return L


def _set_drop(d: _Drop, drop: Drop):
    d.stream, d.thr16, d.scale = drop or NO_DROP


def layer_fwd(L: _AttnLayout, a: _LayerFwd):
    _lib.check(_lib.load().mmbert_layer_fwd(_stream(), ctypes.addressof(L), ctypes.addressof(a)), "mmbert_layer_fwd")


def layer_bwd(L: _AttnLayout, a: _LayerBwd):
    _lib.check(_lib.load().mmbert_layer_bwd(_stream(), ctypes.addressof(L), ctypes.addressof(a)), "mmbert_layer_bwd")


_UNWRAPPED = dict(gemm_nt=gemm_nt, attn_fwd=attn_fwd, attn_fwd_first=attn_fwd_first, attn_probs_first=attn_probs_first, attn_bwd=attn_bwd, ln_fwd=ln_fwd, ln_bwd=ln_bwd)


def launches_unwrapped() -> bool:
    g = globals()
    return all(g[k] is v for k, v in _UNWRAPPED.items())
```

Measured before the change: 1255.

## Skip QKV GEMM tiles for K/V columns beyond the live key-row count

Adds a row-limited variant of the NT GEMM that reads a device-side row count and skips output tiles in the K/V column range (columns at or past H) whose rows lie beyond that count. The persistent 8-phase kernel gets a compacted tile walk over only the live tiles, with XCD grouping adjusted. The layer forward passes layout.counts as the limit when split attention with masked-key skipping is active. This removes QKV projection work for key/value rows the attention never reads, at the cost of extra indexing logic, a device-side read of the limit, and a grid that is still sized for the full tile count.

```diff
diff --git a/include/mmbert_hip.h b/include/mmbert_hip.h
--- a/include/mmbert_hip.h
+++ b/include/mmbert_hip.h
@@ -20,12 +20,20 @@
                    const void* U, int ldu, float alpha, const float* alpha_dev,
                    uint32_t drop_stream, uint32_t drop_thr16, float drop_scale, int* tile_queue);
 
+int mmbert_gemm_nt_rl(mmbert_stream_t stream, const void* A, int lda, const void* B, int ldb, void* C, int ldc,
+                      int M, int N, int K, int epi, const float* bias, const void* R, int ldr, void* aux, int ldaux,
+                      const void* U, int ldu, float alpha, const float* alpha_dev,
+                      uint32_t drop_stream, uint32_t drop_thr16, float drop_scale, int* tile_queue,
+                      const int* row_limit, int limit_col0, int rows_hint);
+
 int mmbert_gemm_nt_splitk(mmbert_stream_t stream, const void* A, int lda, const void* B, int ldb, void* C, int ldc,
                           int M, int N, int K, void* workspace, const void* R, int ldr);
 size_t mmbert_gemm_nt_splitk_workspace(int M, int N, int K);
 
 void mmbert_gemm_nt_force(int mode);
 int mmbert_gemm_nt_describe(int M, int N, int K, int epi, int with_queue, int* out);
+int mmbert_gemm_nt_describe_rl(int M, int N, int K, int epi, int with_queue, int limit_col0, int rows_hint, int* out);
+int mmbert_gemm_nt_limit_walk(int tiles_m, int tiles_n, int bm, int row_limit, int cn, int group_m, int* mn);
 void mmbert_gemm_tn_force_splits(int splits);
 void mmbert_gemm_tn_force_one_launch(int on);
 
@@ -189,6 +197,9 @@
     int* tile_queue;
     mmbert_drop att, h1, h2;
     int rows, H, I, ldx, ldy2; float ln_eps;
+    const int* kv_rows;
+    int kv_rows_hint;
+    int pad_;
 } mmbert_layer_fwd_args;
 typedef struct {
     const void* dy; const int* dy_rows;
diff --git a/msa_amd/_lib.py b/msa_amd/_lib.py
--- a/msa_amd/_lib.py
+++ b/msa_amd/_lib.py
@@ -10,6 +10,9 @@
 
 SIGNATURES = {
     "mmbert_gemm_nt": (I, [P, P, I, P, I, P, I, I, I, I, I, P, P, I, P, I, P, I, F, P, U32, U32, F, P]),
+    "mmbert_gemm_nt_rl": (I, [P, P, I, P, I, P, I, I, I, I, I, P, P, I, P, I, P, I, F, P, U32, U32, F, P, P, I, I]),
+    "mmbert_gemm_nt_describe_rl": (I, [I, I, I, I, I, I, I, P]),
+    "mmbert_gemm_nt_limit_walk": (I, [I, I, I, I, I, I, P]),
     "mmbert_gemm_nt_force": (None, [I]),
     "mmbert_gemm_nt_describe": (I, [I, I, I, I, I, P]),
     "mmbert_gemm_nt_splitk": (I, [P, P, I, P, I, P, I, I, I, I, P, P, I]),
diff --git a/msa_amd/csrc/gemm.hip b/msa_amd/csrc/gemm.hip
--- a/msa_amd/csrc/gemm.hip
+++ b/msa_amd/csrc/gemm.hip
@@ -24,7 +24,26 @@
     int* tile_counter; int* tile_counter_next;
     int queue_xcd;
     int group_m;
+    const int* row_limit; int limit_col0;
+    int group_xcd;
 };
+
+__host__ __device__ constexpr bool nt_epi_limits(int epi) { return epi == EPI_BIAS; }
+
+__host__ __device__ inline int ntl_full_panels(int row_limit, int bm, int tiles_m) {
+    const int f = (row_limit + bm - 1) / bm;
+    return f < tiles_m ? f : tiles_m;
+}
+__host__ __device__ inline int ntl_live_tiles(int tiles_m, int tiles_n, int full, int cn) { return full * tiles_n + (tiles_m - full) * cn; }
+__host__ __device__ inline void ntl_tile_mn(int t, int tiles_n, int gm, int full, int cn, int& tm, int& tn) {
+    const int F = full * tiles_n;
+    if (t >= F) { const int r = t - F, q = r / cn; tm = full + q; tn = r - q * cn; return; }
+    if (gm <= 1) { tm = t / tiles_n; tn = t - tm * tiles_n; return; }
+    const int per = gm * tiles_n, g = t / per, r = t - g * per;
+    const int rest = full - g * gm, gs = gm < rest ? gm : rest;
+    tn = r / gs;
+    tm = g * gm + (r - tn * gs);
+}
 
 __device__ __forceinline__ int xcd_remap(int bid, int nwg) {
     const int q = nwg >> 3, r = nwg & 7, x = bid & 7, j = bid >> 3;
@@ -134,6 +153,13 @@
     const int m0 = (tile / tiles_n) << 7, n0 = (tile % tiles_n) << 7;
     const int kt0 = p.kt_per_split ? (int)blockIdx.z * p.kt_per_split : 0;
     const int kt1 = p.kt_per_split ? min(p.K >> 6, kt0 + p.kt_per_split) : (p.K >> 6);
+    int mlim = p.M;
+    if constexpr (nt_epi_limits(EPI)) {
+        if (p.row_limit && n0 >= p.limit_col0) {
+            mlim = max(0, min(*p.row_limit, p.M));
+            if (m0 >= mlim) return;
+        }
+    }
 
     const int srow = lane >> 3, schunk = (lane & 7) ^ srow;
     const bf16_t* a_src[4]; const bf16_t* b_src[4];
@@ -197,7 +223,7 @@
 #pragma unroll
     for (int i = 0; i < 4; ++i) {
         const int m = m0 + wm * 64 + i * 16 + fr;
-        if (m >= p.M) continue;
+        if (m >= mlim) continue;
 #pragma unroll
         for (int j = 0; j < 4; ++j) {
             const int n = n0 + wn * 64 + j * 16 + fq * 4;
@@ -254,8 +280,24 @@
     constexpr int MQ0 = (MQ == 7) ? 4 : MQ, MQ1 = (MQ == 7) ? 3 : MQ, NB = MQ0 + MQ1;
     constexpr int BMT = 32 * NB;
     const int tiles_n = (p.N + 255) >> 8, tiles_m = (p.M + BMT - 1) / BMT;
-    const int ntiles = tiles_m * tiles_n, G = gridDim.x;
+    const int G = gridDim.x;
     const int nt = p.K >> 6;
+    constexpr bool LIM = nt_epi_limits(EPI), LIMW = LIM;
+    int rl = p.M, full = tiles_m, cn = 0, gm = p.group_m, ntiles = tiles_m * tiles_n;
+    if constexpr (LIM) {
+        if (p.row_limit) {
+            rl = __builtin_amdgcn_readfirstlane(max(0, min(*p.row_limit, p.M)));
+            full = ntl_full_panels(rl, BMT, tiles_m);
+            cn = min(p.limit_col0 >> 8, tiles_n);
+            if (p.group_xcd) gm = max(1, (full + 7) >> 3);
+            ntiles = ntl_live_tiles(tiles_m, tiles_n, full, cn);
+        }
+    }
+    const bool run = !LIMW || (int)blockIdx.x < ntiles;
+    auto tile_mn = [&](int v, int& tmi, int& tni) {
+        if constexpr (LIMW) ntl_tile_mn(xcd_remap(v, ntiles), tiles_n, gm, full, cn, tmi, tni);
+        else ntp_tile_mn(xcd_remap(v, ntiles), tiles_m, tiles_n, gm, tmi, tni);
+    };
     const float alpha_all = __builtin_bit_cast(float, __builtin_amdgcn_readfirstlane(__builtin_bit_cast(int, p.alpha * (p.alpha_dev ? *p.alpha_dev : 1.0f))));
 
     const auto rsA = __builtin_amdgcn_make_buffer_rsrc((void*)p.A, 0, (int)((uint32_t)p.M * (uint32_t)p.lda * 2u), 0x00020000);
@@ -265,7 +307,7 @@
         int l = lane;
         asm volatile("" : "+v"(l));
         int tmi, tni;
-        ntp_tile_mn(xcd_remap(v, ntiles), tiles_m, tiles_n, p.group_m, tmi, tni);
+        tile_mn(v, tmi, tni);
         const int tm0 = tmi * BMT, tn0 = tni << 8;
         const int pos = l & 7;
 #pragma unroll
@@ -284,7 +326,7 @@
         }
     };
     Src cur;
-    set_src(blockIdx.x, cur);
+    if (run) set_src(blockIdx.x, cur);
     Src nxt_store;
     Src& nxt = MULTI ? nxt_store : cur;
     if constexpr (MULTI) nxt_store = cur;
@@ -395,7 +437,7 @@
 
     for (int v = blockIdx.x, vn = ntiles; v < ntiles; v = vn) {
         int tmi, tni;
-        ntp_tile_mn(xcd_remap(v, ntiles), tiles_m, tiles_n, p.group_m, tmi, tni);
+        tile_mn(v, tmi, tni);
         const int m0 = tmi * BMT, n0 = tni << 8;
         __builtin_amdgcn_s_waitcnt(mmb_waitcnt(INFL, 15));
         NT8_KTILE(0, cur, 1, cur, 2, true)
@@ -443,7 +485,11 @@
         asm volatile("" : "+v"(elane));
         const int efr = elane & 15, efq = elane >> 4;
         const float alpha = alpha_all;
-        const bool interior = (m0 + BMT <= q.M) && (n0 + 256 <= q.N);
+        int mlim = q.M;
+        if constexpr (LIM) {
+            if (n0 >= q.limit_col0) mlim = rl;
+        }
+        const bool interior = (m0 + BMT <= mlim) && (n0 + 256 <= q.N);
         const int mrow = m0 + wr * (16 * NB) + efr;
         const int ncol = n0 + wc * 64 + efq * 8;
         constexpr int PRE = 3;
@@ -518,7 +564,7 @@
                 float vv[8];
 #pragma unroll
                 for (int r = 0; r < 8; ++r) vv[r] = acc[i][2 * h + (r >> 2)][r & 3];
-                const bool ok = interior || (m < q.M && n + 8 <= q.N);
+                const bool ok = interior || (m < mlim && n + 8 <= q.N);
                 if constexpr (EPI & EPI_GELU) {
                     if (q.aux) {
                         bf16x8 u;
@@ -569,12 +615,14 @@
 #undef NT8_KTILE
 #undef NT8_PHASE
     };
+    if (run) {
     if constexpr (MQ0 == 3 || MQ1 == 3) {
         if (wave < 4) body(std::integral_constant<int, 2>{}); else body(std::integral_constant<int, 1>{});
     } else {
         body(std::integral_constant<int, MQ0 / 2>{});
     }
     if (wr == 0) __builtin_amdgcn_s_barrier();
+    }
     asm volatile("s_waitcnt vmcnt(0)" ::: "memory");
     if constexpr (MULTI) {
         auto kpe = __builtin_amdgcn_kernarg_segment_ptr();
@@ -600,9 +648,9 @@
     return 0;
 }
 template <int EPI>
-static int launch_nt8(hipStream_t s, const GemmNT& p, int bm, int tiles, int workgroups, int group_m) {
+static int launch_nt8(hipStream_t s, const GemmNT& p, int bm, int tiles, int workgroups, int group_m, int group_xcd) {
     GemmNT q = p;
-    q.group_m = group_m;
+    q.group_m = group_m; q.group_xcd = group_xcd;
     const bool use_queue = p.tile_counter && tiles > workgroups && !(workgroups & 7);
     if (!use_queue) q.tile_counter = q.tile_counter_next = nullptr;
     q.queue_xcd = 1;
@@ -614,7 +662,7 @@
 }
 
 enum { NTK_128 = 0, NTK_8PHASE = 3 };
-struct NTChoice { int kernel, bm, tiles, workgroups, group_m, use_queue; };
+struct NTChoice { int kernel, bm, tiles, workgroups, group_m, use_queue, group_xcd, live; };
 
 static bool nt8_eligible(const GemmNT& p, int epi) {
     const long long m = p.M, esz = (epi & EPI_OUT_F32) ? 4 : 2;
@@ -622,15 +670,24 @@
            m * p.ldr * 2 < (1ll << 32) && m * p.ldaux * 2 < (1ll << 32) && m * p.ldu * 2 < (1ll << 32);
 }
 
-static int nt_group_m(int M, int N, int K, int bm, int tiles, int cus) {
+static int nt_group_m(int M, int N, int K, int bm, int tiles, int cus, int* per_xcd = nullptr) {
+    if (per_xcd) *per_xcd = 0;
     if (tiles <= cus) return 1;
     if ((long long)N * K * 2 > (8ll << 20)) return tiles > 4 * cus ? 4 : 1;
+    if (per_xcd) *per_xcd = 1;
     return ((M + bm - 1) / bm + 7) / 8;
 }
 
-static NTChoice nt_choose(const GemmNT& p, int epi) {
-    NTChoice c = {NTK_128, 128, ((p.M + 127) / 128) * ((p.N + 127) / 128), 0, 1, 0};
+static NTChoice nt_choose(const GemmNT& p, int epi, int rows_hint = 0) {
+    NTChoice c = {NTK_128, 128, ((p.M + 127) / 128) * ((p.N + 127) / 128), 0, 1, 0, 0, 0};
     c.workgroups = c.tiles;
+    const bool limited = p.row_limit && nt_epi_limits(epi);
+    const int hint = (limited && rows_hint > 0) ? (rows_hint < p.M ? rows_hint : p.M) : p.M;
+    auto live_of = [&](int h, int tw) {
+        const int tm = (p.M + h - 1) / h, tnn = (p.N + tw - 1) / tw, cnn = p.limit_col0 / tw < tnn ? p.limit_col0 / tw : tnn;
+        return limited ? ntl_live_tiles(tm, tnn, ntl_full_panels(hint, h, tm), cnn) : tm * tnn;
+    };
+    c.live = live_of(128, 128);
     const int force = g_nt_force.load();
     const bool big = (p.M >= 512) && (p.N >= 256) && !(p.N & 7) && !(p.ldc & 7) && !(p.ldr & 7) && !(p.ldaux & 7) && !(p.ldu & 7);
     if (force == 1 || !nt8_eligible(p, epi) || (p.N & 7) || (force == 0 && !big)) return c;
@@ -641,8 +698,9 @@
         const int t = tiles_of(h);
         c.kernel = NTK_8PHASE; c.bm = h; c.tiles = t;
         c.workgroups = (h == 128 || t <= cus) ? t : cus;
-        c.group_m = nt_group_m(p.M, p.N, p.K, h, t, cus);
+        c.group_m = nt_group_m(p.M, p.N, p.K, h, t, cus, &c.group_xcd);
         c.use_queue = p.tile_counter != nullptr && t > c.workgroups && !(cus & 7);
+        c.live = live_of(h, 256);
         return c;
     };
     if (force == 128 || force == 192 || force == 224 || force == 256) return take(force);
@@ -657,7 +715,7 @@
         return take(256);
     }
     auto rounds = [&](int t) { return (long long)((t + cus - 1) / cus); };
-    const long long c192 = rounds(t192) * 1680, c224 = rounds(t224) * 1800, c256 = rounds(t256) * 2048;
+    const long long c192 = rounds(live_of(192, 256)) * 1680, c224 = rounds(live_of(224, 256)) * 1800, c256 = rounds(live_of(256, 256)) * 2048;
     int h = 224;
     if (100 * c256 < 97 * c224 && c256 <= c192) h = 256;
     else if (100 * c192 < 97 * c224 && c192 < c256) h = 192;
@@ -665,10 +723,10 @@
 }
 
 template <int EPI>
-static int dispatch_nt(hipStream_t s, const GemmNT& p) {
-    const NTChoice c = nt_choose(p, EPI);
+static int dispatch_nt(hipStream_t s, const GemmNT& p, int rows_hint) {
+    const NTChoice c = nt_choose(p, EPI, rows_hint);
     if (c.kernel == NTK_128) return launch_nt<EPI>(s, p);
-    return launch_nt8<EPI>(s, p, c.bm, c.tiles, c.workgroups, c.group_m);
+    return launch_nt8<EPI>(s, p, c.bm, c.tiles, c.workgroups, c.group_m, c.group_xcd);
 }
 
 struct TNProb { const bf16_t* A; const bf16_t* B; float* W; float* bias; int N, K, lda, ldb, tiles_k, tile0, M, slab_off, bias_off, acc; };
@@ -1009,6 +1067,12 @@
 }
 
 extern "C" {
+int mmbert_gemm_nt_rl(hipStream_t stream, const void* A, int lda, const void* B, int ldb, void* C, int ldc,
+                      int M, int N, int K, int epi, const float* bias, const void* R, int ldr, void* aux, int ldaux,
+                      const void* U, int ldu, float alpha, const float* alpha_dev,
+                      uint32_t drop_stream, uint32_t drop_thr16, float drop_scale, int* tile_queue,
+                      const int* row_limit, int limit_col0, int rows_hint);
+int mmbert_gemm_nt_describe_rl(int M, int N, int K, int epi, int with_queue, int limit_col0, int rows_hint, int* out);
 
 __global__ void nt_splitk_reduce_kernel(const float* __restrict__ slabs, int splits, long long stride, int M, int N, bf16_t* __restrict__ C, int ldc,
                                         const bf16_t* __restrict__ R, int ldr) {
@@ -1057,9 +1121,20 @@
                    int M, int N, int K, int epi, const float* bias, const void* R, int ldr, void* aux, int ldaux,
                    const void* U, int ldu, float alpha, const float* alpha_dev,
                    uint32_t drop_stream, uint32_t drop_thr16, float drop_scale, int* tile_queue) {
+    return mmbert_gemm_nt_rl(stream, A, lda, B, ldb, C, ldc, M, N, K, epi, bias, R, ldr, aux, ldaux, U, ldu, alpha, alpha_dev,
+                             drop_stream, drop_thr16, drop_scale, tile_queue, nullptr, 0, 0);
+}
+
+int mmbert_gemm_nt_rl(hipStream_t stream, const void* A, int lda, const void* B, int ldb, void* C, int ldc,
+                      int M, int N, int K, int epi, const float* bias, const void* R, int ldr, void* aux, int ldaux,
+                      const void* U, int ldu, float alpha, const float* alpha_dev,
+                      uint32_t drop_stream, uint32_t drop_thr16, float drop_scale, int* tile_queue,
+                      const int* row_limit, int limit_col0, int rows_hint) {
     if (M <= 0 || N <= 0) return 0;
     if (K <= 0 || (K & 63) || (N & 3) || (lda & 7) || (ldb & 7) || (ldc & 3)) return -1;
     GemmNT p;
+    const bool lim = row_limit && nt_epi_limits(epi) && limit_col0 >= 0 && !(limit_col0 & 255);
+    p.row_limit = lim ? row_limit : nullptr; p.limit_col0 = lim ? limit_col0 : 0; p.group_xcd = 0;
     p.A = (const bf16_t*)A; p.B = (const bf16_t*)B; p.C = C; p.bias = bias; p.R = (const bf16_t*)R;
     p.aux = (bf16_t*)aux; p.U = (const bf16_t*)U; p.alpha_dev = alpha_dev;
     p.M = M; p.N = N; p.K = K; p.lda = lda; p.ldb = ldb; p.ldc = ldc; p.ldr = ldr; p.ldaux = ldaux; p.ldu = ldu;
@@ -1067,30 +1142,48 @@
     p.kt_per_split = 0; p.split_stride = 0; p.group_m = 1;
     p.tile_counter = tile_queue; p.tile_counter_next = tile_queue ? tile_queue + 8 : nullptr;
     switch (epi) {
-        case 0: return dispatch_nt<0>(stream, p);
-        case EPI_BIAS: return dispatch_nt<EPI_BIAS>(stream, p);
-        case EPI_BIAS | EPI_GELU: return dispatch_nt<EPI_BIAS | EPI_GELU>(stream, p);
-        case EPI_BIAS | EPI_RESID: return dispatch_nt<EPI_BIAS | EPI_RESID>(stream, p);
-        case EPI_RESID: return dispatch_nt<EPI_RESID>(stream, p);
-        case EPI_GELU_BWD: return dispatch_nt<EPI_GELU_BWD>(stream, p);
-        case EPI_OUT_F32: return dispatch_nt<EPI_OUT_F32>(stream, p);
-        case EPI_BIAS | EPI_OUT_F32: return dispatch_nt<EPI_BIAS | EPI_OUT_F32>(stream, p);
+        case 0: return dispatch_nt<0>(stream, p, 0);
+        case EPI_BIAS: return dispatch_nt<EPI_BIAS>(stream, p, rows_hint);
+        case EPI_BIAS | EPI_GELU: return dispatch_nt<EPI_BIAS | EPI_GELU>(stream, p, 0);
+        case EPI_BIAS | EPI_RESID: return dispatch_nt<EPI_BIAS | EPI_RESID>(stream, p, 0);
+        case EPI_RESID: return dispatch_nt<EPI_RESID>(stream, p, 0);
+        case EPI_GELU_BWD: return dispatch_nt<EPI_GELU_BWD>(stream, p, 0);
+        case EPI_OUT_F32: return dispatch_nt<EPI_OUT_F32>(stream, p, 0);
+        case EPI_BIAS | EPI_OUT_F32: return dispatch_nt<EPI_BIAS | EPI_OUT_F32>(stream, p, 0);
         default: return -2;
     }
 }
 
 int mmbert_gemm_nt_describe(int M, int N, int K, int epi, int with_queue, int* out) {
+    int o[9];
+    const int e = mmbert_gemm_nt_describe_rl(M, N, K, epi, with_queue, -1, 0, out ? o : nullptr);
+    if (!e) memcpy(out, o, 8 * sizeof(int));
+    return e;
+}
+int mmbert_gemm_nt_describe_rl(int M, int N, int K, int epi, int with_queue, int limit_col0, int rows_hint, int* out) {
     if (!out || M <= 0 || N <= 0 || K <= 0) return -1;
     GemmNT p = {};
+    static const int dummy_limit = 0;
+    if (limit_col0 >= 0 && !(limit_col0 & 255) && nt_epi_limits(epi)) { p.row_limit = &dummy_limit; p.limit_col0 = limit_col0; }
     p.M = M; p.N = N; p.K = K; p.lda = K; p.ldb = K; p.ldc = N; p.ldr = (epi & (EPI_RESID)) ? N : 0; p.ldaux = (epi & EPI_GELU) ? N : 0;
     p.ldu = (epi & EPI_GELU_BWD) ? N : 0;
     static int dummy_queue[16];
     p.tile_counter = with_queue ? dummy_queue : nullptr;
-    const NTChoice c = nt_choose(p, epi);
+    const NTChoice c = nt_choose(p, epi, rows_hint);
     const int cus = device_cus();
+    out[8] = c.live;
     out[0] = c.kernel; out[1] = c.bm; out[2] = c.kernel == NTK_128 ? 128 : 256; out[3] = c.tiles; out[4] = c.workgroups;
     out[5] = (int)(100.0 * c.tiles / cus + 0.5); out[6] = c.group_m; out[7] = cus;
     return 0;
+}
+
+int mmbert_gemm_nt_limit_walk(int tiles_m, int tiles_n, int bm, int row_limit, int cn, int group_m, int* mn) {
+    if (tiles_m <= 0 || tiles_n <= 0 || bm <= 0 || row_limit < 0 || cn < 0) return -1;
+    if (cn > tiles_n) cn = tiles_n;
+    const int full = ntl_full_panels(row_limit, bm, tiles_m), live = ntl_live_tiles(tiles_m, tiles_n, full, cn);
+    const int gm = group_m > 0 ? group_m : ((full + 7) >> 3 > 1 ? (full + 7) >> 3 : 1);
+    if (mn) for (int t = 0; t < live; ++t) ntl_tile_mn(t, tiles_n, gm, full, cn, mn[2 * t], mn[2 * t + 1]);
+    return live;
 }
 
 #ifdef MMB_STAMPS
diff --git a/msa_amd/csrc/layer.hip b/msa_amd/csrc/layer.hip
--- a/msa_amd/csrc/layer.hip
+++ b/msa_amd/csrc/layer.hip
@@ -14,8 +14,8 @@
 int mmbert_layer_fwd(mmbert_stream_t s, const mmbert_attn_layout* L, const mmbert_layer_fwd_args* a) {
     if (!L || !a || a->rows <= 0) return a && a->rows == 0 ? 0 : -1;
     const int M = a->rows, H = a->H, I = a->I;
-    MMB_TRY(mmbert_gemm_nt(s, a->x, a->ldx, a->Wqkv, H, a->qkv, 3 * H, M, 3 * H, H, MMBERT_EPI_BIAS, a->bqkv, nullptr, 0, nullptr, 0, nullptr, 0,
-                           1.0f, nullptr, 0, 0, 1.0f, a->tile_queue));
+    MMB_TRY(mmbert_gemm_nt_rl(s, a->x, a->ldx, a->Wqkv, H, a->qkv, 3 * H, M, 3 * H, H, MMBERT_EPI_BIAS, a->bqkv, nullptr, 0, nullptr, 0, nullptr, 0,
+                              1.0f, nullptr, 0, 0, 1.0f, a->tile_queue, a->kv_rows, H, a->kv_rows_hint));
     MMB_TRY(mmbert_attn_fwd(s, a->qkv, a->actx, a->lse, L->key_bias, L->bias_start, H, L->heads, L->seq_start, L->seq_len, L->elem_base,
                             L->ftile_seq, L->ftile_r0, L->nftiles, a->att.stream, a->att.thr16, a->att.scale, L->kv_len, L->ftile_qshift, L->ftile_qend));
     MMB_TRY(mmbert_gemm_nt(s, a->actx, H, a->Wo, H, a->z1, H, M, H, H, MMBERT_EPI_BIAS | MMBERT_EPI_RESID, a->bo, a->x, a->ldx, nullptr, 0, nullptr, 0,
diff --git a/msa_amd/model.py b/msa_amd/model.py
--- a/msa_amd/model.py
+++ b/msa_amd/model.py
@@ -306,6 +306,11 @@
         ph = cfg.hidden_dropout_prob if train else 0.0
         pa = cfg.attention_probs_dropout_prob if train else 0.0
         saved = []
+        kv_rows = None
+        if (getattr(layout, "split", False) and getattr(layout, "counts", None) is not None and getattr(layout, "kv_len", None) is not None
+                and getattr(top, "skip_masked_keys", True)):
+            if getattr(top, "qkv_row_limit", True):
+                kv_rows = layout.counts[2:3]
         composite = getattr(top, "composite_layers", True) and ops.launches_unwrapped() and top.debug_hidden is None
         if composite:
             AL = ops.attn_layout_struct(key_bias, layout, backward=False)
@@ -341,6 +346,7 @@
                 a.u, a.m1, a.r1, a.m2, a.r2 = ops._ptr(u), ops._ptr(m1), ops._ptr(r1), ops._ptr(m2), ops._ptr(r2)
                 a.y2, a.ldy2, a.y2_rows = y2.data_ptr(), y2.stride(0), ops._ptr(y_rows) if last else None
                 a.tile_queue = tq
+                a.kv_rows, a.kv_rows_hint = ops._ptr(kv_rows), 0
                 ops._set_drop(a.att, d_att); ops._set_drop(a.h1, d_h1); ops._set_drop(a.h2, d_h2)
                 ops.layer_fwd(AL, a)
                 if probe is not None:
@@ -352,7 +358,7 @@
         for i in range(nl):
             lw = top._lw[i]
             d_att, d_h1, d_h2 = (ops.make_drop(pa, seed, 8 * i), ops.make_drop(ph, seed, 8 * i + 1), ops.make_drop(ph, seed, 8 * i + 2))
-            qkv = ops.gemm_nt(x, lw["Wqkv"], bias=lw["bqkv"])
+            qkv = ops.gemm_nt(x, lw["Wqkv"], bias=lw["bqkv"], row_limit=kv_rows, limit_col0=H)
             actx, lse = ops.attn_fwd(qkv, key_bias, layout, H, drop=d_att, kv_len=kv_len)
             if probe is not None:
                 probe(i, qkv)
diff --git a/msa_amd/ops.py b/msa_amd/ops.py
--- a/msa_amd/ops.py
+++ b/msa_amd/ops.py
@@ -85,7 +85,7 @@
 
 
 def gemm_nt(A, B, *, out=None, bias=None, gelu=False, aux=None, resid=None, gelu_bwd_u=None, alpha=1.0,
-            alpha_dev=None, drop: Drop = None, out_f32=False):
+            alpha_dev=None, drop: Drop = None, out_f32=False, row_limit=None, limit_col0=0, rows_hint=0):
     lib = _lib.load()
     M, K = A.shape
     N = B.shape[0]
@@ -104,6 +104,15 @@
     if out_f32:
         epi |= EPI_OUT_F32
     d = drop or NO_DROP
+    if row_limit is not None:
+        assert row_limit.dtype == torch.int32 and row_limit.device == A.device and row_limit.numel() >= 1
+        _lib.check(lib.mmbert_gemm_nt_rl(_stream(), A.data_ptr(), A.stride(0), B.data_ptr(), B.stride(0), out.data_ptr(), out.stride(0),
+                                         M, N, K, epi, _ptr(bias), _ptr(resid), resid.stride(0) if resid is not None else 0,
+                                         _ptr(aux), aux.stride(0) if aux is not None else 0,
+                                         _ptr(gelu_bwd_u), gelu_bwd_u.stride(0) if gelu_bwd_u is not None else 0,
+                                         float(alpha), _ptr(alpha_dev), d[0], d[1], d[2], _tile_queue(A.device),
+                                         row_limit.data_ptr(), int(limit_col0), int(rows_hint)), "mmbert_gemm_nt_rl")
+        return out
     _lib.check(lib.mmbert_gemm_nt(_stream(), A.data_ptr(), A.stride(0), B.data_ptr(), B.stride(0), out.data_ptr(), out.stride(0),
                                   M, N, K, epi, _ptr(bias), _ptr(resid), resid.stride(0) if resid is not None else 0,
                                   _ptr(aux), aux.stride(0) if aux is not None else 0,
@@ -112,12 +121,19 @@
     return out
 
 
-def gemm_nt_describe(M: int, N: int, K: int, epi: int = 0, with_queue: bool = False) -> dict:
+def gemm_nt_describe(M: int, N: int, K: int, epi: int = 0, with_queue: bool = False, limit_col0: Optional[int] = None, rows_hint: int = 0) -> dict:
     import ctypes
-    out = (ctypes.c_int * 8)()
-    _lib.check(_lib.load().mmbert_gemm_nt_describe(int(M), int(N), int(K), int(epi), int(bool(with_queue)), out), "mmbert_gemm_nt_describe")
+    out = (ctypes.c_int * 9)()
+    if limit_col0 is None:
+        _lib.check(_lib.load().mmbert_gemm_nt_describe(int(M), int(N), int(K), int(epi), int(bool(with_queue)), out), "mmbert_gemm_nt_describe")
+    else:
+        _lib.check(_lib.load().mmbert_gemm_nt_describe_rl(int(M), int(N), int(K), int(epi), int(bool(with_queue)), int(limit_col0), int(rows_hint), out),
+                   "mmbert_gemm_nt_describe_rl")
     kern = {0: "128x128", 1: "ring", 2: "persistent", 3: "8phase"}[out[0]]
-    return dict(kernel=kern, tile=f"{out[1]}x{out[2]}", tiles=out[3], workgroups=out[4], rounds=out[5] / 100.0, group_m=out[6], cus=out[7])
+    d = dict(kernel=kern, tile=f"{out[1]}x{out[2]}", tiles=out[3], workgroups=out[4], rounds=out[5] / 100.0, group_m=out[6], cus=out[7])
+    if limit_col0 is not None:
+        d["live"] = out[8]
+    return d
 
 
 _slab_cache = {}
@@ -1203,7 +1219,8 @@
 class _LayerFwd(ctypes.Structure):
     _fields_ = [(n, _VP) for n in ("x", "Wqkv", "Wo", "W1", "W2", "bqkv", "bo", "b1", "b2", "ln1_g", "ln1_b", "ln2_g", "ln2_b",
                                     "qkv", "actx", "lse", "z1", "y1", "m1", "r1", "u", "g", "z2", "y2", "m2", "r2", "y2_rows", "tile_queue")] + \
-               [("att", _Drop), ("h1", _Drop), ("h2", _Drop)] + [(n, _CI) for n in ("rows", "H", "I", "ldx", "ldy2")] + [("ln_eps", ctypes.c_float)]
+               [("att", _Drop), ("h1", _Drop), ("h2", _Drop)] + [(n, _CI) for n in ("rows", "H", "I", "ldx", "ldy2")] + [("ln_eps", ctypes.c_float)] + \
+               [("kv_rows", _VP), ("kv_rows_hint", _CI), ("pad_", _CI)]
 
 
 class _LayerBwd(ctypes.Structure):
```

Result: slower. 1238 (-1.4%).
